# FertigLab/CoGAPS

Measured on AMD Instinct MI355X. Metric: Gibbs atom proposals/sec, 20000x2000 dense D, nPatterns=50, at 1/2/4/8 GPUs, higher is better.
Workload: dtype f32

## Files before the change

cogaps_amd/csrc/eval_kernel.h:

```cpp
#pragma once
#include "gaps_state.h"
#include "gen_kernel.h"

CG_DEVICE cg_f4 ld4(const float *base, uint32_t j) { return reinterpret_cast<const cg_f4 *>(base)[j]; }
CG_DEVICE cg_f4 ld4_stream(const float *base, uint32_t j) { return cg_ld4_stream(base, j); }
CG_DEVICE void st4(float *base, uint32_t j, cg_f4 v) { reinterpret_cast<cg_f4 *>(base)[j] = v; }
CG_DEVICE cg_f4 f4_zero() { cg_f4 z; z.x = 0.f; z.y = 0.f; z.z = 0.f; z.w = 0.f; return z; }
CG_DEVICE cg_f4 f4_one() { cg_f4 z; z.x = 1.f; z.y = 1.f; z.z = 1.f; z.w = 1.f; return z; }

struct EvalAcc { float s, m; };

#define EVAL_ELEM(V, DD, SS, AA) { float ratio = (V) / (SS); a.s = a.s + (V) * ratio; a.m = a.m + ratio * ((DD) - (AA)); }
#define EVAL_ELEM_CH(V, DD, SS, AA) { float ratio = (V) / (SS); a.s = a.s + (V) * ratio; a.m = a.m + ratio * ((DD) - ((AA) + ch * (V))); }

#define EVAL_MODE_ONE 0
#define EVAL_MODE_CH 1
#define EVAL_MODE_SAME 2

#if defined(GEN_TIMELINE)
extern __device__ unsigned long long g_chain_rt[256 * 4];
__device__ unsigned long long g_eval_timeline[2 * 16 * 2 * 12];
#define EVAL_TS(id) do { if ((t & 63u) == 0u && ets_n < 11u) { ets[ets_n++] = ((unsigned long long)cg_clock() << 8) | (unsigned long long)(id); } } while (0)
#define EVAL_TS_DUMP(ty) do { const uint32_t lastW_ = (cg_bdim() - 1u) >> 6; if (cg_bid() < 16u && (t & 63u) == 0u && ((t >> 6) == 0u || (t >> 6) == lastW_) && qlen >= 40u && (PHASE != EVAL_CHAIN || (qlen >= 140u && hot.gs->nSteps - hot.gs->nDone >= 512u))) { \
    unsigned long long *o_ = &g_eval_timeline[((PHASE != EVAL_FUSED && PHASE != EVAL_CHAIN ? 16u : 0u) * 2u + cg_bid() * 2u + ((t >> 6) ? 1u : 0u)) * 12u]; o_[0] = (unsigned long long)(ty); for (uint32_t i_ = 0; i_ < 11u; ++i_) o_[1 + i_] = i_ < ets_n ? ets[i_] : 0ull; } } while (0)
#define EVAL_PIN(x) asm volatile("" : "+v"(x) :: "memory")
#define EVAL_TS_PARAMS , unsigned long long (&ets)[11], uint32_t &ets_n
#define EVAL_TS_ARGS , ets, ets_n
#else
#define EVAL_TS(id) do { } while (0)
#define EVAL_TS_DUMP(ty) do { } while (0)
#define EVAL_PIN(x) do { } while (0)
#define EVAL_TS_PARAMS
#define EVAL_TS_ARGS
#endif

template <int NC, int V>
CG_DEVICE void eval_vfinish(const float *lds, float (&tot)[NC], const uint32_t nwaves = 0u, const uint32_t tid = 0xFFFFFFFFu)
{
    constexpr int NV = NC * V;
    const uint32_t t = tid == 0xFFFFFFFFu ? cg_tid() : tid, nw = cg_fresh_u32(nwaves ? nwaves : (cg_bdim() >> 6));
    if (t < 64u) {
        const uint32_t i = t < (uint32_t)NV ? t : 0u;
        float y[16];
#pragma unroll
        for (uint32_t w = 0; w < 16; ++w) y[w] = lds[w * NV + i];
#pragma unroll
        for (uint32_t w = 0; w < 16; ++w) y[w] = w < nw ? y[w] : 0.f;
#pragma unroll
        for (uint32_t stride = 1; stride < 16u; stride <<= 1) {
#pragma unroll
            for (uint32_t k = 0; k + stride < 16u; k += 2u * stride) y[k] = y[k] + y[k + stride];
        }
        float z = y[0];
        for (int off = 1; off < V; off <<= 1) z = z + cg_shfl_xor_f32(z, off);
#pragma unroll
        for (int c = 0; c < NC; ++c) tot[c] = cg_lane_read_f32(z, c * V);
    }
}

template <int V>
CG_DEVICE void eval_vpark(float x, int j, float *lds, float (&tot)[1])
{
    x = cg_wave_allsum_f32(x);
    const uint32_t t = cg_tid();
    if (cg_bdim() > 64u) { if ((t & 63u) == 0) lds[(t >> 6) * V + j] = x; }
    else tot[0] = x;
}

struct EvalSpec { uint64_t rng; uint32_t n, mm; float l1, l2; };
CG_DEVICE void eval_spec_run(EvalSpec &sp)
{
    uint64_t r = sp.rng;
    sp.l1 = gm_logf_m(pcg_uniform(r), sp.mm);
    if (sp.n > 1u) sp.l2 = gm_logf_m(pcg_uniform(r), sp.mm);
    sp.n = 0u;
}
template <int NR, int MODE>
CG_DEVICE void eval_alpha(const SamplerDev &S, const uint32_t (&row)[NR], const uint32_t (&col)[NR], uint32_t col2, float ch, uint32_t chunk0, uint32_t stride, float *lds, float (&tot)[2 * NR], EvalSpec &spec EVAL_TS_PARAMS)
{
    constexpr int NC = 2 * NR;
    const uint32_t nq = S.Npad >> 2, BS = cg_bdim(), t = cg_tid(), nw = BS >> 6;
    float ps[NR], pm[NR];
    for (int r = 0; r < NR; ++r) { ps[r] = 0.f; pm[r] = 0.f; }
#if defined(GEN_PROFILE)
    if (!(S.dbg & 4u))
#endif
    for (uint32_t j = chunk0 + t; j < nq; j += stride) {
        cg_f4 v[NR], w2, d[NR], s[NR], p[NR];
#pragma unroll
        for (int r = 0; r < NR; ++r) {
            const float *Dr = S.D + (size_t)row[r] * S.Npad, *Sr = S.S2 + (size_t)row[r] * S.Npad, *Ar = S.AP + (size_t)row[r] * S.Npad;
            const float *Vr = S.other + (size_t)col[r] * S.Npad, *V2 = S.other + (size_t)col2 * S.Npad;
            v[r] = ld4(Vr, j); d[r] = ld4_stream(Dr, j); if (!S.defaultS) s[r] = ld4_stream(Sr, j); p[r] = ld4(Ar, j); if (MODE == EVAL_MODE_SAME) w2 = ld4(V2, j);
        }
        if (spec.n) { cg_sched_fence(); eval_spec_run(spec); cg_sched_fence(); }
        if (S.defaultS) {
#pragma unroll
            for (int r = 0; r < NR; ++r) {
                const float sx = gm_max(d[r].x * 0.1f, 0.1f), sy = gm_max(d[r].y * 0.1f, 0.1f), sz = gm_max(d[r].z * 0.1f, 0.1f), sw = gm_max(d[r].w * 0.1f, 0.1f);
                s[r].x = sx * sx; s[r].y = sy * sy; s[r].z = sz * sz; s[r].w = sw * sw;
            }
        }
#pragma unroll
        for (int r = 0; r < NR; ++r) {
            EvalAcc a; a.s = ps[r]; a.m = pm[r];
            if (MODE == EVAL_MODE_CH) { EVAL_ELEM_CH(v[r].x, d[r].x, s[r].x, p[r].x) EVAL_ELEM_CH(v[r].y, d[r].y, s[r].y, p[r].y) EVAL_ELEM_CH(v[r].z, d[r].z, s[r].z, p[r].z) EVAL_ELEM_CH(v[r].w, d[r].w, s[r].w, p[r].w) }
            else if (MODE == EVAL_MODE_SAME) {
                { float x = v[r].x - w2.x; EVAL_ELEM(x, d[r].x, s[r].x, p[r].x) }
                { float x = v[r].y - w2.y; EVAL_ELEM(x, d[r].y, s[r].y, p[r].y) }
                { float x = v[r].z - w2.z; EVAL_ELEM(x, d[r].z, s[r].z, p[r].z) }
                { float x = v[r].w - w2.w; EVAL_ELEM(x, d[r].w, s[r].w, p[r].w) }
            } else { EVAL_ELEM(v[r].x, d[r].x, s[r].x, p[r].x) EVAL_ELEM(v[r].y, d[r].y, s[r].y, p[r].y) EVAL_ELEM(v[r].z, d[r].z, s[r].z, p[r].z) EVAL_ELEM(v[r].w, d[r].w, s[r].w, p[r].w) }
            ps[r] = a.s; pm[r] = a.m;
        }
    }
    { float z_ = ps[0]; EVAL_PIN(z_); ps[0] = z_; } EVAL_TS(10);
#pragma unroll
    for (int r = 0; r < NR; ++r) { ps[r] = cg_wave_allsum_f32(ps[r]); pm[r] = cg_wave_allsum_f32(pm[r]); }
    if (nw > 1) {
        if ((t & 63u) == 0) {
#pragma unroll
            for (int r = 0; r < NR; ++r) { lds[(t >> 6) * NC + 2 * r] = ps[r]; lds[(t >> 6) * NC + 2 * r + 1] = pm[r]; }
        }
        EVAL_TS(11);
        cg_sync();
        EVAL_TS(12);
        eval_vfinish<NC, 1>(lds, tot);
    } else {
#pragma unroll
        for (int r = 0; r < NR; ++r) { tot[2 * r] = ps[r]; tot[2 * r + 1] = pm[r]; }
    }
}

#define EVAL_SEQ_BS 256
CG_DEVICE float eval_seq_fold(float acc, const float *term, uint32_t n)
{
    for (uint32_t i = 0; i < n; ++i) acc = acc + term[i];
    return acc;
}
template <int NR, int MODE>
CG_DEVICE void eval_alpha_seq(const SamplerDev &S, const uint32_t (&row)[NR], const uint32_t (&col)[NR], uint32_t col2, float ch, float *term, float *lds, float (&tot)[2 * NR])
{
    constexpr int NC = 2 * NR;
    const uint32_t nq = S.Npad >> 2, BS = cg_bdim(), t = cg_tid();
    float acc = 0.f;
    for (uint32_t base = 0; base < nq; base += BS) {
        const uint32_t j = base + t;
        if (j < nq) {
#pragma unroll
            for (int r = 0; r < NR; ++r) {
                const float *Dr = S.D + (size_t)row[r] * S.Npad, *Ar = S.AP + (size_t)row[r] * S.Npad;
                const float *Vr = S.other + (size_t)col[r] * S.Npad, *V2 = S.other + (size_t)col2 * S.Npad;
                const cg_f4 v4 = ld4(Vr, j), d4 = ld4(Dr, j), p4 = ld4(Ar, j);
                cg_f4 s4, w4 = f4_zero();
                if (S.defaultS) {
                    const float sx = gm_max(d4.x * 0.1f, 0.1f), sy = gm_max(d4.y * 0.1f, 0.1f), sz = gm_max(d4.z * 0.1f, 0.1f), sw = gm_max(d4.w * 0.1f, 0.1f);
                    s4.x = sx * sx; s4.y = sy * sy; s4.z = sz * sz; s4.w = sw * sw;
                } else s4 = ld4(S.S2 + (size_t)row[r] * S.Npad, j);
                if (MODE == EVAL_MODE_SAME) w4 = ld4(V2, j);
                const float vv[4] = {v4.x, v4.y, v4.z, v4.w}, dd[4] = {d4.x, d4.y, d4.z, d4.w}, pp[4] = {p4.x, p4.y, p4.z, p4.w}, ss[4] = {s4.x, s4.y, s4.z, s4.w}, ww[4] = {w4.x, w4.y, w4.z, w4.w};
#pragma unroll
                for (int e = 0; e < 4; ++e) {
                    const float v = (MODE == EVAL_MODE_SAME) ? vv[e] - ww[e] : vv[e];
                    const float ratio = v / ss[e];
                    const float ap = (MODE == EVAL_MODE_CH) ? pp[e] + ch * vv[e] : pp[e];
                    term[(2 * r) * 4u * BS + 4u * t + (uint32_t)e] = v * ratio;
                    term[(2 * r + 1) * 4u * BS + 4u * t + (uint32_t)e] = ratio * (dd[e] - ap);
                }
            }
        }
        cg_sync();
        const uint32_t first = 4u * base, n = (S.N - first) < 4u * BS ? (S.N - first) : 4u * BS;
        if (t < (uint32_t)NC) acc = eval_seq_fold(acc, term + t * 4u * BS, n);
        cg_sync();
    }
    if (t < (uint32_t)NC) lds[t] = acc;
    cg_sync();
// ... 87 lines not shown
            st4(S.AP + (size_t)r1 * S.Npad, j, q);
        } else {
            st4(S.AP + (size_t)r1 * S.Npad, j, q);
            cg_f4 w = e.p2;
            w.x = w.x + d2 * e.v2.x; w.y = w.y + d2 * e.v2.y; w.z = w.z + d2 * e.v2.z; w.w = w.w + d2 * e.v2.w;
            st4(S.AP + (size_t)r2 * S.Npad, j, w);
        }
    }
    if (nq > stride) eval_update_ap2(S, r1, c1, d1, r2, c2, d2, chunk0 + stride, stride);
}

CG_DEVICE void eval_store_matrix(const SamplerDev &S, uint32_t row, uint32_t col, float oldv, float newv)
{
    S.mat[(size_t)col * S.Mpad + row] = newv;
    const bool was = oldv > 0.f, is = newv > 0.f;
    if (was != is) { if (is) cg_atomic_add_u32(&S.colPos[col], 1u); else cg_atomic_sub_u32(&S.colPos[col], 1u); }
}
CG_DEVICE void eval_cache_erase(const SamplerDev &S, uint32_t h, uint32_t row, uint32_t col)
{
    const uint32_t k = cg_atomic_add_u32(&S.gs->eraseCount, 1u);
    if (k < S.eraseCap) S.eraseList[k] = ((unsigned long long)(row * S.K + col) << 32) | (unsigned long long)h; else S.gs->error = GAPS_ERR_ERASE_CAP;
}
CG_DEVICE void eval_domain_move(const SamplerDev &S, const PropRec &p, const AtomRec &a)
{
    const uint32_t h = p.h1, l = a.left, r = a.right;
    const uint32_t b1 = gen_bin_of(S, p.curPos), b2 = gen_bin_of(S, p.pos);
    const uint32_t head1 = S.binHead[b1];
    atom_set_pos(S, h, l, r, p.pos);
    if (head1 == h) {
        if (r != CG_NONE && gen_bin_of(S, a.rpos) == b1) S.binHead[b1] = r;
        else { S.binHead[b1] = CG_NONE; bm_clear(S, b1); }
    }
    if (l == CG_NONE || gen_bin_of(S, a.lpos) != b2) S.binHead[b2] = h;
    bm_set(S, b2);
}
struct EvalAtoms { AtomRec a1; uint32_t left2; };
CG_DEVICE EvalAtoms eval_atoms_load(const SamplerDev &S, const PropRec &p, bool writer)
{
    EvalAtoms e; e.a1.pos = 0; e.a1.lpos = 0; e.a1.rpos = 0; e.a1.left = CG_NONE; e.a1.right = CG_NONE; e.a1.mass = 0.f; e.a1.rmass = 0.f; e.a1.idx = 0; e.a1.pad0 = 0; e.left2 = CG_NONE;
    if (writer) { e.a1 = S.atoms[p.h1]; if (p.type == 'E') e.left2 = S.atoms[p.h2].left; }
    return e;
}

template <int NC>
CG_DEVICE void eval_pair_fold(const float *lds, const uint32_t tv, const uint32_t nw, float (&tot)[NC])
{
    constexpr int NV = NC * 2;
    if (tv < 64u) {
        const uint32_t i = tv < (uint32_t)NV ? tv : 0u;
        float y[16];
#pragma unroll
        for (uint32_t w = 0; w < 16; ++w) y[w] = lds[w * NV + i];
#pragma unroll
        for (uint32_t w = 0; w < 16; ++w) y[w] = w < nw ? y[w] : 0.f;
#pragma unroll
        for (uint32_t stride = 1; stride < 16u; stride <<= 1) {
#pragma unroll
            for (uint32_t k = 0; k + stride < 16u; k += 2u * stride) y[k] = y[k] + y[k + stride];
        }
        float z = y[0];
        z = z + cg_shfl_xor_f32(z, 1);
#pragma unroll
        for (int c = 0; c < NC; ++c) tot[c] = cg_lane_read_f32(z, c * 2);
    }
}
template <int NR, int MODE>
CG_DEVICE void eval_pair_alpha(const SamplerDev &S, const uint32_t (&row)[NR], const uint32_t (&col)[NR], uint32_t col2, float ch, const uint32_t u, const uint32_t H, float *lds, EvalSpec &spec)
{
    constexpr int NC = 2 * NR;
    const uint32_t nq = S.Npad >> 2;
    float ps[NR][2], pm[NR][2];
    cg_f4 v[2][NR], w2[2], d[2][NR], sq[2][NR], pp[2][NR];
#pragma unroll
    for (int sl = 0; sl < 2; ++sl) {
        const uint32_t j = u + (uint32_t)sl * H, jj = j < nq ? j : nq - 1u;
#pragma unroll
        for (int r = 0; r < NR; ++r) {
            const float *Dr = S.D + (size_t)row[r] * S.Npad, *Ar = S.AP + (size_t)row[r] * S.Npad, *Vr = S.other + (size_t)col[r] * S.Npad;
            v[sl][r] = ld4(Vr, jj); d[sl][r] = ld4_stream(Dr, jj); pp[sl][r] = ld4(Ar, jj);
            if (!S.defaultS) sq[sl][r] = ld4_stream(S.S2 + (size_t)row[r] * S.Npad, jj);
        }
        w2[sl] = (MODE == EVAL_MODE_SAME) ? ld4(S.other + (size_t)col2 * S.Npad, jj) : f4_zero();
    }
    if (spec.n) { cg_sched_fence(); eval_spec_run(spec); cg_sched_fence(); }
#pragma unroll
    for (int sl = 0; sl < 2; ++sl) {
        const uint32_t j = u + (uint32_t)sl * H;
#pragma unroll
        for (int r = 0; r < NR; ++r) {
            if (S.defaultS) {
                const float sx = gm_max(d[sl][r].x * 0.1f, 0.1f), sy = gm_max(d[sl][r].y * 0.1f, 0.1f), sz = gm_max(d[sl][r].z * 0.1f, 0.1f), sw = gm_max(d[sl][r].w * 0.1f, 0.1f);
                sq[sl][r].x = sx * sx; sq[sl][r].y = sy * sy; sq[sl][r].z = sz * sz; sq[sl][r].w = sw * sw;
            }
            EvalAcc a; a.s = 0.f; a.m = 0.f;
            if (j < nq) {
                const cg_f4 vv = v[sl][r], dd = d[sl][r], ss = sq[sl][r], aa = pp[sl][r], ww = w2[sl];
                if (MODE == EVAL_MODE_CH) { EVAL_ELEM_CH(vv.x, dd.x, ss.x, aa.x) EVAL_ELEM_CH(vv.y, dd.y, ss.y, aa.y) EVAL_ELEM_CH(vv.z, dd.z, ss.z, aa.z) EVAL_ELEM_CH(vv.w, dd.w, ss.w, aa.w) }
                else if (MODE == EVAL_MODE_SAME) {
                    { float x = vv.x - ww.x; EVAL_ELEM(x, dd.x, ss.x, aa.x) }
                    { float x = vv.y - ww.y; EVAL_ELEM(x, dd.y, ss.y, aa.y) }
                    { float x = vv.z - ww.z; EVAL_ELEM(x, dd.z, ss.z, aa.z) }
                    { float x = vv.w - ww.w; EVAL_ELEM(x, dd.w, ss.w, aa.w) }
                } else { EVAL_ELEM(vv.x, dd.x, ss.x, aa.x) EVAL_ELEM(vv.y, dd.y, ss.y, aa.y) EVAL_ELEM(vv.z, dd.z, ss.z, aa.z) EVAL_ELEM(vv.w, dd.w, ss.w, aa.w) }
            }
            ps[r][sl] = a.s; pm[r][sl] = a.m;
        }
    }
#pragma unroll
    for (int r = 0; r < NR; ++r) {
#pragma unroll
        for (int sl = 0; sl < 2; ++sl) { ps[r][sl] = cg_wave_allsum_f32(ps[r][sl]); pm[r][sl] = cg_wave_allsum_f32(pm[r][sl]); }
    }
    if ((u & 63u) == 0u) {
        float *o = lds + (u >> 6) * (NC * 2);
#pragma unroll
        for (int r = 0; r < NR; ++r) { o[(2 * r) * 2 + 0] = ps[r][0]; o[(2 * r) * 2 + 1] = ps[r][1]; o[(2 * r + 1) * 2 + 0] = pm[r][0]; o[(2 * r + 1) * 2 + 1] = pm[r][1]; }
    }
}
CG_DEVICE void eval_pair_update(const SamplerDev &S, const DecRec &d, const uint32_t u, const uint32_t H)
{
    const uint32_t nq = S.Npad >> 2;
    if (d.n == 0u) return;
    float *AP1 = S.AP + (size_t)d.r1 * S.Npad; const float *V1 = S.other + (size_t)d.c1 * S.Npad;
    const bool second = d.n == 2u, same = second && d.r1 == d.r2;
    float *AP2 = S.AP + (size_t)(second ? d.r2 : d.r1) * S.Npad; const float *V2 = S.other + (size_t)(second ? d.c2 : d.c1) * S.Npad;
    cg_f4 v1[2], p1[2], v2[2], p2[2];
#pragma unroll
    for (int sl = 0; sl < 2; ++sl) {
        const uint32_t j = u + (uint32_t)sl * H, jj = j < nq ? j : nq - 1u;
        v1[sl] = ld4(V1, jj); p1[sl] = ld4(AP1, jj); v2[sl] = ld4(V2, jj); p2[sl] = ld4(AP2, jj);
    }
#pragma unroll
    for (int sl = 0; sl < 2; ++sl) {
        const uint32_t j = u + (uint32_t)sl * H;
        if (j < nq) {
            cg_f4 q = p1[sl];
            q.x = q.x + d.d1 * v1[sl].x; q.y = q.y + d.d1 * v1[sl].y; q.z = q.z + d.d1 * v1[sl].z; q.w = q.w + d.d1 * v1[sl].w;
            if (same) { q.x = q.x + d.d2 * v2[sl].x; q.y = q.y + d.d2 * v2[sl].y; q.z = q.z + d.d2 * v2[sl].z; q.w = q.w + d.d2 * v2[sl].w; }
            st4(AP1, j, q);
            if (second && !same) {
                cg_f4 w = p2[sl];
                w.x = w.x + d.d2 * v2[sl].x; w.y = w.y + d.d2 * v2[sl].y; w.z = w.z + d.d2 * v2[sl].z; w.w = w.w + d.d2 * v2[sl].w;
                st4(AP2, j, w);
            }
        }
    }
}
CG_DEVICE void eval_chain_pair(const SamplerDev &S, unsigned long long *grans, const uint32_t tag, const float T, const PropRec &pA, const PropRec &pB, const uint32_t qA, const uint32_t qB)
{
    CG_SHARED float ldsP[2][16 * 8];
    CG_SHARED DecRec decP[2];
    const uint32_t t = cg_tid(), H = cg_bdim() >> 1, h = t >= H ? 1u : 0u, u = t - h * H, nwH = H >> 6;
    const PropRec p = h ? pB : pA;
    const uint32_t q = h ? qB : qA;
    const uint32_t mm = GM_MATH_PORTABLE;
    const float lambda = S.lambda;
    const bool scalarLane = u < 64u;
    uint64_t rng = p.rng;
    const bool two = (p.type == 'M' || p.type == 'E');
    const float m1 = p.m1, m2 = p.m2, old1 = p.old1, old2 = p.old2;
    const bool gibbs1 = (p.gibbs & 1u) != 0u, gibbs2 = (p.gibbs & 2u) != 0u;
    const bool need = (p.type == 'B') ? gibbs1 : ((p.type == 'D' || p.type == 'M') ? true : (gibbs1 || gibbs2));
    const bool diff = two && p.r1 != p.r2;
    const uint32_t alphaUnits = need ? (!two ? 4u : (diff ? 8u : 5u)) : 0u;
    EvalSpec spec; spec.rng = rng; spec.mm = mm; spec.l1 = 0.f; spec.l2 = 0.f;
    spec.n = (scalarLane && need && (p.type == 'D' || p.type == 'M')) ? ((p.type == 'D' && gibbs1) ? 2u : 1u) : 0u;
    float *lds = &ldsP[h][0];
    if (need) {
        const uint32_t rowA[1] = {p.r1}, colA[1] = {p.c1};
        if (diff) { const uint32_t rowAB[2] = {p.r1, p.r2}, colAB[2] = {p.c1, p.c2}; eval_pair_alpha<2, EVAL_MODE_ONE>(S, rowAB, colAB, 0u, 0.f, u, H, lds, spec); }
        else if (p.type == 'D') eval_pair_alpha<1, EVAL_MODE_CH>(S, rowA, colA, 0u, -1.f * m1, u, H, lds, spec);
        else if (two) eval_pair_alpha<1, EVAL_MODE_SAME>(S, rowA, colA, p.c2, 0.f, u, H, lds, spec);
        else eval_pair_alpha<1, EVAL_MODE_ONE>(S, rowA, colA, 0u, 0.f, u, H, lds, spec);
    }
    cg_sync();
    float s = 0.f, smu = 0.f;
    if (need) {
        if (diff) { float tot[4] = {0.f, 0.f, 0.f, 0.f}; eval_pair_fold<4>(lds, u, nwH, tot); s = tot[0] + tot[2]; smu = tot[1] - tot[3]; }
        else { float t2[2] = {0.f, 0.f}; eval_pair_fold<2>(lds, u, nwH, t2); s = t2[0]; smu = t2[1]; }
        if (spec.n) eval_spec_run(spec);
    }
    s = s * T; smu = smu * T;
    DecRec owe; owe.n = 0; owe.r1 = 0; owe.c1 = 0; owe.d1 = 0.f; owe.r2 = 0; owe.c2 = 0; owe.d2 = 0.f; owe.pad = 0;
    if (scalarLane) {
        uint32_t code = CHAIN_NONE, nUpd = 0; float val = 0.f;
        if (p.type == 'B') {
            float bv = 0.f; uint32_t bhas = 0;
            if (gibbs1) { OptF g = gm_gibbs_mass(s, smu, 0.f, S.maxGibbsMass, rng, S.luts, true, lambda); bv = g.v; bhas = g.has ? 1u : 0u; }
            else { bv = pcg_exponential(rng, lambda, mm); bhas = 1u; }
            if (bhas != 0u && bv >= GAPS_EPSILON) { code = CHAIN_APPLY; val = bv; nUpd = 1u; owe.n = 1u; owe.r1 = p.r1; owe.c1 = p.c1; owe.d1 = bv; }
            else code = CHAIN_ERASE;
        } else if (p.type == 'D') {
            float rebirth = m1; bool drew = false;
            if (gibbs1) { OptF g = gm_gibbs_mass(s, smu, 0.f, S.maxGibbsMass, rng, S.luts, true, lambda); if (g.has) { rebirth = g.v; drew = true; } }
            const float deltaLL = rebirth * (smu - s * rebirth / 2.f);
            const float logU = drew ? spec.l2 : spec.l1;
            if (logU < deltaLL) {
                if (rebirth != m1) { const float nv = gm_max(old1 + (rebirth - m1), 0.f); code = CHAIN_APPLY; val = rebirth; nUpd = 1u; owe.n = 1u; owe.r1 = p.r1; owe.c1 = p.c1; owe.d1 = nv - old1; }
            } else { const float nv = gm_max(old1 + (-1.f * m1), 0.f); code = CHAIN_ERASE; nUpd = 1u; owe.n = 1u; owe.r1 = p.r1; owe.c1 = p.c1; owe.d1 = nv - old1; }
        } else if (p.type == 'M') {
            const float deltaLL = -1.f * m1 * (smu + s * m1 / 2.f);
            if (spec.l1 < deltaLL) { const float nv1 = gm_max(old1 + (-m1), 0.f); code = CHAIN_APPLY; nUpd = 2u; owe.n = 2u; owe.r1 = p.r1; owe.c1 = p.c1; owe.d1 = nv1 - old1; owe.r2 = p.r2; owe.c2 = p.c2; owe.d2 = m1; }
        } else if (need) {
            OptF g0 = gm_gibbs_mass(s, smu, -m1, m2, rng, S.luts, false, 0.f);
            const float gv = g0.v, n1 = m1 + gv, n2 = m2 - gv;
            if (g0.has && n1 > GAPS_EPSILON && n2 > GAPS_EPSILON) {
                const float nv1 = gm_max(old1 + (n1 - m1), 0.f), nv2 = gm_max(old2 + (n2 - m2), 0.f);
                code = CHAIN_APPLY; val = gv; nUpd = 2u; owe.n = 2u; owe.r1 = p.r1; owe.c1 = p.c1; owe.d1 = nv1 - old1; owe.r2 = p.r2; owe.c2 = p.c2; owe.d2 = nv2 - old2;
            }
        }
        if (u == 0u) {
            unsigned long long *gr = grans + (size_t)q * CHAIN_GRAN_STRIDE; const uint32_t units = nUpd * 3u + alphaUnits;
            cg_store_agent_u64(&gr[0], ((unsigned long long)tag << 32) | (unsigned long long)(code | (units << 8)));
            cg_store_agent_u64(&gr[1], ((unsigned long long)tag << 32) | (unsigned long long)gm_f2u(val));
            decP[h] = owe;
        }
    }
    cg_sync();
    const DecRec d = decP[h];
    eval_pair_update(S, d, u, H);
    cg_sync();
}

#if defined(GEN_PROFILE) && !defined(GEN_SUBMARKS) && !defined(GEN_ROUNDMARKS)
#define EVAL_PROF(i) do { if (t == 0 && cg_bid() == 0) { unsigned long long now_ = cg_clock(); cg_atomic_add_u64(&S.gs->prof[8 + (i)], now_ - eprof_last); eprof_last = now_; } } while (0)
#else
#define EVAL_PROF(i) do { } while (0)
#endif

#define EVAL_FUSED 0
#define EVAL_ALPHA 1
#define EVAL_APPLY 2
#define EVAL_SEQ 3
#define EVAL_CHAIN 5
#define EVAL_CHAIN_SPLIT 6
#define EVAL_DECIDE 4

struct EvalHot { const PropRec *queue; const GenScalars *gs; uint32_t queueCap; const ChainSlot *slot; unsigned long long *grans; };
struct EvalFirst { PropRec p; uint32_t qlen; float T; uint32_t tag; };
template <int PHASE>
CG_DEVICE EvalFirst eval_first(const EvalHot hot, uint32_t slices, uint32_t vbid)
{
    const uint32_t qFirst = (PHASE == EVAL_FUSED || PHASE == EVAL_SEQ || PHASE == EVAL_CHAIN) ? vbid : vbid / slices;
    EvalFirst f; f.p = hot.queue[qFirst < hot.queueCap ? qFirst : 0u]; f.T = hot.gs->annealTemp;
    if (PHASE == EVAL_CHAIN || PHASE == EVAL_CHAIN_SPLIT) { const ChainSlot cs = *hot.slot; f.qlen = cs.qlen; f.tag = cs.tag; }
    else { f.qlen = hot.gs->qlen; f.tag = (PHASE == EVAL_DECIDE) ? (uint32_t)hot.gs->batchEpoch : 0u; }
    return f;
}
template <int PHASE>
CG_DEVICE const SamplerDev &eval_record(const SamplerDev CG_CONSTANT *sp)
{
    cg_sched_fence();
    cg_const_lines lines;
    cg_const_warm_begin<sizeof(SamplerDev)>(sp, lines);
    sp = cg_const_warm_end(sp, lines);
    return *(const SamplerDev *)sp;
}
CG_DEVICE void eval_chain_updates(const SamplerDev &S, const EvalHot hot, const uint32_t tag, const uint32_t qlen, const uint32_t wg, const uint32_t nwg)
{
    const uint32_t TPB = cg_bdim(), nq = S.Npad >> 2;
    uint32_t parts = (nq + 4u * TPB - 1u) / (4u * TPB);
    parts = parts < 1u ? 1u : (parts > 64u ? 64u : parts);
    for (uint32_t item = wg; item < qlen * parts; item += nwg) {
        const uint32_t q = item / parts, part = item - q * parts;
        const PropRec p = hot.queue[q < hot.queueCap ? q : 0u];
        const unsigned long long *gr = hot.grans + (size_t)q * CHAIN_GRAN_STRIDE;
        unsigned long long g0 = 0ull, g1 = 0ull; uint32_t spins = 0; bool have = true;
        for (;;) {
            g0 = cg_load_l2_u64(&gr[0]); g1 = cg_load_l2_u64(&gr[1]);
            const bool ok = (uint32_t)(g0 >> 32) == tag && (uint32_t)(g1 >> 32) == tag;
            if (cg_ballot(!ok) == 0ull) break;
            if (cg_poll_expired(++spins)) { if (cg_tid() == 0u) S.gs->error = GAPS_ERR_SPIN; have = false; break; }
            cg_poll_pause();
        }
        if (!have) return;
        const uint32_t code = (uint32_t)g0 & 0xFFu; const float val = gm_u2f((uint32_t)g1);
        const float m1 = p.m1, m2 = p.m2, old1 = p.old1, old2 = p.old2;
        if (code == CHAIN_APPLY) {
            if (p.type == 'B') eval_update_ap(S, p.r1, p.c1, val, part * TPB, TPB * parts);
            else if (p.type == 'D') { const float nv = gm_max(old1 + (val - m1), 0.f); eval_update_ap(S, p.r1, p.c1, nv - old1, part * TPB, TPB * parts); }
            else if (p.type == 'M') { const float nv1 = gm_max(old1 + (-m1), 0.f); eval_update_ap2(S, p.r1, p.c1, nv1 - old1, p.r2, p.c2, m1, part * TPB, TPB * parts); }
            else if (p.type == 'E') {
                const float n1 = m1 + val, n2 = m2 - val;
                const float nv1 = gm_max(old1 + (n1 - m1), 0.f), nv2 = gm_max(old2 + (n2 - m2), 0.f);
                eval_update_ap2(S, p.r1, p.c1, nv1 - old1, p.r2, p.c2, nv2 - old2, part * TPB, TPB * parts);
            }
        } else if (code == CHAIN_ERASE && p.type == 'D') { const float nv = gm_max(old1 + (-1.f * m1), 0.f); eval_update_ap(S, p.r1, p.c1, nv - old1, part * TPB, TPB * parts); }
    }
}

template <int PHASE, bool SINGLE>
CG_DEVICE void eval_body(const SamplerDev &S, uint32_t slices, const uint32_t vbid, const uint32_t vgdim, const EvalHot hot, const EvalFirst &first)
{
#if defined(GEN_TIMELINE)
    unsigned long long ets[11]; uint32_t ets_n = 0;
#endif
    constexpr bool CHAINP = PHASE == EVAL_CHAIN_SPLIT;
    constexpr bool CHAIN = PHASE == EVAL_CHAIN || CHAINP;
    constexpr bool FUSEDF = PHASE == EVAL_FUSED || PHASE == EVAL_CHAIN;
    const uint32_t qFirst = (FUSEDF || PHASE == EVAL_SEQ) ? vbid : vbid / slices;
    PropRec pNext = first.p;
    const uint32_t qlen = first.qlen;
    const float T = first.T;
    CG_SHARED float lds[16 * 4];
    CG_SHARED float decf; CG_SHARED uint32_t deci;

    CG_SHARED float seqTerm[PHASE == EVAL_SEQ ? 4 * 4 * EVAL_SEQ_BS : 1];
    constexpr bool WHOLE = FUSEDF || PHASE == EVAL_SEQ;
    const uint32_t mm = (PHASE == EVAL_SEQ) ? S.mathMode : GM_MATH_PORTABLE;
    const uint32_t t = cg_tid(), BS = cg_bdim();
#if defined(GEN_PROFILE) && !defined(GEN_SUBMARKS) && !defined(GEN_ROUNDMARKS)
    unsigned long long eprof_last = cg_clock();
#endif
    const float lambda = S.lambda;
    EVAL_TS(0);
    const bool multiWave = BS > 64u;
    const bool scalarLane = !multiWave || t < 64u;
    const uint32_t slice = WHOLE ? 0u : vbid % slices;
    const uint32_t qStep = WHOLE ? vgdim : vgdim / slices;
    const uint32_t chunk0 = slice * BS, stride = WHOLE ? BS : S.redW;
    constexpr bool DECIDE = PHASE == EVAL_DECIDE || CHAINP;
    const bool decider = DECIDE && slice + 1u == slices;
    const bool writer = !CHAIN && (DECIDE ? decider : slice == 0u) && t == 0u;
#if defined(GEN_TIMELINE)
#define EVAL_PUBLISH_RT() do { if (CHAIN && t == 0u && q < 255u && qlen >= 140u && hot.gs->nSteps - hot.gs->nDone >= 512u) g_chain_rt[q * 4u + 1u] = __builtin_amdgcn_s_memrealtime(); } while (0)
#else
#define EVAL_PUBLISH_RT() do { } while (0)
#endif
#define EVAL_PUBLISH(CODE, VAL, NUPD) do { EVAL_TS(7); EVAL_PUBLISH_RT(); if (CHAIN && t == 0u) { unsigned long long *gr_ = hot.grans + (size_t)q * CHAIN_GRAN_STRIDE; const uint32_t units_ = (NUPD) * 3u + alphaUnits; \
        cg_store_agent_u64(&gr_[0], ((unsigned long long)first.tag << 32) | (unsigned long long)((CODE) | (units_ << 8))); \
        cg_store_agent_u64(&gr_[1], ((unsigned long long)first.tag << 32) | (unsigned long long)gm_f2u(VAL)); } } while (0)
#define EVAL_BCAST(F0, I0) do { if (multiWave && !DECIDE) { if (t == 0) { decf = (F0); deci = (I0); } cg_sync(); (F0) = decf; (I0) = deci; } } while (0)
    if (PHASE == EVAL_DECIDE && vbid == 0u && t == 0u) S.gs->applyCount = qlen;
    for (uint32_t q = qFirst; ; q += qStep) {
        const PropRec p = pNext;
        if (q >= qlen) break;
        if (PHASE == EVAL_CHAIN && q + qStep < qlen && (S.Npad >> 2) <= BS && BS >= 128u) {
            const uint32_t qB = q + qStep;
            const PropRec pB = hot.queue[qB < hot.queueCap ? qB : 0u];
            const uint32_t qN = qB + qStep;
            if (qN < qlen) pNext = hot.queue[qN < hot.queueCap ? qN : 0u];
#if defined(COGAPS_EMUL)
            if (t == 0u) cg_atomic_add_u64(&S.gs->prof[7], 1ull);
#endif
            eval_chain_pair(S, hot.grans, first.tag, T, p, pB, q, qB);
            if (qN >= qlen) break;
            q = qB;
            continue;
        }
        { uint32_t ty_ = p.type; EVAL_PIN(ty_); }
        EVAL_TS(1);
        uint64_t rng = p.rng; uint32_t nUpd = 0;
#if defined(EVAL_ATOMS_LATE)
        EvalAtoms ea = eval_atoms_load(S, p, writer && PHASE == EVAL_SEQ);
#else
        EvalAtoms ea = eval_atoms_load(S, p, writer && (PHASE == EVAL_FUSED || PHASE == EVAL_SEQ));
#endif
        bool eaLoaded = false;
        const bool two = (p.type == 'M' || p.type == 'E');
        const float m1 = p.m1, m2 = p.m2, old1 = p.old1, old2 = p.old2;
        const bool gibbs1 = (p.gibbs & 1u) != 0u, gibbs2 = (p.gibbs & 2u) != 0u;
        EVAL_PROF(0);
        EVAL_TS(2);
#if defined(GEN_PROFILE)
        if (S.dbg & 1u) { if (p.type == 0xFFu || m1 == -1.f) S.queueUnits[q] = (uint32_t)old1; break; }
#endif
        bool need = (p.type == 'B') ? gibbs1 : ((p.type == 'D' || p.type == 'M') ? true : (gibbs1 || gibbs2));
#if defined(GEN_PROFILE)
        if (S.dbg & 16u) need = false;
#endif
        const bool diff = two && p.r1 != p.r2;
        const uint32_t alphaUnits = need ? (!two ? 4u : (diff ? 8u : 5u)) : 0u;
        float s = 0.f, smu = 0.f;
        uint32_t typeX = p.type;
        constexpr bool PRE = FUSEDF && SINGLE;
        EvalPre pre; pre.v1 = f4_zero(); pre.p1 = f4_zero(); pre.v2 = f4_zero(); pre.p2 = f4_zero();
        const uint32_t jPre = chunk0 + t;
#define EVAL_PREFETCH() do { if (PRE && jPre < (S.Npad >> 2)) { \
            pre.v1 = ld4(S.other + (size_t)p.c1 * S.Npad, jPre); pre.p1 = ld4(S.AP + (size_t)p.r1 * S.Npad, jPre); \
            if (two) { pre.v2 = ld4(S.other + (size_t)p.c2 * S.Npad, jPre); if (p.r1 != p.r2) pre.p2 = ld4(S.AP + (size_t)p.r2 * S.Npad, jPre); } } } while (0)
        DecRec owe; owe.n = 0; owe.r1 = 0; owe.c1 = 0; owe.d1 = 0.f; owe.r2 = 0; owe.c2 = 0; owe.d2 = 0.f; owe.pad = 0;
#define EVAL_UPD1(ROW, COL, DELTA) do { if (DECIDE) { owe.n = 1u; owe.r1 = (ROW); owe.c1 = (COL); owe.d1 = (DELTA); } \
            else if (PRE) eval_update_pre1(S, (ROW), (COL), (DELTA), chunk0, stride, pre.v1, pre.p1); else eval_update_ap(S, (ROW), (COL), (DELTA), chunk0, stride); } while (0)
#define EVAL_UPD2(R1, C1, D1, R2, C2, D2) do { if (DECIDE) { owe.n = 2u; owe.r1 = (R1); owe.c1 = (C1); owe.d1 = (D1); owe.r2 = (R2); owe.c2 = (C2); owe.d2 = (D2); } \
            else if (PRE) eval_update_pre2(S, (R1), (C1), (D1), (R2), (C2), (D2), chunk0, stride, pre); else eval_update_ap2(S, (R1), (C1), (D1), (R2), (C2), (D2), chunk0, stride); } while (0)
        constexpr bool AHEAD = (FUSEDF && SINGLE) || DECIDE;
        EvalSpec spec; spec.rng = rng; spec.mm = mm; spec.l1 = 0.f; spec.l2 = 0.f;
        spec.n = (AHEAD && scalarLane && need && (p.type == 'D' || p.type == 'M')) ? ((p.type == 'D' && gibbs1) ? 2u : 1u) : 0u;
        if (need) {
            float tot[4] = {0.f, 0.f, 0.f, 0.f};
            if (PHASE == EVAL_SEQ) {
                const uint32_t rowA[1] = {p.r1}, colA[1] = {p.c1};
                if (diff) {
                    const uint32_t rowAB[2] = {p.r1, p.r2}, colAB[2] = {p.c1, p.c2};
                    eval_alpha_seq<2, EVAL_MODE_ONE>(S, rowAB, colAB, 0u, 0.f, seqTerm, lds, tot);
                } else {
                    float t2[2] = {0.f, 0.f};
                    if (p.type == 'D') eval_alpha_seq<1, EVAL_MODE_CH>(S, rowA, colA, 0u, -1.f * m1, seqTerm, lds, t2);
                    else if (two) eval_alpha_seq<1, EVAL_MODE_SAME>(S, rowA, colA, p.c2, 0.f, seqTerm, lds, t2);
                    else eval_alpha_seq<1, EVAL_MODE_ONE>(S, rowA, colA, 0u, 0.f, seqTerm, lds, t2);
                    tot[0] = t2[0]; tot[1] = t2[1];
                }
            } else if (PHASE != EVAL_APPLY) {
                const uint32_t rowA[1] = {p.r1}, colA[1] = {p.c1};
                if (diff) {
                    const uint32_t rowAB[2] = {p.r1, p.r2}, colAB[2] = {p.c1, p.c2};
                    eval_alpha<2, EVAL_MODE_ONE>(S, rowAB, colAB, 0u, 0.f, chunk0, stride, lds, tot, spec EVAL_TS_ARGS);
                } else {
                    float t2[2] = {0.f, 0.f};
                    if (p.type == 'D') eval_alpha<1, EVAL_MODE_CH>(S, rowA, colA, 0u, -1.f * m1, chunk0, stride, lds, t2, spec EVAL_TS_ARGS);
                    else if (two) eval_alpha<1, EVAL_MODE_SAME>(S, rowA, colA, p.c2, 0.f, chunk0, stride, lds, t2, spec EVAL_TS_ARGS);
                    else eval_alpha<1, EVAL_MODE_ONE>(S, rowA, colA, 0u, 0.f, chunk0, stride, lds, t2, spec EVAL_TS_ARGS);
                    tot[0] = t2[0]; tot[1] = t2[1];
                }
                if (PHASE == EVAL_ALPHA) { if (t == 0) { float *o = S.partials + (size_t)q * 64u + slice; o[0] = tot[0]; o[16] = tot[1]; o[32] = tot[2]; o[48] = tot[3]; } }
                if (DECIDE && t < 64u) {
                    unsigned long long *gr = S.grans + (size_t)q * 64u;
                    if (!decider) {
                        if (t < 4u) { const float v = t == 0u ? tot[0] : (t == 1u ? tot[1] : (t == 2u ? tot[2] : tot[3])); cg_store_agent_u64(&gr[slice * 4u + t], ((unsigned long long)first.tag << 32) | (unsigned long long)gm_f2u(v)); }
                    } else {
                        ea = eval_atoms_load(S, p, writer); eaLoaded = true;
                        const uint32_t comp = t >> 4, sl = t & 15u;
                        const bool want = sl + 1u < slices;
                        unsigned long long g = 0ull; uint32_t spins = 0;
                        for (;;) {
                            if (want) g = cg_load_l2_u64(&gr[sl * 4u + comp]);
                            const bool ok = !want || (uint32_t)(g >> 32) == first.tag;
                            if (cg_ballot(!ok) == 0ull) break;
                            if (cg_poll_expired(++spins)) { if (t == 0u) S.gs->error = GAPS_ERR_SPIN; typeX = 0u; break; }
                            cg_poll_pause();
                        }
                        const float own = comp == 0u ? tot[0] : (comp == 1u ? tot[1] : (comp == 2u ? tot[2] : tot[3]));
                        float z = want ? gm_u2f((uint32_t)g) : (sl + 1u == slices ? own : 0.f);
                        const uint32_t slots = S.redW / BS;
                        for (uint32_t st = 1; st < slots; st <<= 1) z = z + cg_shfl_xor_f32(z, (int)st);
                        tot[0] = cg_lane_read_f32(z, 0); tot[1] = cg_lane_read_f32(z, 16); tot[2] = cg_lane_read_f32(z, 32); tot[3] = cg_lane_read_f32(z, 48);
                    }
                }
            } else {
                if (t < 64u) {
                    const uint32_t slots = S.redW / BS;
                    float z = ((t & 15u) < slices) ? S.partials[(size_t)q * 64u + t] : 0.f;
                    for (uint32_t st = 1; st < slots; st <<= 1) z = z + cg_shfl_xor_f32(z, (int)st);
                    tot[0] = cg_lane_read_f32(z, 0); tot[1] = cg_lane_read_f32(z, 16); tot[2] = cg_lane_read_f32(z, 32); tot[3] = cg_lane_read_f32(z, 48);
                }
            }
            s = diff ? tot[0] + tot[2] : tot[0]; smu = diff ? tot[1] - tot[3] : tot[1];
            if (AHEAD && spec.n) eval_spec_run(spec);
        }
        EVAL_PIN(s); EVAL_TS(3);
        if (FUSEDF) EVAL_PREFETCH();
#if defined(EVAL_ATOMS_LATE)
        if (PHASE == EVAL_FUSED) ea = eval_atoms_load(S, p, writer);
#endif
        if (PHASE == EVAL_APPLY || (DECIDE && !eaLoaded)) ea = eval_atoms_load(S, p, writer);
        if (PHASE == EVAL_ALPHA || (DECIDE && !decider)) { if (q + qStep >= qlen) break; { const uint32_t qn_ = q + qStep; pNext = hot.queue[qn_ < hot.queueCap ? qn_ : 0u]; } cg_sync(); continue; }
        s = s * T; smu = smu * T;
#if defined(GEN_PROFILE)
        if (S.dbg & 8u) { if (q + qStep >= qlen) break; { const uint32_t qn_ = q + qStep; pNext = hot.queue[qn_ < hot.queueCap ? qn_ : 0u]; } cg_sync(); continue; }
#endif
        if (typeX == 'B') {
            float bv = 0.f; uint32_t bhas = 0;
            if (scalarLane) {
                if (gibbs1) { OptF g = gm_gibbs_mass(s, smu, 0.f, S.maxGibbsMass, rng, S.luts, true, lambda); bv = g.v; bhas = g.has ? 1u : 0u; }
                else { bv = pcg_exponential(rng, lambda, mm); bhas = 1u; }
                if (bhas != 0u && bv >= GAPS_EPSILON) EVAL_PUBLISH(CHAIN_APPLY, bv, 1u); else EVAL_PUBLISH(CHAIN_ERASE, 0.f, 0u);
            }
            EVAL_PIN(bv); EVAL_TS(4);
            EVAL_BCAST(bv, bhas);
            EVAL_TS(5);
            if (bhas != 0u && bv >= GAPS_EPSILON) {
                EVAL_UPD1(p.r1, p.c1, bv);
                ++nUpd;
                if (writer) { atom_set_mass(S, p.h1, ea.a1.left, bv); eval_store_matrix(S, p.r1, p.c1, old1, old1 + bv); }
            } else if (writer) eval_cache_erase(S, p.h1, p.r1, p.c1);
        } else if (typeX == 'D') {
            float rebirth = m1;
            EVAL_PROF(1);
            uint32_t acc = 0;
            if (scalarLane) {
                bool drew = false;
                if (gibbs1) {
                    OptF g = gm_gibbs_mass(s, smu, 0.f, S.maxGibbsMass, rng, S.luts, true, lambda);
                    if (g.has) { rebirth = g.v; drew = true; }
                }
                const float deltaLL = rebirth * (smu - s * rebirth / 2.f);
                const float logU = (AHEAD && need) ? (drew ? spec.l2 : spec.l1) : gm_logf_m(pcg_uniform(rng), mm);
                acc = (logU < deltaLL) ? 1u : 0u;
                if (acc != 0u) { if (rebirth != m1) EVAL_PUBLISH(CHAIN_APPLY, rebirth, 1u); else EVAL_PUBLISH(CHAIN_NONE, 0.f, 0u); } else EVAL_PUBLISH(CHAIN_ERASE, 0.f, 1u);
            }
            EVAL_PIN(acc); EVAL_TS(4);
            EVAL_BCAST(rebirth, acc);
            EVAL_TS(5);
            EVAL_PROF(2);
            if (acc != 0u) {
                if (rebirth != m1) {
                    const float nv = gm_max(old1 + (rebirth - m1), 0.f);
                    EVAL_UPD1(p.r1, p.c1, nv - old1);
                    ++nUpd;
                    if (writer) { eval_store_matrix(S, p.r1, p.c1, old1, nv); atom_set_mass(S, p.h1, ea.a1.left, rebirth); }
                }
            } else {
                const float nv = gm_max(old1 + (-1.f * m1), 0.f);
                EVAL_UPD1(p.r1, p.c1, nv - old1);
                ++nUpd;
                if (writer) { eval_store_matrix(S, p.r1, p.c1, old1, nv); eval_cache_erase(S, p.h1, p.r1, p.c1); }
            }
            EVAL_PROF(3);
        } else if (typeX == 'M') {
            uint32_t acc = 0; float unused = 0.f;
            if (scalarLane) { const float deltaLL = -1.f * m1 * (smu + s * m1 / 2.f); const float logU = (AHEAD && need) ? spec.l1 : gm_logf_m(pcg_uniform(rng), mm); acc = (logU < deltaLL) ? 1u : 0u;
                              if (acc) EVAL_PUBLISH(CHAIN_APPLY, 0.f, 2u); else EVAL_PUBLISH(CHAIN_NONE, 0.f, 0u); }
            EVAL_PIN(acc); EVAL_TS(4);
            EVAL_BCAST(unused, acc);
            EVAL_TS(5);
            if (acc) {
                const float nv1 = gm_max(old1 + (-m1), 0.f);
                EVAL_UPD2(p.r1, p.c1, nv1 - old1, p.r2, p.c2, m1);
                nUpd += 2;
                if (writer) {
                    eval_domain_move(S, p, ea.a1);
                    eval_store_matrix(S, p.r1, p.c1, old1, nv1);
                    eval_store_matrix(S, p.r2, p.c2, old2, old2 + m1);
                }
            }
        } else if (need && typeX == 'E') {
            float gv = 0.f; uint32_t gh = 0;
            if (scalarLane) { OptF g0 = gm_gibbs_mass(s, smu, -m1, m2, rng, S.luts, false, 0.f); gv = g0.v; gh = g0.has ? 1u : 0u;
                              if (gh != 0u && m1 + gv > GAPS_EPSILON && m2 - gv > GAPS_EPSILON) EVAL_PUBLISH(CHAIN_APPLY, gv, 2u); else EVAL_PUBLISH(CHAIN_NONE, 0.f, 0u); }
            EVAL_PIN(gv); EVAL_TS(4);
            EVAL_BCAST(gv, gh);
            EVAL_TS(5);
            const float n1 = m1 + gv, n2 = m2 - gv;
            if (gh != 0u && n1 > GAPS_EPSILON && n2 > GAPS_EPSILON) {
                const float nv1 = gm_max(old1 + (n1 - m1), 0.f);
                const float nv2 = gm_max(old2 + (n2 - m2), 0.f);
                EVAL_UPD2(p.r1, p.c1, nv1 - old1, p.r2, p.c2, nv2 - old2);
                nUpd += 2;
                if (writer) {
                    eval_store_matrix(S, p.r1, p.c1, old1, nv1);
                    eval_store_matrix(S, p.r2, p.c2, old2, nv2);
                    atom_set_mass(S, p.h1, ea.a1.left, n1); atom_set_mass(S, p.h2, ea.left2, n2);
                }
            }
        }
        else EVAL_PUBLISH(CHAIN_NONE, 0.f, 0u);
        EVAL_TS(6);
        EVAL_TS_DUMP(p.type | (nUpd << 8) | ((p.r1 == p.r2 ? 1u : 0u) << 16));
        if (DECIDE && writer) S.dec[q] = owe;
        if (writer) {
            uint32_t units = nUpd * 3u;
            if (need) units += !two ? 4u : (diff ? 8u : 5u);
            S.queueUnits[q] = units;
        }
        if (q + qStep >= qlen) break;
        { const uint32_t qn_ = q + qStep; pNext = hot.queue[qn_ < hot.queueCap ? qn_ : 0u]; }
        cg_sync();
    }
#if !defined(COGAPS_EMUL)
    if (CHAINP) eval_chain_updates(S, hot, first.tag, qlen, vbid, vgdim);
#endif
}

template <int PHASE>
#ifndef EVAL_APPLY_WAVES
#define EVAL_APPLY_WAVES 6
#endif
CG_KERNEL void CG_LAUNCH_BOUNDS2((PHASE == EVAL_SEQ ? EVAL_SEQ_BS : 1024), (PHASE == EVAL_FUSED || PHASE == EVAL_SEQ ? 4 : (PHASE == EVAL_APPLY || PHASE == EVAL_DECIDE ? EVAL_APPLY_WAVES : 8))) eval_kernel(const PropRec *hotQueue, const GenScalars *hotGs, uint32_t hotCap, uint32_t slices, const SamplerDev CG_CONSTANT *sp)
{
    EvalHot hot; hot.queue = hotQueue; hot.gs = hotGs; hot.queueCap = hotCap; hot.slot = nullptr; hot.grans = nullptr;
    const EvalFirst first = eval_first<PHASE>(hot, slices, cg_bid());
    const SamplerDev &S = eval_record<PHASE>(sp);
    eval_body<PHASE, true>(S, slices, cg_bid(), cg_gdim(), hot, first);
}

template <int PHASE>
#ifndef EVAL_MULTI_FUSED_WAVES
#define EVAL_MULTI_FUSED_WAVES 6
#endif
CG_KERNEL void CG_LAUNCH_BOUNDS2(1024, (PHASE == EVAL_FUSED ? EVAL_MULTI_FUSED_WAVES : (PHASE == EVAL_APPLY ? EVAL_APPLY_WAVES : 8))) eval_kernel_multi(const SamplerDev CG_CONSTANT *arr, uint32_t slices, uint32_t wgPerChain)
{
    const uint32_t chain = cg_bid() / wgPerChain;
    const SamplerDev CG_CONSTANT *sp = arr + chain;
    cg_const_warm<sizeof(SamplerDev)>(sp);
    const SamplerDev &S = *(const SamplerDev *)sp;
    EvalHot hot; hot.queue = S.queue; hot.gs = S.gs; hot.queueCap = S.queueCap; hot.slot = nullptr; hot.grans = nullptr;
    const uint32_t vbid = cg_bid() - chain * wgPerChain;
    eval_body<PHASE, false>(S, slices, vbid, wgPerChain, hot, eval_first<PHASE>(hot, slices, vbid));
}

CG_DEVICE void eval_apply_items(const SamplerDev &S, const uint32_t wg, const uint32_t nwg)
{
    const uint32_t count = S.gs->applyCount;
    const uint32_t TPB = cg_bdim(), nq = S.Npad >> 2;
    uint32_t parts = (nq + 4u * TPB - 1u) / (4u * TPB);
    parts = parts < 1u ? 1u : (parts > 64u ? 64u : parts);
    for (uint32_t item = wg; item < count * parts; item += nwg) {
        const uint32_t q = item / parts, part = item - q * parts;
        const DecRec d = S.dec[q];
        if (d.n == 1u) eval_update_ap(S, d.r1, d.c1, d.d1, part * TPB, TPB * parts);
        else if (d.n == 2u) eval_update_ap2(S, d.r1, d.c1, d.d1, d.r2, d.c2, d.d2, part * TPB, TPB * parts);
    }
}
template <int WIN>
CG_KERNEL void CG_LAUNCH_BOUNDS(WIN + 64) gen_apply_kernel(const uint64_t *lcgMul, const uint64_t *lcgInc, GenScalars *gs, const unsigned long long *eraseList, const uint32_t *queueUnits,
                                                          uint32_t eraseCap, uint32_t queueCap, const SamplerDev CG_CONSTANT *sp)
{
    if (cg_bid() != 0u) {
        cg_const_warm<sizeof(SamplerDev)>(sp);
        eval_apply_items(*(const SamplerDev *)sp, cg_bid() - 1u, cg_gdim() - 1u);
        return;
    }
    GenHot hot; hot.lcgMul = lcgMul; hot.lcgInc = lcgInc; hot.gs = gs; hot.eraseList = eraseList; hot.queueUnits = queueUnits; hot.eraseCap = eraseCap; hot.queueCap = queueCap;
    gen_body<WIN, true, false, 0>(sp, hot);
}
```

cogaps_amd/csrc/gen_chain_apply.h:

```cpp
#pragma once
struct ChainItem {
    uint32_t type; float m1, m2, old1, old2; uint64_t pos; unsigned long long eraseEntry;
    float *mass1, *rm1, *mass2, *rm2;
    float *mat1, *mat2; uint32_t *col1, *col2;
    uint64_t *pos1, *rposL, *lposR;
    uint32_t mb1, mb2;
    uint32_t *head1, *head2; uint32_t head1Val, h1;
    unsigned long long *b0clr, *b0set, *b1set, *b2set; uint32_t bit1, bit2, bit1w, bit2w;
    uint32_t hL, hR, h2, l2, cell1, cell2, idx;
    uint32_t sparse; float *rows1, *rows2; unsigned long long *fl1, *fl2; unsigned long long fbit1, fbit2; float colv1, colv2; uint32_t flg1, flg2;
};
CG_DEVICE void chain_item_clear(ChainItem &it)
{
    it.type = 0; it.m1 = 0.f; it.m2 = 0.f; it.old1 = 0.f; it.old2 = 0.f; it.pos = 0; it.eraseEntry = 0ull;
    it.mass1 = nullptr; it.rm1 = nullptr; it.mass2 = nullptr; it.rm2 = nullptr; it.mat1 = nullptr; it.mat2 = nullptr; it.col1 = nullptr; it.col2 = nullptr;
    it.mb1 = 0; it.mb2 = 0;
    it.pos1 = nullptr; it.rposL = nullptr; it.lposR = nullptr; it.head1 = nullptr; it.head2 = nullptr; it.head1Val = CG_NONE; it.h1 = 0;
    it.b0clr = nullptr; it.b0set = nullptr; it.b1set = nullptr; it.b2set = nullptr; it.bit1 = 0; it.bit2 = 0; it.bit1w = 0; it.bit2w = 0;
    it.hL = CG_NONE; it.hR = CG_NONE; it.h2 = CG_NONE; it.l2 = CG_NONE; it.cell1 = 0; it.cell2 = 0; it.idx = 0;
    it.sparse = 0; it.rows1 = nullptr; it.rows2 = nullptr; it.fl1 = nullptr; it.fl2 = nullptr; it.fbit1 = 0ull; it.fbit2 = 0ull; it.colv1 = 0.f; it.colv2 = 0.f; it.flg1 = 0; it.flg2 = 0;
}
struct ChainMid { AtomRec a; uint32_t l2, head1, b1, b2; unsigned long long x1, x2;
                  float colv1, colv2; unsigned long long fw1, fw2; };
CG_DEVICE ChainMid chain_fetch_mid(const SamplerDev &S, const PropRec &p, const bool sparse)
{
    ChainMid m;
    const uint32_t hE = p.type == 'E' ? p.h2 : p.h1;
    m.b1 = gen_bin_of(S, p.curPos); m.b2 = gen_bin_of(S, p.pos);
    const uint32_t w0 = m.b2 >> 6, w1 = w0 >> 6, w2 = w1 >> 6;
    m.a = S.atoms[p.h1];
    m.l2 = S.atoms[hE].left;
    m.head1 = S.binHead[m.b1];
    m.x1 = S.bits1[w1]; m.x2 = S.bits2[w2];
    m.colv1 = 0.f; m.colv2 = 0.f; m.fw1 = 0ull; m.fw2 = 0ull;
    if (sparse) {
        m.colv1 = S.mat[(size_t)p.c1 * S.Mpad + p.r1]; m.fw1 = S.mflags[(size_t)p.c1 * S.Mw + (p.r1 >> 6)];
        m.colv2 = S.mat[(size_t)p.c2 * S.Mpad + p.r2]; m.fw2 = S.mflags[(size_t)p.c2 * S.Mw + (p.r2 >> 6)];
    }
    return m;
}
CG_DEVICE void chain_fetch_build(const SamplerDev &S, const PropRec &p, const ChainMid &m, ChainItem &it, const bool sparse);
CG_DEVICE void chain_fetch(const SamplerDev &S, const PropRec *queueRd, uint32_t q, ChainItem &it, const bool sparse)
{
    const PropRec p = queueRd[q];
    const ChainMid m = chain_fetch_mid(S, p, sparse);
    chain_fetch_build(S, p, m, it, sparse);
}
CG_DEVICE void chain_fetch_build(const SamplerDev &S, const PropRec &p, const ChainMid &m, ChainItem &it, const bool sparse)
{
    chain_item_clear(it);
    it.type = p.type; it.m1 = p.m1; it.m2 = p.m2; it.old1 = p.old1; it.old2 = p.old2; it.pos = p.pos; it.h1 = p.h1;
    it.eraseEntry = ((unsigned long long)(p.r1 * S.K + p.c1) << 32) | (unsigned long long)p.h1;
    const AtomRec a = m.a;
    it.hL = a.left; it.hR = a.right; it.idx = a.idx; it.cell1 = p.r1 * S.K + p.c1; it.cell2 = p.r2 * S.K + p.c2; it.h2 = p.h2; it.l2 = m.l2;
    it.mass1 = &S.atoms[p.h1].mass; it.rm1 = a.left != CG_NONE ? &S.atoms[a.left].rmass : nullptr;
    it.mat1 = &S.mat[(size_t)p.c1 * S.Mpad + p.r1]; it.col1 = &S.colPos[p.c1];
    const bool two = p.type == 'M' || p.type == 'E';
    if (two) { it.mat2 = &S.mat[(size_t)p.c2 * S.Mpad + p.r2]; it.col2 = &S.colPos[p.c2]; }
    if (sparse) {
        it.sparse = 1u;
        it.rows1 = &S.rows[(size_t)p.r1 * S.Kpad + p.c1]; it.fl1 = &S.mflags[(size_t)p.c1 * S.Mw + (p.r1 >> 6)]; it.fbit1 = 1ull << (p.r1 & 63u);
        it.colv1 = m.colv1; it.flg1 = (uint32_t)((m.fw1 >> (p.r1 & 63u)) & 1ull);
        if (two) {
            it.rows2 = &S.rows[(size_t)p.r2 * S.Kpad + p.c2]; it.fl2 = &S.mflags[(size_t)p.c2 * S.Mw + (p.r2 >> 6)]; it.fbit2 = 1ull << (p.r2 & 63u);
            it.colv2 = m.colv2; it.flg2 = (uint32_t)((m.fw2 >> (p.r2 & 63u)) & 1ull);
        }
    }
    if (p.type == 'E') { const uint32_t l2 = m.l2; it.mass2 = &S.atoms[p.h2].mass; it.rm2 = l2 != CG_NONE ? &S.atoms[l2].rmass : nullptr; }
    if (p.type == 'M') {
        const uint32_t b1 = m.b1, b2 = m.b2;
        it.mb1 = b1; it.mb2 = b2;
        const uint32_t head1 = m.head1;
        const uint32_t w0 = b2 >> 6, w1 = w0 >> 6, w2 = w1 >> 6;
        const unsigned long long x1 = m.x1, x2 = m.x2;
        it.pos1 = &S.atoms[p.h1].pos; it.rposL = a.left != CG_NONE ? &S.atoms[a.left].rpos : nullptr; it.lposR = a.right != CG_NONE ? &S.atoms[a.right].lpos : nullptr;
        if (head1 == p.h1) {
            it.head1 = &S.binHead[b1];
            if (a.right != CG_NONE && gen_bin_of(S, a.rpos) == b1) it.head1Val = a.right; else { it.head1Val = CG_NONE; it.b0clr = &S.bits0[b1 >> 6]; it.bit1 = b1 & 63u; }
        }
        if (a.left == CG_NONE || gen_bin_of(S, a.lpos) != b2) it.head2 = &S.binHead[b2];
        it.b0set = &S.bits0[w0]; it.bit2 = b2 & 63u;
        if (!((x1 >> (w0 & 63u)) & 1ull)) { it.b1set = &S.bits1[w1]; it.bit1w = w0 & 63u; }
        if (!((x2 >> (w1 & 63u)) & 1ull)) { it.b2set = &S.bits2[w2]; it.bit2w = w1 & 63u; }
    }
}
CG_DEVICE void chain_store_matrix(float *cell, uint32_t *col, float oldv, float newv)
{
    *cell = newv;
    const bool was = oldv > 0.f, is = newv > 0.f;
    if (was != is) { if (is) cg_atomic_add_u32(col, 1u); else cg_atomic_sub_u32(col, 1u); }
}
CG_DEVICE void chain_store_hybrid(float *rowCell, float *colCell, unsigned long long *flagWord, unsigned long long bit, uint32_t *colCount, float rowNew, float colNew, bool wasFlagged)
{
    *rowCell = rowNew;
    const bool zero = colNew < GAPS_EPSILON;
    if (zero) {
        if (wasFlagged) { (void)cg_atomic_and_u64(flagWord, ~bit); (void)cg_atomic_sub_u32(colCount, 1u); }
        *colCell = 0.f;
    } else {
        if (!wasFlagged) { (void)cg_atomic_or_u64(flagWord, bit); (void)cg_atomic_add_u32(colCount, 1u); }
        *colCell = colNew;
    }
}
CG_DEVICE bool chain_apply(const ChainItem &it, uint32_t code, float val)
{
    const uint32_t tB = it.type == 'B', tD = it.type == 'D', tM = it.type == 'M', tE = it.type == 'E';
    const bool app = code == CHAIN_APPLY, era = code == CHAIN_ERASE;
    const float n1 = tE ? it.m1 + val : val, n2 = it.m2 - val;
    float d1 = tB ? val : (tD ? (val - it.m1) : (tM ? -it.m1 : (n1 - it.m1)));
    d1 = (era && tD) ? -1.f * it.m1 : d1;
    const float s1 = it.old1 + d1;
    const float nv1 = tB ? s1 : gm_max(s1, 0.f);
    const float s2 = it.old2 + (tM ? it.m1 : (n2 - it.m2));
    const float nv2 = tM ? s2 : gm_max(s2, 0.f);
    const bool doMat1 = app || (era && tD != 0u), doMat2 = app && (tM | tE) != 0u;
    const bool doMass1 = app && tM == 0u, doMass2 = app && tE != 0u;
    if (doMass1) { *it.mass1 = n1; if (it.rm1) *it.rm1 = n1; }
    if (doMass2) { *it.mass2 = n2; if (it.rm2) *it.rm2 = n2; }
    if (it.sparse) {
        if (doMat1) { const float colNew = tB ? it.colv1 + d1 : nv1; chain_store_hybrid(it.rows1, it.mat1, it.fl1, it.fbit1, it.col1, nv1, colNew, it.flg1 != 0u); }
        if (doMat2) { const float colNew = tM ? it.colv2 + it.m1 : nv2; chain_store_hybrid(it.rows2, it.mat2, it.fl2, it.fbit2, it.col2, nv2, colNew, it.flg2 != 0u); }
    } else {
        if (doMat1) chain_store_matrix(it.mat1, it.col1, it.old1, nv1);
        if (doMat2) chain_store_matrix(it.mat2, it.col2, it.old2, nv2);
    }
    if (app && tM != 0u) {
        *it.pos1 = it.pos; if (it.rposL) *it.rposL = it.pos; if (it.lposR) *it.lposR = it.pos;
        if (it.head1) *it.head1 = it.head1Val;
        if (it.b0clr) cg_atomic_and_u64(it.b0clr, ~(1ull << it.bit1));
        if (it.head2) *it.head2 = it.h1;
        cg_atomic_or_u64(it.b0set, 1ull << it.bit2);
        if (it.b1set) cg_atomic_or_u64(it.b1set, 1ull << it.bit1w);
        if (it.b2set) cg_atomic_or_u64(it.b2set, 1ull << it.bit2w);
    }
    return era;
}
```

cogaps_amd/csrc/gen_draw.h:

```cpp
#pragma once
struct GenRoundCtx {
    unsigned t; uint64_t jm0, ji0, jm1, ji1, seed1, batchEpoch, g_qrng; uint32_t n0, updBase, remaining, K, g_skip, e_prevQ; float dp0, g_u1, g_u2; GenScalars *gs;
    float tabHi, tabLo;
    PropRec *queueOut;
    uint32_t dpBase;
    uint32_t sparse;
};
struct GenSpec {
    uint32_t bBefore, dBefore, guess, active; float u1, u2;
    uint32_t go, ct, info; uint64_t rng, pos; uint32_t bin, r1, c1;
};
template <int WIN>
CG_DEVICE void gen_spec_a1(const SamplerDev &S, GenShared<WIN> &sh, const GenRoundCtx &c, const uint32_t nLo, const uint32_t nHi, const float dpAtLo, const float dpAtHi, GenSpec &sp)
{
    const unsigned t = c.t;
    const uint32_t winN = c.remaining < (uint32_t)WIN ? c.remaining : (uint32_t)WIN;
    const uint32_t active = t < winN;
    uint64_t s = (c.g_skip ? c.jm1 : c.jm0) * c.g_qrng + (c.g_skip ? c.ji1 : c.ji0);
    float u1 = pcg_uniform(s), u2 = pcg_uniform(s);
    const uint32_t cached = (c.g_skip != 0u) & (uint32_t)(t == 0u);
    u1 = cached ? c.g_u1 : u1; u2 = cached ? c.g_u2 : u2;
    const uint32_t gLo = gen_decide(u1, u2, nLo, nLo, dpAtLo, dpAtLo), gHi = gen_decide(u1, u2, nHi, nHi, dpAtHi, dpAtHi);
    if (cg_ballot(active && gLo != gHi) != 0ull && (t & 63u) == 0u) sh.specBad = 1u;
#if defined(GEN_SPEC_BAD_EVERY)
    if (t == 0u && (sh.g.batchEpoch % (uint64_t)GEN_SPEC_BAD_EVERY) == 0ull) sh.specBad = 1u;
#endif
    const uint32_t guess = active ? gHi : (uint32_t)GEN_T_NONE;
    sh.u1[t] = u1; sh.u2[t] = u2;
    uint32_t eX[4], tX[4];
    gen_count4<WIN>(sh.wtot4, t, guess == 'B', guess == 'D', guess == 'M', guess == 'E', eX, tX);
    sp.bBefore = eX[0]; sp.dBefore = eX[1]; sp.u1 = u1; sp.u2 = u2; sp.guess = guess; sp.active = active;
    const uint32_t goA = (uint32_t)(guess != GEN_T_NONE);
    const uint32_t k0 = (uint32_t)(guess == 'B') | (uint32_t)(guess == 'D'), k1 = (uint32_t)(guess == 'M');
    const uint32_t T0 = tX[0] + tX[1], T1 = tX[2], T2 = tX[3];
    if (goA) {
        uint32_t slot = T0 + T1 + eX[3];
        slot = k1 ? T0 + eX[2] : slot;
        slot = k0 ? eX[0] + eX[1] : slot;
        sh.perm[slot] = (uint16_t)t;
        sh.info[t] = guess | (eX[0] << 8);
    }
    if (t == 0) { sh.nWork = T0 + T1 + T2; sh.nBD = T0; }
}
template <int WIN>
CG_DEVICE void gen_spec_slot(const SamplerDev &S, GenShared<WIN> &sh, const GenRoundCtx &c, GenSpec &sp)
{
    const unsigned t = c.t;
    const bool go = t < sh.nWork;
    sp.go = go ? 1u : 0u;
    sp.ct = go ? (uint32_t)sh.perm[t] : 0u;
    sp.info = go ? sh.info[sp.ct] : 0u;
    sp.rng = go ? pcg_from_seed(sh.seed[sp.ct]) : 0ull;
    sp.pos = 0; sp.bin = 0; sp.r1 = 0; sp.c1 = 0;
    if (go && (sp.info & 0xFFu) == 'B') {
        uint64_t x = pcg_u64(sp.rng);
        while (x >= S.limitL) x = pcg_u64(sp.rng);
        sp.pos = (S.iPartL == 1ull ? x : gm_udiv64(x, S.iPartL)) + 1ull;
        sp.bin = gen_bin_of(S, sp.pos); sp.r1 = gen_div_k(S, sp.bin); sp.c1 = sp.bin - sp.r1 * c.K;
    }
}

CG_DEVICE void gen_mark_dirty(uint32_t *dirty, uint32_t bin)
{
    const uint32_t w = (bin >> 6) & 16383u;
    cg_atomic_or_u32(&dirty[w >> 5], 1u << (w & 31u));
}

struct GenNotePos { uint32_t a, b; };
template <int WORDS>
CG_DEVICE GenNotePos gen_note_pos(uint32_t key)
{
    constexpr uint32_t LOG2 = WORDS == 4096 ? 17u : (WORDS == 2048 ? 16u : 13u);
    static_assert(WORDS == 4096 || WORDS == 2048 || WORDS == 256, "bit numbers are 17 / 16 / 13 bits of the hash");
    const uint32_t h = key * 2654435761u;
    GenNotePos p; p.a = h >> (32u - LOG2); p.b = (h ^ (h >> 11)) & ((1u << LOG2) - 1u);
    return p;
}
CG_DEVICE void gen_note_set(uint32_t *bits, const GenNotePos p)
{
    cg_atomic_or_u32(&bits[p.a >> 5], 1u << (p.a & 31u));
    cg_atomic_or_u32(&bits[p.b >> 5], 1u << (p.b & 31u));
}
CG_DEVICE uint32_t gen_note_get(const uint32_t *bits, const GenNotePos p)
{
    return (bits[p.a >> 5] >> (p.a & 31u)) & (bits[p.b >> 5] >> (p.b & 31u)) & 1u;
}

struct GenDraw {
    uint32_t go, flags; bool isB, pick;
    uint64_t rng, rngPick, pos, cpos;
    uint32_t h1, h2, i1, hl, hr, r1, c1, r2, c2, bin;
    float nm1, nm2, amass, m2x, old1, old2; uint32_t gib1, gib2;
    uint64_t lposB, rposB; float rmassB;
    uint32_t headBin, v2, v3, xPick; bool redo;
};
CG_DEVICE void gen_draw_clear(GenDraw &d)
{
    d.go = 0; d.flags = 0; d.isB = false; d.pick = false; d.rng = 0; d.rngPick = 0; d.pos = 0; d.cpos = 0;
    d.h1 = CG_NONE; d.h2 = CG_NONE; d.i1 = CG_NONE; d.hl = CG_NONE; d.hr = CG_NONE; d.r1 = 0; d.c1 = 0; d.r2 = 0; d.c2 = 0; d.bin = 0;
    d.nm1 = 0.f; d.nm2 = 0.f; d.amass = 0.f; d.m2x = 0.f; d.old1 = 0.f; d.old2 = 0.f; d.gib1 = 0; d.gib2 = 0; d.lposB = 0; d.rposB = 0; d.rmassB = 0.f;
    d.headBin = 0; d.v2 = CG_NONE; d.v3 = CG_NONE; d.xPick = 0; d.redo = false;
}
template <int WIN, bool SPEC, bool AHEAD = false>
CG_DEVICE void gen_draw_a(const SamplerDev &S, const GenRoundCtx &c, const GenSpec *spec, const bool go, const uint32_t type, const uint32_t bBefore, const uint64_t rng0, const uint32_t nR, GenDraw &d)
{
    gen_draw_clear(d);
    d.go = go ? 1u : 0u;
    d.isB = go && type == 'B';
    d.pick = go && type != 'B';
    d.rng = rng0;
    const uint32_t nT = nR + bBefore;
    if (d.isB) {
        if (SPEC) { d.pos = spec->pos; d.bin = spec->bin; d.r1 = spec->r1; d.c1 = spec->c1; }
        else {
            uint64_t x = pcg_u64(d.rng);
            while (x >= S.limitL) x = pcg_u64(d.rng);
            d.pos = (S.iPartL == 1ull ? x : gm_udiv64(x, S.iPartL)) + 1ull;
            d.bin = gen_bin_of(S, d.pos); d.r1 = gen_div_k(S, d.bin); d.c1 = d.bin - d.r1 * c.K;
        }
        d.i1 = nT;
    } else if (d.pick) {
        if (AHEAD) {
            uint64_t r2 = d.rng; d.xPick = pcg_u32(r2);
            if (d.xPick >= nT * (0xFFFFFFFFu / nT)) d.redo = true;
        }
        d.i1 = pcg_uniform32(d.rng, 0u, nT - 1u);
        if (d.i1 >= nR) { d.flags |= GEN_F_FAIL; d.pick = false; }
    }
    d.rngPick = d.rng;
}
template <int WIN, bool AHEAD, class F>
CG_DEVICE void gen_draw_b(const SamplerDev &S, GenShared<WIN> &sh, const GenRoundCtx &c, const uint32_t type, GenDraw &d, F underTrip, const uint32_t keepH1 = CG_NONE, const bool soft = false)
{
    const uint32_t K = c.K;
    const bool isB = d.isB, pick = d.pick;
    uint32_t flags = d.flags;
    uint64_t rng = d.rng, pos = d.pos, cpos = 0, lbpos = 0, rbpos = 0;
    uint32_t h1 = CG_NONE, h2 = CG_NONE, hl = CG_NONE, hr = CG_NONE;
    uint32_t r1 = d.r1, c1 = d.c1, r2 = 0, c2 = 0; float nm1 = 0.f, nm2 = 0.f;
    uint32_t bin = d.bin, headBin = 0; unsigned long long w0 = 0;
    const uint32_t i1 = d.i1;
    uint32_t v1 = CG_NONE;
    unsigned long long w0n = 0ull;
    uint32_t v2 = CG_NONE;
    AtomRec b3; b3.pos = 0; b3.lpos = 0; b3.rpos = 0; b3.left = CG_NONE; b3.right = CG_NONE; b3.mass = 0.f; b3.rmass = 0.f; b3.idx = 0;
    if (isB) { w0 = S.bits0[bin >> 6]; w0n = ((bin >> 6) + 1u < S.nWords0) ? S.bits0[(bin >> 6) + 1u] : 0ull; }
    if (pick) v1 = keepH1 != CG_NONE ? keepH1 : S.vec[i1];
    underTrip();
    bool slowB = false;
    if (isB) {
        const uint32_t bit = bin & 63u;
        if ((w0 >> bit) & 1ull) headBin = bin;
        else {
            flags |= GEN_F_BINEMPTY; if (w0 == 0ull) flags |= GEN_F_WORDZERO;
            const unsigned long long m = (bit == 63u) ? 0ull : (w0 & ~((2ull << bit) - 1ull));
            if (m) headBin = (bin & ~63u) + (uint32_t)cg_ctz64(m); else if (w0n) headBin = (bin & ~63u) + 64u + (uint32_t)cg_ctz64(w0n);
            else slowB = true;
        }
    }
    AtomRec a; a.pos = 0; a.lpos = 0; a.rpos = 0; a.left = CG_NONE; a.right = CG_NONE; a.mass = 0.f; a.rmass = 0.f; a.idx = 0;
    if (isB && !slowB) v2 = S.binHead[headBin];
    if (pick) { h1 = v1; a = S.atoms[h1]; }
    uint64_t lp = 0, rp = 0;
    float m2x = 0.f;
    bool frontE = false;
    if (pick) {
        cpos = a.pos;
        const uint32_t b1 = gen_bin_of(S, cpos);
        r1 = gen_div_k(S, b1); c1 = b1 - r1 * K;
        hl = a.left;
        if (type == 'M') { hr = a.right; lp = a.lpos; rp = a.rpos; }
        else if (type == 'E') {
            hr = a.right;
            if (hr != CG_NONE) { h2 = hr; rbpos = a.rpos; m2x = a.rmass; }
            else { h2 = sh.g.front; frontE = true; }
        }
    }
    if ((AHEAD || soft) && frontE) { d.redo = true; frontE = false; h2 = h1; }
    float old1 = 0.f, old2 = 0.f; uint32_t gib1 = 0, gib2 = 0;
    uint64_t lposB = 0, rposB = 0; float rmassB = 0.f;
    if (AHEAD && isB && !slowB && v2 == CG_NONE) { d.redo = true; slowB = true; }
    if (isB && !slowB) b3 = S.atoms[v2];
    if (frontE) b3 = S.atoms[h2];
    if (isB || pick) { old1 = c.sparse ? S.rows[(size_t)r1 * S.Kpad + c1] : S.mat[(size_t)c1 * S.Mpad + r1]; gib1 = S.otherColPos[c1]; }
    if (pick && type == 'M') {
        if (hl != CG_NONE) { flags |= GEN_F_HASLEFT; lbpos = lp; } else lbpos = 0;
        if (hr != CG_NONE) { flags |= GEN_F_HASRIGHT; rbpos = rp; } else rbpos = S.rboundNone;
        pos = pcg_uniform64(rng, lbpos + 1ull, rbpos - 1ull);
        const uint32_t bin2 = gen_bin_of(S, pos);
        r2 = gen_div_k(S, bin2); c2 = bin2 - r2 * K;
        if (r1 == r2 && c1 == c2) flags |= GEN_F_INLINE;
    }
    if (pick && type == 'E' && !frontE) {
        flags |= GEN_F_HASRIGHT;
        const uint32_t bin2 = gen_bin_of(S, rbpos);
        r2 = gen_div_k(S, bin2); c2 = bin2 - r2 * K;
    }
    if (pick && (type == 'M' || (type == 'E' && !frontE))) { old2 = c.sparse ? S.rows[(size_t)r2 * S.Kpad + c2] : S.mat[(size_t)c2 * S.Mpad + r2]; gib2 = S.otherColPos[c2]; }
    if (isB) {
        if (!slowB) {
            if ((flags & GEN_F_BINEMPTY) || b3.pos > pos) { hr = v2; hl = b3.left; lposB = b3.lpos; rposB = b3.pos; rmassB = b3.mass; flags |= GEN_F_NEWHEAD; }
            else if (b3.pos == pos) slowB = true;
            else {
                uint32_t cur = v2, nxt = b3.right; uint64_t curPos = b3.pos, nxtPos = b3.rpos; float nxtMass = b3.rmass;
                for (;;) {
                    if (nxt == CG_NONE) break;
                    if (nxtPos == pos) { slowB = true; break; }
                    if (nxtPos > pos) break;
                    if (AHEAD) { if (d.v3 != CG_NONE) { d.redo = true; break; } d.v3 = nxt; }
                    const AtomRec w = S.atoms[nxt];
                    cur = nxt; curPos = nxtPos; nxt = w.right; nxtPos = w.rpos; nxtMass = w.rmass;
                }
                hl = cur; hr = nxt; lposB = curPos; rposB = nxtPos; rmassB = nxtMass;
            }
        }
        if (AHEAD && slowB) { d.redo = true; slowB = false; }
#if defined(EXP_NO_SLOW)
        slowB = false;
#endif
        if (slowB) {
            bool occ, nh;
            gen_find_gap(S, pos, bin, &hl, &hr, &occ, &nh);
            while (occ) {
                pos = pcg_uniform64(rng, 1ull, S.domainLenU);
                bin = gen_bin_of(S, pos); r1 = gen_div_k(S, bin); c1 = bin - r1 * K;
                gen_find_gap(S, pos, bin, &hl, &hr, &occ, &nh);
            }
            flags &= ~(GEN_F_BINEMPTY | GEN_F_WORDZERO | GEN_F_NEWHEAD);
            if (nh) flags |= GEN_F_NEWHEAD;
            if (S.binHead[bin] == CG_NONE) { flags |= GEN_F_BINEMPTY; if (S.bits0[bin >> 6] == 0ull) flags |= GEN_F_WORDZERO; }
            old1 = c.sparse ? S.rows[(size_t)r1 * S.Kpad + c1] : S.mat[(size_t)c1 * S.Mpad + r1]; gib1 = S.otherColPos[c1];
            lposB = (hl != CG_NONE) ? S.atoms[hl].pos : 0ull;
            if (hr != CG_NONE) { rposB = S.atoms[hr].pos; rmassB = S.atoms[hr].mass; } else { rposB = 0ull; rmassB = 0.f; }
        }
    } else if (pick && type == 'E') {
        if (frontE) {
            rbpos = b3.pos; m2x = b3.mass;
            const uint32_t bin2 = gen_bin_of(S, rbpos);
            r2 = gen_div_k(S, bin2); c2 = bin2 - r2 * K;
            old2 = c.sparse ? S.rows[(size_t)r2 * S.Kpad + c2] : S.mat[(size_t)c2 * S.Mpad + r2]; gib2 = S.otherColPos[c2];
        }
        if (r1 == r2 && c1 == c2 && !((AHEAD || soft) && d.redo)) {
            flags |= GEN_F_INLINE;
            const float m1 = a.mass, m2 = m2x;
#if defined(EXP_NO_GAMMA)
            const float newMass = m1;
#else
            const float newMass = pcg_trunc_gamma_upper(rng, S.luts, m1 + m2, 1.f / S.lambda, S.mathMode);
#endif
            const float delta = (m1 > m2) ? newMass - m1 : m2 - newMass;
            if (m1 + delta > GAPS_EPSILON && m2 - delta > GAPS_EPSILON) { flags |= GEN_F_APPLY; nm1 = m1 + delta; nm2 = m2 - delta; }
        }
    }
    d.flags = flags; d.rng = rng; d.pos = pos; d.cpos = cpos; d.h1 = h1; d.h2 = h2; d.hl = hl; d.hr = hr; d.r1 = r1; d.c1 = c1; d.r2 = r2; d.c2 = c2; d.bin = bin;
    d.nm1 = nm1; d.nm2 = nm2; d.amass = a.mass; d.m2x = m2x; d.old1 = old1; d.old2 = old2; d.gib1 = gib1; d.gib2 = gib2; d.lposB = lposB; d.rposB = rposB; d.rmassB = rmassB;
    d.headBin = headBin; d.v2 = v2;
}

struct GenCheck { GenNotePos atomA, atomB, slot, cellA, cellB, eraseA; uint32_t iPartS; };
CG_DEVICE GenCheck gen_draw_check(const GenSpec &sp, const GenDraw &d, const uint32_t nRs, const uint32_t K)
{
    const bool isB = (sp.info & 0xFFu) == 'B';
    GenCheck c;
    c.cellA = gen_note_pos<GEN_DIRTY_CELLS>(isB ? d.bin : d.r1 * K + d.c1); c.cellB = gen_note_pos<GEN_DIRTY_CELLS>(d.r2 * K + d.c2);
    c.atomA = gen_note_pos<GEN_DIRTY_ATOMS>(isB ? d.v2 : d.h1); c.atomB = gen_note_pos<GEN_DIRTY_ATOMS>(d.v3); c.slot = gen_note_pos<GEN_DIRTY_ATOMS>(~d.i1);
    c.eraseA = gen_note_pos<GEN_DIRTY_ERASE>(d.h1);
    c.iPartS = 0xFFFFFFFFu / (nRs + (sp.info >> 8));
    return c;
}
#ifndef GEN_MOVED_PICK_ATOMS_PER_ERASED
#define GEN_MOVED_PICK_ATOMS_PER_ERASED 10240u
#endif
template <int WIN>
CG_DEVICE uint32_t gen_draw_valid(const SamplerDev &S, GenShared<WIN> &sh, const GenSpec &sp, const GenDraw &d, const GenCheck &ck, const uint32_t nR, const uint32_t m, uint32_t &moved)
{
    moved = 0u;
    const uint32_t type = sp.info & 0xFFu, bBefore = sp.info >> 8;
    uint32_t bad = d.redo ? 1u : 0u, light = 0u;
#if defined(GEN_AHEAD_BAD_EVERY)
    if (((sp.ct + (uint32_t)sh.g.batchEpoch) % (uint32_t)GEN_AHEAD_BAD_EVERY) == 0u) { if (sp.ct & 1u) bad = 1u; else light = 1u; }
#endif
    const bool isB = type == 'B';
    const bool reads = isB || d.pick;
    const uint32_t nA = gen_note_get(sh.dAtom, ck.atomA), nB = gen_note_get(sh.dAtom, ck.atomB), nS = gen_note_get(sh.dAtom, ck.slot);
    const uint32_t cA = gen_note_get(sh.dCell, ck.cellA), cB = gen_note_get(sh.dCell, ck.cellB);
    if (isB) { if (reads) bad |= nA | cA; if (d.v3 != CG_NONE) bad |= nB; }
    else if (d.pick) {
        const uint32_t nE = gen_note_get(sh.dErase, ck.eraseA);
        light |= nA | cA | ((type == 'M' || type == 'E') ? cB : 0u);
        bad |= nA & nE;
    }
#if defined(GEN_TIMELINE)
    uint32_t tlSame = 1u, tlQ = 0u, tlRem = 0u, tlDirty = 0u;
#endif
    if (isB) {
        const uint32_t wFirst = d.bin >> 6;
        uint32_t wLast = d.headBin >> 6; wLast = wLast > wFirst + 1u ? wLast : wFirst + 1u;
        uint32_t dd = (wLast - wFirst >= 16384u) ? 1u : 0u;
        for (uint32_t w = wFirst; !dd && w <= wLast; ) {
            const uint32_t wm = w & 16383u, n = 32u - (wm & 31u), left = wLast - w + 1u, take = n < left ? n : left;
            const uint32_t bits = sh.dirty[wm >> 5] >> (wm & 31u);
            dd = bits & (take >= 32u ? 0xFFFFFFFFu : ((1u << take) - 1u));
            w += take;
        }
        bad |= dd ? 1u : 0u;
#if defined(GEN_TIMELINE)
        tlDirty = dd;
#endif
    } else if (m != 0u && type != 0u) {
        const uint32_t nT = nR + bBefore;
        uint32_t q = ck.iPartS, rem = 0xFFFFFFFFu - q * nT;
        const uint32_t up = (uint32_t)(rem >= nT);
        q += up; rem -= up ? nT : 0u;
        const uint32_t lo = d.i1 * q;
        const uint32_t same = (uint32_t)(rem < nT) & (uint32_t)(d.xPick < 0xFFFFFFFFu - rem) & (uint32_t)(d.xPick >= lo) & (uint32_t)(d.xPick - lo < q) & (uint32_t)(!(d.pick && d.i1 >= nR));
        const uint32_t nSp = d.pick ? nS : 0u;
        moved = (uint32_t)((uint64_t)nR >= (uint64_t)(GEN_MOVED_PICK_ATOMS_PER_ERASED) * (uint64_t)m) & (same ^ 1u) & (uint32_t)(bad == 0u) & (nSp ^ 1u);
        bad |= ((same ^ 1u) & (moved ^ 1u)) | nSp;
        light |= moved;
#if defined(GEN_TIMELINE)
        tlSame = same; tlQ = q; tlRem = rem;
#endif
    }
    const bool ok = !(d.go != 0u && (bad | light) != 0u);
    const uint32_t level = d.go == 0u ? 0u : (bad ? 2u : (light && (d.pick || moved) ? 1u : (light ? 2u : 0u)));
#if defined(GEN_TIMELINE)
    if (d.go) {
        const uint32_t movedL = (!isB && m != 0u && type != 0u) ? (uint32_t)(((bad & 1u) != 0u) && !(d.redo) && !((reads ? (nA | cA) : 0u) & 1u)) : 0u;
        cg_atomic_add_u64(&g_ahead_why[0], 1ull);
        if (!ok) cg_atomic_add_u64(&g_ahead_why[1], 1ull);
        if (movedL | moved) cg_atomic_add_u64(&g_ahead_why[2], 1ull);
        if (d.pick && m != 0u && nS) cg_atomic_add_u64(&g_ahead_why[3], 1ull);
        if (reads && (nA | ((isB && d.v3 != CG_NONE) ? nB : 0u))) cg_atomic_add_u64(&g_ahead_why[4], 1ull);
        if (reads && (cA | ((d.pick && (type == 'M' || type == 'E')) ? cB : 0u))) cg_atomic_add_u64(&g_ahead_why[5], 1ull);
        if (isB && !ok && !d.redo && !(nA | cA)) cg_atomic_add_u64(&g_ahead_why[6], 1ull);
        if (d.redo) cg_atomic_add_u64(&g_ahead_why[7], 1ull);
    }
    if (level == 2u) {
        uint32_t cause = d.redo ? 64u : 0u;
        if (isB) {
            const uint32_t hasB = (uint32_t)(d.v3 != CG_NONE);
            const uint32_t ers = (nA & gen_note_get(sh.dErase, gen_note_pos<GEN_DIRTY_ERASE>(d.v2))) | (hasB & nB & gen_note_get(sh.dErase, gen_note_pos<GEN_DIRTY_ERASE>(d.v3)));
            if (tlDirty) cause |= 4u;
            if (ers) cause |= 2u; else if (nA | cA | (hasB & nB)) cause |= 1u;
        } else {
            if (d.pick && (nA & gen_note_get(sh.dErase, ck.eraseA))) cause |= 32u;
            if (tlSame == 0u) {
                uint32_t clear = 0u;
                if (!d.redo && tlQ != 0u && tlRem < nR + bBefore && d.xPick < 0xFFFFFFFFu - tlRem) {
                    const uint32_t iNew = d.xPick / tlQ;
                    clear = (uint32_t)(iNew < nR) & (gen_note_get(sh.dAtom, gen_note_pos<GEN_DIRTY_ATOMS>(~iNew)) ^ 1u);
                }
                cause |= clear ? 8u : 16u;
            } else if (d.pick && m != 0u && nS) cause |= 128u;
        }
        if (cause) cg_atomic_or_u32(&sh.rtCause, cause);
    }
    if (moved) cg_atomic_or_u32(&sh.rtCause, 256u);
#endif
#if defined(COGAPS_EMUL)
    if (d.go) cg_atomic_add_u64(&S.gs->prof[level == 0u ? 8 : (level == 1u ? 10 : 9)], 1ull);
#endif
    (void)ok;
    return level;
}
```

cogaps_amd/csrc/gen_handover_pass.h:

```cpp
            uint32_t unitAcc = 0;
            for (uint32_t base = 0; base < e_prevQ; base += HP_STRIDE) {
                const uint32_t q = base + (HP_LANE);
                bool have = (HP_MINE) && q < e_prevQ;
                if (HP_FETCH(base)) { chain_item_clear(it); if (have) chain_fetch(S, hot.queueRd, q, it, isSparse); }
                const GenNotePos nH1 = gen_note_pos<GEN_DIRTY_ATOMS>(it.h1), nHL = gen_note_pos<GEN_DIRTY_ATOMS>(it.hL), nHR = gen_note_pos<GEN_DIRTY_ATOMS>(it.hR),
                                 nH2 = gen_note_pos<GEN_DIRTY_ATOMS>(it.h2), nL2 = gen_note_pos<GEN_DIRTY_ATOMS>(it.l2), nIdx = gen_note_pos<GEN_DIRTY_ATOMS>(~it.idx),
                                 nC1 = gen_note_pos<GEN_DIRTY_CELLS>(it.cell1), nC2 = gen_note_pos<GEN_DIRTY_CELLS>(it.cell2);
                const unsigned long long *gr = hot.grans + (size_t)q * CHAIN_GRAN_STRIDE;
                unsigned long long g0 = 0ull, g1 = 0ull; uint32_t spins = 0;
                for (;;) {
                    if (have) { g0 = cg_load_l2_u64(&gr[0]); g1 = cg_load_l2_u64(&gr[1]); }
                    const bool ok = !have || ((uint32_t)(g0 >> 32) == tag && (uint32_t)(g1 >> 32) == tag);
                    if (cg_ballot(!ok) == 0ull) break;
                    if (cg_poll_expired(++spins)) { if (!ok) { have = false; S.queueUnits[q] = CHAIN_DROPPED_MARK(tag); } if ((t & 63u) == 0u) { gs->error = GAPS_ERR_SPIN; sh.spinFail = 1u; } break; }
                    cg_poll_pause();
                }
#if defined(GEN_TEST_SPIN_FAIL_EPOCH)
                if (cg_ballot(have && tag == (uint32_t)GEN_TEST_SPIN_FAIL_EPOCH && (q % 3u) == 1u) != 0ull) {
                    if (have && (q % 3u) == 1u) { have = false; S.queueUnits[q] = CHAIN_DROPPED_MARK(tag); }
                    if ((t & 63u) == 0u) { gs->error = GAPS_ERR_SPIN; sh.spinFail = 1u; }
                }
#endif
                GEN_TS(33);
                if (base == 0u) GEN_RT_AT(3, WIN);
                const uint32_t code = have ? ((uint32_t)g0 & 0xFFu) : CHAIN_NONE;
                if (have) unitAcc += ((uint32_t)g0 >> 8) << (it.sparse ? 5u : 0u);
                const bool er = have && code == CHAIN_ERASE, ap = have && code == CHAIN_APPLY;
                if (er) gen_mark_dirty(sh.dirty, it.cell1);
                if (ap && it.type == 'M') { gen_mark_dirty(sh.dirty, it.mb1); gen_mark_dirty(sh.dirty, it.mb2); }
                if (er || ap) {
                    gen_note_set(sh.dAtom, nH1);
                    if (it.hL != CG_NONE) gen_note_set(sh.dAtom, nHL);
                    if ((er || it.type == 'M') && it.hR != CG_NONE) gen_note_set(sh.dAtom, nHR);
                    if (ap && it.type == 'E') { gen_note_set(sh.dAtom, nH2); if (it.l2 != CG_NONE) gen_note_set(sh.dAtom, nL2); }
                    if (er) {
                        gen_note_set(sh.dAtom, nIdx);
                        gen_note_set(sh.dErase, gen_note_pos<GEN_DIRTY_ERASE>(it.h1));
                        if (it.hL != CG_NONE) gen_note_set(sh.dErase, gen_note_pos<GEN_DIRTY_ERASE>(it.hL));
                        if (it.hR != CG_NONE) gen_note_set(sh.dErase, gen_note_pos<GEN_DIRTY_ERASE>(it.hR));
                    }
                    if (ap || it.type == 'D') gen_note_set(sh.dCell, nC1);
                    if (ap && (it.type == 'M' || it.type == 'E')) gen_note_set(sh.dCell, nC2);
                }
                const unsigned long long em = cg_ballot(er);
                if (em) {
                    const uint32_t cntE = (uint32_t)cg_popc64(em);
                    uint32_t b0 = 0;
                    if ((t & 63u) == 0u) b0 = cg_atomic_add_u32(&sh.eraseN, cntE);
                    b0 = cg_wave_bcast_u32(b0, 0);
                    if (er) {
                        const uint32_t k = b0 + (uint32_t)cg_popc64(em & ((1ull << (t & 63u)) - 1ull));
                        const unsigned long long e = it.eraseEntry;
                        if (k < (uint32_t)FLUSH_MAX) sh.eraseTmp[k] = e;
                        if (k < eraseCap) eraseList[k] = e; else gs->error = GAPS_ERR_ERASE_CAP;
                    }
                }
                if (have) chain_apply(it, code, gm_u2f((uint32_t)g1));
#if defined(COGAPS_EMUL)
                if (have && base) cg_atomic_add_u64(&gs->prof[6], 1ull);
                if (have && HP_FETCH(0u)) cg_atomic_add_u64(&gs->prof[2], 1ull);
#endif
            }
            const uint32_t waveUnits = cg_wave_sum_u32(unitAcc);
            if ((t & 63u) == 0u && waveUnits) cg_atomic_add_u32(&sh.unitSum, waveUnits);
```

cogaps_amd/csrc/gen_kernel.h:

```cpp
#pragma once
#include "gaps_state.h"

#if defined(GEN_TIMELINE)
__device__ unsigned long long g_timeline[8 * 64];
#define GEN_TS(id) do { if ((t & 63u) == 0u && ts_n < 64u) { sh.ts[(t & ~63u) + ts_n] = ((unsigned long long)cg_clock() << 8) | (unsigned long long)(id); ++ts_n; } } while (0)
#define GEN_TS_DUMP_WAVE() do { if ((t & 63u) == 0u && ts_ok && (t >> 6) < 8u) { for (uint32_t i_ = 0; i_ < 64u; ++i_) g_timeline[(t & ~63u) + i_] = i_ < ts_n ? sh.ts[(t & ~63u) + i_] : 0ull; } } while (0)
#define GEN_TS_INIT() uint32_t ts_n = 0
#define GEN_TS_RESUME(k) ts_n = (k)
#define GEN_TS_ZERO(a, b) do { if ((t & 63u) == 0u) for (uint32_t i_ = (a); i_ < (b); ++i_) sh.ts[(t & ~63u) + i_] = 0ull; } while (0)
#define GEN_PIN(x) asm volatile("" : "+v"(x) :: "memory")
__device__ unsigned long long g_ahead_why[8];
__device__ unsigned long long g_chain_gen[8];
#define GEN_RT(i) do { if (t == 0u) sh.rt[(i)] = __builtin_amdgcn_s_memrealtime(); } while (0)
#define GEN_RT_AT(i, lane) do { if (t == (unsigned)(lane)) sh.rt[(i)] = __builtin_amdgcn_s_memrealtime(); } while (0)
#define GEN_LOG_N 65536
__device__ unsigned long long g_chain_log[GEN_LOG_N * 8]; __device__ unsigned int g_chain_log_n;
#define GEN_RT_DUMP() do { if (t == 0u && sh.rtOn) { for (int i_ = 0; i_ < 8; ++i_) g_chain_gen[i_] = sh.rt[i_]; } \
    if (t == 0u && sh.rtLog) { const unsigned int k_ = atomicAdd(&g_chain_log_n, 1u) % GEN_LOG_N; for (int i_ = 0; i_ < 6; ++i_) g_chain_log[k_ * 8 + i_] = sh.rt[i_]; \
        g_chain_log[k_ * 8 + 6] = sh.rtInfo; g_chain_log[k_ * 8 + 7] = (unsigned long long)roundNo | ((unsigned long long)sh.rtCause << 32); } } while (0)
#else
#define GEN_TS(id) do { } while (0)
#define GEN_TS_INIT() do { } while (0)
#define GEN_TS_RESUME(k) do { } while (0)
#define GEN_TS_ZERO(a, b) do { } while (0)
#define GEN_PIN(x) do { } while (0)
#define GEN_RT(i) do { } while (0)
#define GEN_RT_AT(i, lane) do { } while (0)
#define GEN_RT_DUMP() do { } while (0)
#define GEN_TS_DUMP_WAVE() do { } while (0)
#endif

#if defined(GEN_TIMELINE_ROUND2)
#define GEN_TS_ROUND_OK(r) ((r) == 2u)
#else
#define GEN_TS_ROUND_OK(r) true
#endif
#define GEN_T_NONE 0
#define GEN_F_INLINE 1u
#define GEN_F_FAIL 2u
#define GEN_F_HAZARD 4u
#define GEN_F_HASRIGHT 8u
#define GEN_F_APPLY 16u
#define GEN_F_HASLEFT 32u
#define GEN_F_NEWHEAD 64u
#define GEN_F_BINEMPTY 128u
#define GEN_F_WORDZERO 256u

#define GEN_STAMP_COMMITTED 0xFFFFFFull
#define GEN_TAB_BBITS (WIN <= 128 ? 9 : 10)
#define GEN_TAB_NB (1 << GEN_TAB_BBITS)
#ifndef GEN_LDS_ROUNDS_MAX
#define GEN_LDS_ROUNDS_MAX 3
#endif
#define GEN_LDS_ROUNDS_FIT (((4 * GEN_TAB_NB) * 7 * 10) / (31 * WIN * 10))
#define GEN_LDS_ROUNDS (GEN_LDS_ROUNDS_FIT >= GEN_LDS_ROUNDS_MAX ? GEN_LDS_ROUNDS_MAX : (GEN_LDS_ROUNDS_FIT < 1 ? 1 : GEN_LDS_ROUNDS_FIT))
#define GEN_K_ROW 0u
#define GEN_K_ATOM 1u
#define GEN_K_GAP 2u
#define GEN_K_INL 3u
#define GEN_GS_WORDS ((uint32_t)(offsetof(GenScalars, evalProps) / 4u + 2u))
#define GEN_GS_ERROR_WORD ((uint32_t)(offsetof(GenScalars, error) / 4u))
#ifndef FLUSH_MAX
#define FLUSH_MAX 64
#endif
#define CG_KEEP 0xFFFFFFFEu
#define GEN_CHAIN_THREADS 512

#define GEN_DIRTY_ATOMS 4096
#define GEN_DIRTY_CELLS 2048
#define GEN_DIRTY_ERASE 256
struct GenTabVal { uint32_t used, gap, inl, pad; };
struct GenTabKeys { uint32_t k[4]; };

template <int WIN>
struct GenShared {
    uint64_t cpos[WIN], pos[WIN];
    float u1[WIN], u2[WIN];
    uint8_t type[WIN];
    uint64_t seed[WIN];
    uint32_t info[WIN];
    uint16_t perm[WIN];
    unsigned long long mq[WIN / 64], mb[WIN / 64], md[WIN / 64];
    uint32_t wtotA[3][WIN / 64], wtotB[3][WIN / 64], wtot4[4][WIN / 64];
    uint64_t fpos[FLUSH_MAX], flpos[FLUSH_MAX], frpos[FLUSH_MAX]; float frmass[FLUSH_MAX]; uint32_t fh[FLUSH_MAX], fl[FLUSH_MAX], fr[FLUSH_MAX], fidx[FLUSH_MAX], fbin[FLUSH_MAX], fhead[FLUSH_MAX], vt[FLUSH_MAX], lowSlot[FLUSH_MAX], lowH[FLUSH_MAX];
    uint32_t nLow, newFront, flushM, flushBase, unitSum, frontPending;
    uint32_t freeTop[16];
#if defined(GEN_TIMELINE)
    unsigned long long ts[8 * 64];
    unsigned long long rt[8]; uint32_t rtOn, rtLog; unsigned long long rtInfo; uint32_t rtCause;
#endif
    alignas(16) uint32_t bkey[4 * GEN_TAB_NB];
    alignas(16) GenTabVal bval[4 * GEN_TAB_NB];
    float dpLo[WIN], dpHi[WIN];
    uint64_t jmul[WIN + 1], jinc[WIN + 1];
    GenScalars g;
    uint64_t qrngRound, batchEpoch;
    uint32_t roundNo, stopKey;
    uint32_t nR, minAtoms, processed, qlen, skip, remaining;
    uint32_t nWork, nBD, updBase; float u1c, u2c;
    unsigned long long eraseTmp[FLUSH_MAX]; uint32_t eraseN, specBad, spinFail;
    float dpWin[4 * WIN];
    uint32_t dirty[512];
    alignas(16) uint32_t dAtom[GEN_DIRTY_ATOMS]; uint32_t dCell[GEN_DIRTY_CELLS]; uint32_t dErase[GEN_DIRTY_ERASE]; uint32_t anyRedo;
};

CG_DEVICE uint32_t gen_bin_of(const SamplerDev &S, uint64_t pos)
{
    double e = (double)pos * S.invBinLen;
    uint32_t q = (e >= S.numBins) ? (uint32_t)S.numBins : (uint32_t)e;
    const uint64_t prod = (uint64_t)q * S.binLength;
    if (prod > pos) --q;
    else if (pos - prod >= S.binLength) ++q;
    return q;
}

CG_DEVICE uint32_t gen_div_k(const SamplerDev &S, uint32_t bin)
{
    uint32_t q = (uint32_t)((double)bin * S.invK);
    q += (uint32_t)(bin - q * S.K >= S.K);
    return q;
}

CG_DEVICE void bm_set(const SamplerDev &S, uint32_t bin)
{
    uint32_t w0 = bin >> 6, w1 = w0 >> 6, w2 = w1 >> 6;
    cg_atomic_or_u64(&S.bits0[w0], 1ull << (bin & 63));
    if (!((S.bits1[w1] >> (w0 & 63)) & 1ull)) cg_atomic_or_u64(&S.bits1[w1], 1ull << (w0 & 63));
    if (!((S.bits2[w2] >> (w1 & 63)) & 1ull)) cg_atomic_or_u64(&S.bits2[w2], 1ull << (w1 & 63));
}
CG_DEVICE void bm_clear(const SamplerDev &S, uint32_t bin)
{
    cg_atomic_and_u64(&S.bits0[bin >> 6], ~(1ull << (bin & 63)));
}
CG_DEVICE uint32_t bm_prev_flat(const unsigned long long *w, uint32_t i)
{
    uint32_t wi = i >> 6, bit = i & 63;
    unsigned long long m = bit ? (w[wi] & ((1ull << bit) - 1ull)) : 0ull;
    for (;;) {
        if (m) return (wi << 6) + 63u - (uint32_t)cg_clz64(m);
        if (wi == 0) return CG_NONE;
        --wi; m = w[wi];
    }
}
CG_DEVICE uint32_t bm_next_flat(const unsigned long long *w, uint32_t nw, uint32_t i)
{
    uint32_t wi = i >> 6, bit = i & 63;
    unsigned long long m = (bit == 63) ? 0ull : (w[wi] & ~((2ull << bit) - 1ull));
    for (;;) {
        if (m) return (wi << 6) + (uint32_t)cg_ctz64(m);
        ++wi; if (wi >= nw) return CG_NONE;
        m = w[wi];
    }
}
CG_DEVICE uint32_t bm_prev_l1(const SamplerDev &S, uint32_t i)
{
    uint32_t wi = i >> 6, bit = i & 63;
    unsigned long long m = bit ? (S.bits1[wi] & ((1ull << bit) - 1ull)) : 0ull;
    if (m) return (wi << 6) + 63u - (uint32_t)cg_clz64(m);
    uint32_t cur = wi;
    for (;;) {
        uint32_t p = bm_prev_flat(S.bits2, cur);
        if (p == CG_NONE) return CG_NONE;
        unsigned long long x = S.bits1[p];
        if (x) return (p << 6) + 63u - (uint32_t)cg_clz64(x);
        cur = p;
    }
}
CG_DEVICE uint32_t bm_next_l1(const SamplerDev &S, uint32_t i)
{
    uint32_t wi = i >> 6, bit = i & 63;
    unsigned long long m = (bit == 63) ? 0ull : (S.bits1[wi] & ~((2ull << bit) - 1ull));
    if (m) return (wi << 6) + (uint32_t)cg_ctz64(m);
    uint32_t cur = wi;
    for (;;) {
        uint32_t p = bm_next_flat(S.bits2, S.nWords2, cur);
        if (p == CG_NONE) return CG_NONE;
        unsigned long long x = S.bits1[p];
        if (x) return (p << 6) + (uint32_t)cg_ctz64(x);
        cur = p;
    }
}
CG_DEVICE uint32_t bm_prev_bin(const SamplerDev &S, uint32_t bin)
{
    uint32_t wi = bin >> 6, bit = bin & 63;
    unsigned long long m = bit ? (S.bits0[wi] & ((1ull << bit) - 1ull)) : 0ull;
    if (m) return (wi << 6) + 63u - (uint32_t)cg_clz64(m);
// ... 185 lines not shown
```

cogaps_amd/csrc/gen_populate.h:

```cpp
#pragma once

#include "gen_flush.h"
#include "gen_draw.h"
#include "gen_round.h"
#include "gen_chain_apply.h"

struct GenClockEnd {
    unsigned long long *slot; unsigned t;
    CG_DEVICE GenClockEnd(unsigned t_) : slot(nullptr), t(t_) {}
    CG_DEVICE ~GenClockEnd() { if (slot && (t & 63u) == 0u) cg_atomic_max_u64(slot, cg_realtime()); }
};
template <int WIN, bool ASYNC, bool CHAIN = false, int SP = -1>
CG_DEVICE void gen_body_sh(const SamplerDev CG_CONSTANT *sp, const GenHot hot, GenShared<WIN> &sh)
{
    GenClockEnd clockEnd(cg_tid());
    constexpr unsigned TPB = (unsigned)WIN + 64u;
    const unsigned t = cg_tid();
    const bool attempt = t < (unsigned)WIN, helper = t >= (unsigned)WIN && t < TPB, spare = t >= TPB, applier = CHAIN && !attempt;
    const unsigned ht = t - (unsigned)WIN, ta = attempt ? t : 0u;
    GenScalars *gs = hot.gs;

    GEN_TS_INIT(); GEN_TS(0); GEN_TS(0);
    GEN_RT(0);
    const uint64_t jm0 = hot.lcgMul[2u * ta], ji0 = hot.lcgInc[2u * ta];
    const uint64_t jm1 = hot.lcgMul[ta ? 2u * (ta - 1u) : 0u], ji1 = hot.lcgInc[ta ? 2u * (ta - 1u) : 0u];
    unsigned long long specE = (!CHAIN && helper && ht < (unsigned)FLUSH_MAX && ht < hot.eraseCap) ? hot.eraseList[ht] : 0ull;
    PropRec p0; p0.type = 0; p0.h1 = 0; p0.h2 = 0; p0.pos = 0; p0.curPos = 0; p0.r1 = 0; p0.c1 = 0; p0.r2 = 0; p0.c2 = 0; p0.m1 = 0.f; p0.m2 = 0.f; p0.old1 = 0.f; p0.old2 = 0.f;
    if (applier && ht < hot.queueCap) p0 = hot.queueRd[ht];

    uint32_t units = (!CHAIN && attempt && t < hot.queueCap) ? hot.queueUnits[t] : 0u;
    const uint64_t jmW = hot.lcgMul[2 * WIN], jiW = hot.lcgInc[2 * WIN];
    constexpr uint32_t GSW = (uint32_t)(sizeof(GenScalars) / 4u);
    static_assert(GSW <= 2u * TPB, "at most two words of GenScalars per lane");
    const uint32_t gword = (t < GSW) ? reinterpret_cast<const uint32_t *>(gs)[t] : 0u;
    const uint32_t gword2 = (t + TPB < GSW) ? reinterpret_cast<const uint32_t *>(gs)[t + TPB] : 0u;
    cg_sched_fence();
    GEN_TS(26);
    cg_const_lines lines;
    if (ASYNC) cg_const_warm_begin<sizeof(SamplerDev)>(sp, lines);
    {
        GenTabKeys none; none.k[0] = none.k[1] = none.k[2] = none.k[3] = GEN_TAB_EMPTY;
        static_assert(offsetof(GenShared<WIN>, bval) == offsetof(GenShared<WIN>, bkey) + 16u * (size_t)GEN_TAB_NB, "keys and value words are contiguous");
        constexpr uint32_t UNITS = 5u * (uint32_t)GEN_TAB_NB, ROUNDS = (UNITS + TPB - 1u) / TPB;
        GenTabKeys *tab = reinterpret_cast<GenTabKeys *>(&sh.bkey[0]) + t;
#pragma unroll
        for (uint32_t k = 0; k < ROUNDS; ++k) { if (!CHAIN && !spare && ((k + 1u) * TPB <= UNITS || t + k * TPB < UNITS)) tab[k * TPB] = none; }
        if (CHAIN) {
            static_assert(offsetof(GenShared<WIN>, dCell) == offsetof(GenShared<WIN>, dAtom) + 4u * (size_t)GEN_DIRTY_ATOMS
                          && offsetof(GenShared<WIN>, dErase) == offsetof(GenShared<WIN>, dCell) + 4u * (size_t)GEN_DIRTY_CELLS, "the note tables are contiguous");
            GenTabKeys *dt = reinterpret_cast<GenTabKeys *>(&sh.dAtom[0]);
            GenTabKeys zero; zero.k[0] = zero.k[1] = zero.k[2] = zero.k[3] = 0u;
            for (uint32_t i = t; i < (uint32_t)(GEN_DIRTY_ATOMS + GEN_DIRTY_CELLS + GEN_DIRTY_ERASE) / 4u; i += cg_bdim()) dt[i] = zero;
        }
    }
    GEN_TS(27);
    if (ASYNC) sp = cg_const_warm_end(sp, lines);
    const SamplerDev &S = *(const SamplerDev *)sp;
    const bool isSparse = SP < 0 ? S.sparse != 0u : SP != 0;
    GEN_TS(28);
    if (t < GSW) reinterpret_cast<uint32_t *>(&sh.g)[t] = gword;
    if (t + TPB < GSW) reinterpret_cast<uint32_t *>(&sh.g)[t + TPB] = gword2;
    if (t == 0) { sh.newFront = CG_KEEP; sh.unitSum = 0; sh.jmul[WIN] = jmW; sh.jinc[WIN] = jiW; if (CHAIN) { sh.eraseN = 0; sh.specBad = 0; sh.spinFail = 0; sh.anyRedo = 0; } }
    if (attempt) { sh.jmul[t] = jm0; sh.jinc[t] = ji0; }
    GEN_TS(29);
    cg_sync_lds();
    uint32_t e_m = CHAIN ? 0u : cg_uniform_u32(sh.g.eraseCount);
    const uint32_t e_n = cg_uniform_u32(sh.g.nAtoms), e_fc = cg_uniform_u32(sh.g.freeCount), e_prevQ = cg_uniform_u32(sh.g.qlen),
                   e_nDone = cg_uniform_u32(sh.g.nDone), e_nSteps = cg_uniform_u32(sh.g.nSteps);
    GEN_TS(1);
    const bool updateDone = e_nDone >= e_nSteps;
    uint64_t seedC = 0ull; bool dpStaged = false, trySpec = false, specDone = false; uint32_t dpBase = 0;
    GenSpec specKeep; specKeep.bBefore = 0; specKeep.dBefore = 0; specKeep.guess = 0; specKeep.active = 0; specKeep.u1 = 0.f; specKeep.u2 = 0.f; specKeep.go = 0; specKeep.ct = 0; specKeep.info = 0;
    specKeep.rng = 0; specKeep.pos = 0; specKeep.bin = 0; specKeep.r1 = 0; specKeep.c1 = 0;
    uint64_t epoch0 = 0;
    GenDraw drawKeep; gen_draw_clear(drawKeep);
    GenCheck checkKeep; checkKeep.atomA.a = checkKeep.atomA.b = checkKeep.atomB.a = checkKeep.atomB.b = checkKeep.slot.a = checkKeep.slot.b = 0u;
    checkKeep.cellA.a = checkKeep.cellA.b = checkKeep.cellB.a = checkKeep.cellB.b = checkKeep.eraseA.a = checkKeep.eraseA.b = 0u; checkKeep.iPartS = 1u;
    if (!CHAIN) {
        GEN_TS_ZERO(7u, 13u);
#if defined(GEN_TIMELINE)
        if (t == 0u) { sh.rtOn = 0u; sh.rtLog = 0u; sh.rtCause = 0u; }
#endif
        if (attempt) {
            if (t >= e_prevQ) units = 0;
            for (uint32_t q = t + WIN; q < e_prevQ; q += WIN) units += S.queueUnits[q];
            const uint32_t waveUnits = cg_wave_sum_u32(units);
            if ((t & 63u) == 0u && waveUnits) cg_atomic_add_u32(&sh.unitSum, waveUnits);
        }
    } else {
        unsigned long long *const eraseList = S.eraseList; const uint32_t eraseCap = S.eraseCap;
        GEN_TS(30);
        GEN_RT(1);
#if defined(GEN_TIMELINE)
        if (t == 0u) { sh.rtOn = (e_prevQ >= 140u && e_nSteps - e_nDone >= 512u) ? 1u : 0u; sh.rt[6] = 0ull; sh.rt[7] = 0ull; sh.rtCause = 0u; sh.rtLog = (WIN == 256 && e_prevQ >= 100u && e_nSteps - e_nDone >= 512u) ? 1u : 0u; }
#endif
#if defined(GEN_TEST_APPLIER_LANES)
        const uint32_t NA = (uint32_t)GEN_TEST_APPLIER_LANES, al = t - (uint32_t)WIN;
        const bool applying = applier && al < NA;
#else
        const uint32_t NA = cg_bdim() - (uint32_t)WIN, al = t - (uint32_t)WIN;
        const bool applying = applier;
#endif
        const bool have0 = applying && al < e_prevQ;
#if defined(GEN_TEST_APPLIER_LANES)
        constexpr bool ATTEMPTS_APPLY = SP == 1;
#else
        constexpr bool ATTEMPTS_APPLY = SP == 1 && 2 * WIN >= GEN_CHAIN_THREADS;
#endif
        const uint32_t passLanes = ATTEMPTS_APPLY ? NA + (uint32_t)WIN : NA;
        ChainMid mid0; mid0.l2 = CG_NONE; mid0.head1 = CG_NONE; mid0.b1 = 0; mid0.b2 = 0; mid0.x1 = 0ull; mid0.x2 = 0ull;
        mid0.a.pos = 0; mid0.a.lpos = 0; mid0.a.rpos = 0; mid0.a.left = CG_NONE; mid0.a.right = CG_NONE; mid0.a.mass = 0.f; mid0.a.rmass = 0.f; mid0.a.idx = 0; mid0.a.pad0 = 0;
        const uint32_t freeTopAhead = (helper && ht < 16u && ht < e_fc) ? S.freeHandles[e_fc - 1u - ht] : CG_NONE;
        if (applier) mid0 = chain_fetch_mid(S, p0, isSparse);
        if (!updateDone && attempt) seedC = S.seeds[e_nDone + t < e_nSteps ? e_nDone + t : e_nSteps - 1u];
        const uint32_t span = e_prevQ + (uint32_t)(WIN - 1);
        dpBase = e_n > span ? e_n - span : 0u;
        const uint32_t dpCnt = e_n + (uint32_t)WIN - dpBase;
        dpStaged = !updateDone && dpCnt <= 4u * (uint32_t)WIN;
        const uint32_t nLo = e_n > e_prevQ ? e_n - e_prevQ : 0u, nHi = e_n;
        trySpec = dpStaged && nLo >= 2u;
        float dpw[4] = {0.f, 0.f, 0.f, 0.f};
        if (dpStaged && !spare) {
#pragma unroll
            for (uint32_t k = 0; k < 4u; ++k) { const uint32_t i = t + k * TPB; dpw[k] = S.deathProb[dpBase + (i < dpCnt ? i : dpCnt - 1u)]; }
        }
        cg_sched_fence();
        GEN_TS(31);
        GenRoundCtx rcS; GenSpec spS;
        rcS.t = t; rcS.jm0 = jm0; rcS.ji0 = ji0; rcS.jm1 = jm1; rcS.ji1 = ji1; rcS.seed1 = 0ull; rcS.g_qrng = sh.g.qrng; rcS.g_skip = sh.g.useCached ? 1u : 0u;
        rcS.g_u1 = sh.g.u1; rcS.g_u2 = sh.g.u2; rcS.remaining = e_nSteps - e_nDone; rcS.K = S.K; rcS.sparse = isSparse ? 1u : 0u;
        spS.bBefore = 0; spS.dBefore = 0; spS.guess = 0; spS.active = 0; spS.u1 = 0.f; spS.u2 = 0.f; spS.go = 0; spS.ct = 0; spS.info = 0; spS.rng = 0; spS.pos = 0; spS.bin = 0; spS.r1 = 0; spS.c1 = 0;
        if (trySpec && attempt) {
            const float dpAtLo = gm_death_prob((double)(uint64_t)nLo, S.domainLenD, S.alphaD, S.numBins), dpAtHi = gm_death_prob((double)(uint64_t)nHi, S.domainLenD, S.alphaD, S.numBins);
            gen_spec_a1<WIN>(S, sh, rcS, nLo, nHi, dpAtLo, dpAtHi, spS);
        } else if (trySpec) cg_sync_lds();
        if (trySpec) { for (uint32_t i = t; i < 512u; i += cg_bdim()) sh.dirty[i] = 0u; }
        if (dpStaged && !spare) {
#pragma unroll
            for (uint32_t k = 0; k < 4u; ++k) { const uint32_t i = t + k * TPB; if (i < dpCnt) sh.dpWin[i] = dpw[k]; }
        }
        ChainItem it; chain_item_clear(it);
        if (trySpec) {
            if (attempt && spS.guess != (uint32_t)GEN_T_NONE) sh.seed[t] = seedC;
            cg_sync_lds();
            if (attempt) gen_spec_slot<WIN>(S, sh, rcS, spS);
        }
        const bool drawAhead = trySpec && cg_uniform_u32(sh.specBad) == 0u;
        if (have0) chain_fetch_build(S, p0, mid0, it, isSparse);
        if (helper && ht < 16u) sh.freeTop[ht] = freeTopAhead;
        GEN_TS(32);
        epoch0 = sh.g.batchEpoch;
        const uint32_t tag = (uint32_t)epoch0;
        if (S.launchClock) clockEnd.slot = S.launchClock + 2u * (tag % GAPS_CLOCK_RING) + 1u;
#if defined(COGAPS_EMUL)
        if (t == 0 && e_prevQ) cg_atomic_add_u64(&gs->prof[13], 1ull);
#endif
        if (attempt) {
#if !defined(EXP_NO_AHEAD)
            if (drawAhead) {
                const uint32_t typeS = spS.info & 0xFFu;
                gen_draw_a<WIN, true, true>(S, rcS, &spS, spS.go != 0u, typeS, spS.info >> 8, spS.rng, e_n, drawKeep);
                gen_draw_b<WIN, true>(S, sh, rcS, typeS, drawKeep, [&]() {});
            }
#endif
            if (drawAhead) checkKeep = gen_draw_check(spS, drawKeep, e_n, rcS.K);
            GEN_PIN(drawKeep.flags); GEN_PIN(drawKeep.old1); GEN_PIN(drawKeep.old2);
            GEN_TS(36);
            GEN_RT(2);
            if constexpr (ATTEMPTS_APPLY) {
#define HP_STRIDE passLanes
#define HP_LANE (NA + t)
#define HP_MINE true
#define HP_FETCH(b) true
#include "gen_handover_pass.h"
#undef HP_STRIDE
#undef HP_LANE
#undef HP_MINE
#undef HP_FETCH
            }
        } else {
            {
                GenTabKeys none; none.k[0] = none.k[1] = none.k[2] = none.k[3] = GEN_TAB_EMPTY;
                constexpr uint32_t UNITS = 5u * (uint32_t)GEN_TAB_NB;
                GenTabKeys *tab = reinterpret_cast<GenTabKeys *>(&sh.bkey[0]);
                const uint32_t nAll = cg_bdim() - (uint32_t)WIN;
#pragma unroll 4
                for (uint32_t i = t - (uint32_t)WIN; i < UNITS; i += nAll) tab[i] = none;
            }
#define HP_STRIDE passLanes
#define HP_LANE al
#define HP_MINE applying
#define HP_FETCH(b) (b)
#include "gen_handover_pass.h"
#undef HP_STRIDE
#undef HP_LANE
#undef HP_MINE
#undef HP_FETCH
        }
        GEN_TS(34);
        if (drawAhead) cg_sync_lds(); else cg_sync();
        GEN_TS(35);
        GEN_RT(4);
        const uint32_t sfRaw = sh.spinFail, emRaw = sh.eraseN;
        if (cg_uniform_u32(sfRaw) != 0u) {
            if (t == 0u) { gs->applyCount = e_prevQ; gs->savedErase = emRaw; gs->qlen = 0u; gs->nSteps = e_nDone; ChainSlot cs; cs.qlen = 0u; cs.tag = tag + 1u; *hot.slotWr = cs; }
            return;
        }
        if (spare) {
            if (drawAhead && !updateDone) { cg_sync_lds(); cg_sync(); }
            { const bool ts_ok = e_prevQ >= 140u && e_nSteps - e_nDone >= 512u; (void)ts_ok; GEN_TS_DUMP_WAVE(); }
            return;
        }
        e_m = cg_uniform_u32(emRaw);
        if (e_m > eraseCap) e_m = eraseCap;
        if (helper) specE = (ht < (unsigned)FLUSH_MAX && ht < e_m) ? sh.eraseTmp[ht] : 0ull;
        specDone = drawAhead;
#if defined(GEN_TIMELINE)
        if (t == 0u) sh.rtInfo = (unsigned long long)e_prevQ | ((unsigned long long)e_m << 16) | ((unsigned long long)(specDone ? 1u : 0u) << 32);
#endif
#if defined(COGAPS_EMUL)
        if (t == 0 && !updateDone) cg_atomic_add_u64(&gs->prof[specDone ? 12 : 11], 1ull);
#endif
        if (specDone) specKeep = spS;
    }
    if (updateDone) {
        if (!CHAIN) cg_sync_lds();
        if (!helper) return;
        GenFlushRegs fr;
        gen_flush_fetch<WIN>(S, fr, ht, e_m, e_n, specE, e_fc);
        if (ht == 0) { sh.flushM = 0; sh.flushBase = e_fc; sh.nLow = 0; }
        cg_wave_sync();
        for (int part = 0; part < 4; ++part) { gen_flush_part<WIN>(S, sh, fr, ht, e_m, e_n, e_fc, part); cg_wave_sync(); }
        if (ht == 0) { gs->nAtoms = sh.g.nAtoms; gs->front = sh.g.front; gs->freeCount = sh.g.freeCount; gs->eraseCount = 0; gs->qlen = 0; gs->batchNproc = 0; gs->updateFlushed = 1;
                       gs->evalBytes = sh.g.evalBytes + (unsigned long long)sh.unitSum * S.unitBytes; gs->evalProps = sh.g.evalProps + e_prevQ;
                       if (CHAIN) { ChainSlot cs; cs.qlen = 0; cs.tag = (uint32_t)sh.g.batchEpoch; *hot.slotWr = cs; } }
        return;
    }
    if (helper) { gen_helper<WIN>(S, sh, gs, ht, specE, e_m, e_n, e_fc, e_prevQ, e_nDone, e_nSteps, CHAIN ? hot.slotWr : nullptr, CHAIN && specDone); return; }

    const uint64_t seed1 = CHAIN ? seedC : ((e_nDone + t < e_nSteps) ? S.seeds[e_nDone + t] : 0ull);
    const uint32_t n0 = e_n - e_m;
    const bool fromWin = CHAIN && dpStaged;
    float tabHi = 0.f, tabLo = 0.f, dp0 = 0.f;
    if (!(CHAIN && specDone)) {
        tabHi = fromWin ? sh.dpWin[n0 + t - dpBase] : S.deathProb[n0 + t]; tabLo = (n0 >= t) ? (fromWin ? sh.dpWin[n0 - t - dpBase] : S.deathProb[n0 - t]) : 0.f;
        dp0 = fromWin ? sh.dpWin[n0 - dpBase] : gm_death_prob((double)(uint64_t)n0, S.domainLenD, S.alphaD, S.numBins);
    }
    const uint64_t batchEpoch = (CHAIN ? epoch0 : sh.g.batchEpoch) + 1;
    const uint32_t updBase = e_nDone;
// ... 68 lines not shown
```

cogaps_amd/csrc/gen_round.h:

```cpp
#pragma once
template <int WIN, bool FIRST, bool SPEC = false, bool AHEAD = false>
CG_DEVICE bool gen_round(const SamplerDev &S, GenShared<WIN> &sh, const GenRoundCtx &c, const uint32_t roundNo, const GenSpec *spec = nullptr, const GenDraw *ahead = nullptr, const bool aheadValid = true, const bool keepPick = false, const bool movedPick = false)
{
    static_assert(FIRST || !SPEC, "only a batch's first window is classified ahead of the decisions");
    static_assert(SPEC || !AHEAD, "only a window classified ahead is drawn ahead");
    const unsigned t = c.t;
    const uint64_t jm0 = c.jm0, ji0 = c.ji0, jm1 = c.jm1, ji1 = c.ji1, seed1 = c.seed1, batchEpoch = c.batchEpoch;
    const uint32_t updBase = c.updBase, remaining = c.remaining, K = c.K;
    GenScalars *gs = c.gs;
    constexpr bool first = FIRST;
    GEN_TS_INIT(); GEN_TS_RESUME(FIRST ? (AHEAD ? 16u : 13u) : 40u);
    GEN_TS(4);
    const uint32_t nR = first ? c.n0 : sh.nR, minR = first ? c.n0 : sh.minAtoms, skip = first ? c.g_skip : sh.skip, processed = first ? 0u : sh.processed;
    const uint64_t qrngRound = first ? c.g_qrng : sh.qrngRound;
    const float u1c = first ? c.g_u1 : sh.u1c, u2c = first ? c.g_u2 : sh.u2c;
    const float dpLo0 = first ? c.dp0 : sh.dpLo[0], dpHi0 = first ? c.dp0 : sh.dpHi[0];
    const uint32_t left_ = remaining - processed;
    const uint32_t winN = left_ < (uint32_t)WIN ? left_ : (uint32_t)WIN;

    uint32_t bBeforeA1 = 0, dBeforeA1 = 0, guessA1 = 0, activeA1 = 0; float u1A1 = 0.f, u2A1 = 0.f;
    if (SPEC) { bBeforeA1 = spec->bBefore; dBeforeA1 = spec->dBefore; guessA1 = spec->guess; activeA1 = spec->active; u1A1 = spec->u1; u2A1 = spec->u2; }
    else {
        const uint32_t active = t < winN;
        const uint32_t tt = active ? t : 0u;
// ... 3 lines not shown
        const uint32_t cached = (skip != 0u) & (uint32_t)(t == 0u);
        u1 = cached ? u1c : u1; u2 = cached ? u2c : u2;
        uint32_t guess = gen_decide(u1, u2, minR, nR, dpLo0, dpHi0);
        guess = active ? guess : (uint32_t)GEN_T_NONE;
        GEN_PIN(guess); GEN_PIN(u1); GEN_PIN(u2);
        GEN_TS(5);
        sh.u1[t] = u1; sh.u2[t] = u2;
        if (first) { sh.dpHi[t] = c.tabHi; sh.dpLo[t] = c.tabLo; }
        uint32_t eX[4], tX[4];
        gen_count4<WIN>(sh.wtot4, t, guess == 'B', guess == 'D', guess == 'M', guess == 'E', eX, tX);
        GEN_TS(6);
        bBeforeA1 = eX[0]; dBeforeA1 = eX[1]; u1A1 = u1; u2A1 = u2; guessA1 = guess; activeA1 = active;
        const uint32_t go = (uint32_t)(guess != GEN_T_NONE);
        const uint32_t k0 = (uint32_t)(guess == 'B') | (uint32_t)(guess == 'D'), k1 = (uint32_t)(guess == 'M');
        const uint32_t T0 = tX[0] + tX[1], T1 = tX[2], T2 = tX[3];
        if (go) {
            uint32_t slot = T0 + T1 + eX[3];
            slot = k1 ? T0 + eX[2] : slot;
            slot = k0 ? eX[0] + eX[1] : slot;
            sh.perm[slot] = (uint16_t)t;
            sh.info[t] = guess | (eX[0] << 8);
            sh.seed[t] = mySeed;
        }
        GEN_TS(8);
        if (t == 0) sh.nWork = T0 + T1 + T2;
    }
    if (!SPEC) cg_sync_lds();
    GEN_TS(9);

    const bool go = SPEC ? spec->go != 0u : t < sh.nWork;
    const uint32_t ct = SPEC ? spec->ct : (go ? (uint32_t)sh.perm[t] : 0u);
    const uint32_t info = SPEC ? spec->info : (go ? sh.info[ct] : 0u);
    const uint32_t type = info & 0xFFu, bBefore = info >> 8;
    auto exactDecide = [&]() {
        const float dpLoX = SPEC ? (nR >= dBeforeA1 ? sh.dpWin[nR - dBeforeA1 - c.dpBase] : 0.f) : sh.dpLo[dBeforeA1];
        const float dpHiX = SPEC ? sh.dpWin[nR + bBeforeA1 - c.dpBase] : sh.dpHi[bBeforeA1];
        const uint32_t exact = gen_decide(u1A1, u2A1, (uint64_t)minR - dBeforeA1, (uint64_t)nR + bBeforeA1, dpLoX, dpHiX);
        const uint32_t hazA = activeA1 & (uint32_t)(exact != guessA1);
        const uint32_t failA = activeA1 & (hazA ^ 1u) & (uint32_t)(guessA1 == GEN_T_NONE);
        if (hazA | failA) cg_atomic_min_u32(&sh.stopKey, 2u * t + (hazA ^ 1u));
        GEN_TS(7);
    };
    GenDraw d;
    if (AHEAD) {
        d = *ahead;
        if (d.isB) d.i1 = nR + bBefore;
#if !defined(EXP_NO_REDO)
        const bool again = go && !aheadValid;
        if (cg_ballot(again) != 0ull) {
            const bool soft = again && keepPick && movedPick;
            GenDraw r; gen_draw_a<WIN, SPEC>(S, c, spec, again, type, bBefore, SPEC ? spec->rng : 0ull, nR, r);
            gen_draw_b<WIN, false>(S, sh, c, type, r, [&]() {}, (keepPick && !movedPick) ? ahead->h1 : CG_NONE, soft);
            if (cg_ballot(soft) != 0ull) {
                uint32_t cut = (soft && r.redo) ? 1u : 0u;
                if (soft && r.pick) cut |= gen_note_get(sh.dAtom, gen_note_pos<GEN_DIRTY_ATOMS>(~r.i1)) | gen_note_get(sh.dErase, gen_note_pos<GEN_DIRTY_ERASE>(r.h1));
#if defined(GEN_TEST_MOVED_PICK_FLAG_EVERY)
                if (soft && ((ct + (uint32_t)batchEpoch) % (uint32_t)GEN_TEST_MOVED_PICK_FLAG_EVERY) == 0u) cut = 1u;
#endif
                if (cut) r.flags |= GEN_F_HAZARD;
#if defined(GEN_TIMELINE)
                if (cut) cg_atomic_or_u32(&sh.rtCause, 512u);
#endif
#if defined(COGAPS_EMUL)
                if (soft) cg_atomic_add_u64(&gs->prof[cut ? 3 : 1], 1ull);
#endif
            }
            if (again) d = r;
        }
#endif
        exactDecide();
    } else {
        gen_draw_a<WIN, SPEC>(S, c, spec, go, type, bBefore, SPEC ? spec->rng : (go ? pcg_from_seed(sh.seed[ct]) : 0ull), nR, d);
        GEN_PIN(d.i1); GEN_PIN(d.bin); GEN_PIN(d.pos);
        GEN_TS(10);
        if (FIRST) cg_sync();
        GEN_TS(25);
        gen_draw_b<WIN, false>(S, sh, c, type, d, exactDecide);
    }
    uint32_t flags = d.flags;
    const bool isB = d.isB, pick = d.pick;
    const uint64_t rng = d.rng, pos = d.pos, cpos = d.cpos;
    uint32_t h1 = d.h1, h2 = d.h2, i1 = d.i1, i2 = CG_NONE; const uint32_t hl = d.hl, hr = d.hr;
    const uint32_t r1 = d.r1, c1 = d.c1, r2 = d.r2, c2 = d.c2, bin = d.bin; const float nm1 = d.nm1, nm2 = d.nm2;
    const float old1 = d.old1, old2 = d.old2, m2x = d.m2x; const uint32_t gib1 = d.gib1, gib2 = d.gib2;
    const uint64_t lposB = d.lposB, rposB = d.rposB; const float rmassB = d.rmassB;
    struct { float mass; } a; a.mass = d.amass;
    (void)isB; (void)pick;
    GEN_TS(14);

    const bool live = go && !(flags & GEN_F_FAIL);
    const bool queuedM = live && type == 'M' && !(flags & GEN_F_INLINE);
    const bool ldsRound = FIRST || roundNo <= (uint32_t)GEN_LDS_ROUNDS;
#if defined(COGAPS_EMUL)
    if (!FIRST && t == 0) cg_atomic_add_u64(&gs->prof[ldsRound ? 14 : 15], 1ull);
#endif
    const uint32_t gord = processed + ct;
    uint32_t rs0 = 0, rs1 = 0, rs2 = 0, rf0 = 0, rf1 = 0, rf2 = 0;
    uint64_t d9 = 0, d10 = 0;
    if (!FIRST && ldsRound && live && type == 'B') { d9 = (hl != CG_NONE) ? S.atomDest[hl] : 0ull; d10 = (hr != CG_NONE) ? S.atomDest[hr] : 0ull; }
    if (go) { sh.cpos[ct] = cpos; sh.pos[ct] = pos; sh.type[ct] = queuedM ? (uint8_t)'M' : (uint8_t)0; }
    if (live && ldsRound) {
        const uint32_t inl = flags & GEN_F_INLINE, tB = type == 'B', tD = type == 'D', tM = type == 'M';
        const uint32_t k0 = inl ? h1 : (GEN_TAB_ROW | r1), f0 = inl << 1;
        const uint32_t use1 = 1u ^ (inl & tM), use2 = tM & (inl ^ 1u);
        const uint32_t hlKey = (hl == CG_NONE) ? GEN_TAB_FRONT : hl;
        uint32_t k1 = GEN_TAB_ROW | r2;
        k1 = tD ? h1 : k1;
        k1 = tB ? hlKey : k1;
        k1 = inl ? h2 : k1;
        k1 = use1 ? k1 : k0;
        uint32_t f1 = inl ? 2u : tB; f1 = use1 ? f1 : f0;
        const uint32_t k2 = use2 ? h1 : k0, f2 = use2 ? 0u : f0;
        const uint32_t hh0 = gen_tab_hash(k0), hh1 = gen_tab_hash(k1), hh2 = gen_tab_hash(k2);
        uint32_t b0 = gen_tab_bucket<WIN>(hh0), b1_ = gen_tab_bucket<WIN>(hh1), b2_ = gen_tab_bucket<WIN>(hh2);
        const uint32_t j0 = gen_tab_start<WIN>(hh0), j1 = gen_tab_start<WIN>(hh1), j2 = gen_tab_start<WIN>(hh2);
        uint32_t s0 = 0, s1 = 0, s2 = 0, d0 = 0, d1 = 0, d2 = 0;
        for (uint32_t i = 0; ; ++i) {
            const uint32_t p0 = d0 ? s0 : 4u * b0 + ((j0 + i) & 3u), p1 = d1 ? s1 : 4u * b1_ + ((j1 + i) & 3u), p2 = d2 ? s2 : 4u * b2_ + ((j2 + i) & 3u);
            const uint32_t o0 = cg_atomic_cas_u32(&sh.bkey[p0], GEN_TAB_EMPTY, k0);
            const uint32_t o1 = cg_atomic_cas_u32(&sh.bkey[p1], GEN_TAB_EMPTY, k1);
            const uint32_t o2 = cg_atomic_cas_u32(&sh.bkey[p2], GEN_TAB_EMPTY, k2);
            s0 = p0; s1 = p1; s2 = p2;
            d0 |= (uint32_t)(o0 == GEN_TAB_EMPTY) | (uint32_t)(o0 == k0);
            d1 |= (uint32_t)(o1 == GEN_TAB_EMPTY) | (uint32_t)(o1 == k1);
            d2 |= (uint32_t)(o2 == GEN_TAB_EMPTY) | (uint32_t)(o2 == k2);
            if (d0 & d1 & d2) break;
            const uint32_t wrap = (i & 3u) == 3u;
            b0 = (b0 + wrap) & (uint32_t)(GEN_TAB_NB - 1); b1_ = (b1_ + wrap) & (uint32_t)(GEN_TAB_NB - 1); b2_ = (b2_ + wrap) & (uint32_t)(GEN_TAB_NB - 1);
        }
        uint32_t *words = &sh.bval[0].used;
        cg_atomic_min_u32(&words[4u * s0 + f0], gord);
        cg_atomic_min_u32(&words[4u * s1 + f1], gord);
        cg_atomic_min_u32(&words[4u * s2 + f2], gord);
        rs0 = s0; rs1 = s1; rs2 = s2; rf0 = f0; rf1 = f1; rf2 = f2;
    } else if (live) {
        uint32_t rk[3], rid[3]; int nk = 0;
        const bool inl = (flags & GEN_F_INLINE) != 0;
        if (type == 'B') { rk[0] = GEN_K_ROW; rid[0] = r1; rk[1] = GEN_K_GAP; rid[1] = (hl == CG_NONE) ? 0u : hl + 1u; nk = 2; }
        else if (type == 'D') { rk[0] = GEN_K_ROW; rid[0] = r1; rk[1] = GEN_K_ATOM; rid[1] = h1; nk = 2; }
        else if (type == 'M') {
            if (inl) { rk[0] = GEN_K_INL; rid[0] = h1; nk = 1; }
            else { rk[0] = GEN_K_ROW; rid[0] = r1; rk[1] = GEN_K_ROW; rid[1] = r2; rk[2] = GEN_K_ATOM; rid[2] = h1; nk = 3; }
        } else {
            if (inl) { rk[0] = GEN_K_INL; rid[0] = h1; rk[1] = GEN_K_INL; rid[1] = h2; nk = 2; }
            else { rk[0] = GEN_K_ROW; rid[0] = r1; rk[1] = GEN_K_ROW; rid[1] = r2; nk = 2; }
        }
        const unsigned long long st = gen_stamp(batchEpoch, roundNo, ct);
        for (int k = 0; k < nk; ++k) cg_atomic_max_u64(gen_stamp_ptr(S, rk[k], rid[k]), st);
    }
    GEN_TS(15);
    if (ldsRound) cg_sync_lds(); else cg_sync();
    GEN_TS(16);

    if (live && ldsRound) {
        const uint32_t tB = type == 'B', tM = type == 'M', tE = type == 'E', inl = flags & GEN_F_INLINE;
        const uint32_t hasL = hl != CG_NONE, hasR = hr != CG_NONE, noRight = (flags & GEN_F_HASRIGHT) == 0u;
        uint32_t key[6], use[6];
        key[0] = GEN_TAB_ROW | r1; use[0] = 1u;
        key[1] = GEN_TAB_ROW | r2; use[1] = tM | tE;
        key[2] = ((tM | tB) & hasL) ? hl : GEN_TAB_FRONT; use[2] = tM | tB | (tE & noRight);
        const uint32_t eInl = tE & (uint32_t)(inl != 0u);
        key[3] = eInl ? (hasL ? hl : GEN_TAB_FRONT) : hr; use[3] = ((tM | tB) & hasR) | eInl;
        const uint32_t tD = type == 'D';
        key[4] = h1; use[4] = tM | tE | tD;
        key[5] = h2; use[5] = tE;
        uint32_t bk[6]; GenTabKeys kq[6];
        for (int k = 0; k < 6; ++k) { bk[k] = gen_tab_bucket<WIN>(gen_tab_hash(key[k])); kq[k] = *(const GenTabKeys *)&sh.bkey[4u * bk[k]]; }
// ... 95 lines not shown
                else if (u == 2 && sh.type[ix] == 'M') { ma = sh.cpos[ix]; mb = sh.pos[ix]; mv = true; }
                if (mv) { const uint64_t lo = ma < mb ? ma : mb, hi = ma < mb ? mb : ma; if (lo < pos && pos < hi) fail = true; }
                if (res[6 + k] == 2) haz = true;
            }
        } else if (tM) {
            if (res[2] != 0 || res[3] != 0) fail = true;
            if (res[4] == 2 || res[5] == 2) fail = true;
            if (res[6] == 2 || res[7] == 2 || res[8] == 2) haz = true;
        } else if (tE) {
            if (res[4] == 2 || res[5] == 2) fail = true;
            if (res[6] == 2 || res[7] == 2) haz = true;
            if (res[9] == 2) haz = true;
        } else if (tD) {
            if (res[6] == 2) haz = true;
        }
        if (haz) flags |= GEN_F_HAZARD; else if (fail) flags |= GEN_F_FAIL;
    }
    GEN_TS(18);
    if (go && (flags & (GEN_F_HAZARD | GEN_F_FAIL))) cg_atomic_min_u32(&sh.stopKey, 2u * ct + ((flags & GEN_F_HAZARD) ? 0u : 1u));
    if (ldsRound) cg_sync_lds(); else cg_sync();
    GEN_TS(19);

    const uint32_t stopKey = sh.stopKey;
    const uint32_t stopT = (stopKey == 0xFFFFFFFFu) ? winN : (stopKey >> 1);
    const bool stopFail = (stopKey != 0xFFFFFFFFu) && (stopKey & 1u);
    const bool commit = go && ct < stopT;
    const bool queued = commit && (type == 'B' || type == 'D' || !(flags & GEN_F_INLINE));
    const uint32_t c_fc = sh.g.freeCount, c_handleHi = sh.g.handleHi, c_flushBase = sh.flushBase, c_flushM = sh.flushM, c_qlen = sh.qlen;
    const uint32_t c_traceOn = sh.g.traceOn, c_traceCount = sh.g.traceCount, c_traceCap = sh.g.traceCap, c_nBatches = sh.g.nBatches;
    const bool endB = stopFail || (processed + stopT >= remaining);
    if (commit) {
        const unsigned long long bit = 1ull << (ct & 63u);
        if (queued) cg_atomic_or_u64(&sh.mq[ct >> 6], bit);
        if (type == 'B') { cg_atomic_or_u64(&sh.mb[ct >> 6], bit); if (hl == CG_NONE) sh.frontPending = 1u; }
        if (type == 'D') cg_atomic_or_u64(&sh.md[ct >> 6], bit);
    }
    cg_sync_lds();
    GEN_TS(20);
    if (commit) {
        uint32_t qBefore = 0, bRank = 0;
        {
            const uint32_t wq = ct >> 6; const unsigned long long lt = (1ull << (ct & 63u)) - 1ull;
            for (uint32_t w = 0; w < wq; ++w) { qBefore += (uint32_t)cg_popc64(sh.mq[w]); bRank += (uint32_t)cg_popc64(sh.mb[w]); }
            qBefore += (uint32_t)cg_popc64(sh.mq[wq] & lt); bRank += (uint32_t)cg_popc64(sh.mb[wq] & lt);
        }
        const unsigned long long done = (batchEpoch << 24) | GEN_STAMP_COMMITTED;
        const bool more = !endB;
        if (type == 'B') {
            const uint32_t fc = c_fc;
            uint32_t hb;
            if (bRank < fc) { const uint32_t fi = fc - 1u - bRank; hb = (fi >= c_flushBase && fi - c_flushBase < c_flushM) ? sh.fh[fi - c_flushBase] : ((fi < c_flushBase && c_flushBase - 1u - fi < 16u) ? sh.freeTop[c_flushBase - 1u - fi] : S.freeHandles[fi]); }
            else hb = c_handleHi + (bRank - fc);
            const uint32_t idx = nR + bRank;
            if (hb >= S.atomCap || idx >= S.atomCap) { gs->error = GAPS_ERR_ATOM_CAP; hb = 0; }
            S.vec[idx] = hb;
            AtomRec n; n.pos = pos; n.lpos = lposB; n.rpos = rposB; n.left = hl; n.right = hr; n.mass = 0.f; n.rmass = rmassB; n.idx = idx; n.pad0 = 0;
            S.atoms[hb] = n;
            h1 = hb;
            if (hl != CG_NONE) { S.atoms[hl].right = hb; S.atoms[hl].rpos = pos; S.atoms[hl].rmass = 0.f; } else { sh.g.front = hb; if (endB) gs->front = hb; }
            if (hr != CG_NONE) { S.atoms[hr].left = hb; S.atoms[hr].lpos = pos; }
            if (flags & GEN_F_NEWHEAD) S.binHead[bin] = hb;
            if (flags & GEN_F_BINEMPTY) {
                cg_atomic_or_u64(&S.bits0[bin >> 6], 1ull << (bin & 63u));
                if (flags & GEN_F_WORDZERO) { const uint32_t wa = bin >> 6, wb = wa >> 6, wc = wb >> 6; cg_atomic_or_u64(&S.bits1[wb], 1ull << (wa & 63u)); cg_atomic_or_u64(&S.bits2[wc], 1ull << (wb & 63u)); }
            }
            if (more) { S.rowStamp[r1] = done; S.atomStamp[hb] = done; S.atomDest[hb] = 0ull; }
        } else if (type == 'D') {
            if (more) { S.rowStamp[r1] = done; S.atomStamp[h1] = done; S.atomDest[h1] = 0ull; }
        } else if (type == 'M') {
            if (flags & GEN_F_INLINE) atom_set_pos(S, h1, hl, hr, pos);
            else if (more) { S.rowStamp[r1] = done; S.rowStamp[r2] = done; S.atomStamp[h1] = done; S.atomDest[h1] = pos; }
        } else {
            if (flags & GEN_F_INLINE) { if (flags & GEN_F_APPLY) { atom_set_mass(S, h1, hl, nm1); atom_set_mass(S, h2, (hr != CG_NONE) ? h1 : CG_NONE, nm2); } }
            else if (more) { S.rowStamp[r1] = done; S.rowStamp[r2] = done; }
        }
        if (queued) {
            const uint32_t slot = c_qlen + qBefore;
            if (slot >= S.queueCap) gs->error = GAPS_ERR_QUEUE_CAP;
            else {
                if (c_traceOn && type == 'E') i2 = S.atoms[h2].idx;
                PropRec p; p.pos = (type == 'M') ? pos : 0ull; p.rng = rng; p.h1 = h1; p.h2 = h2; p.i1 = i1; p.i2 = i2;
                p.r1 = r1; p.c1 = c1; p.r2 = r2; p.c2 = c2; p.type = type; p.batch = 0; p.pad[0] = p.pad[1] = p.pad[2] = 0;
                const bool two = type == 'M' || type == 'E';
                p.gibbs = (gib1 > 0u ? 1u : 0u) | ((two && gib2 > 0u) ? 2u : 0u);
                p.m1 = (type == 'B') ? 0.f : a.mass; p.m2 = (type == 'E') ? m2x : 0.f;
                p.old1 = old1; p.old2 = two ? old2 : 0.f; p.curPos = (type == 'M') ? cpos : 0ull;
                c.queueOut[slot] = p;
                if (c_traceOn) { const uint32_t ti = c_traceCount + slot; if (ti < c_traceCap) { p.batch = c_nBatches; S.trace[ti] = p; } }
            }
        }
    }
    if (!endB && ldsRound) {
        if (live) {
            uint32_t *words = &sh.bval[0].used;
            const bool behind = !(ct < stopT);
            if (rf0 != 0u || behind) cg_atomic_cas_u32(&words[4u * rs0 + rf0], gord, GEN_TAB_EMPTY);
            if (rf1 != 0u || behind) cg_atomic_cas_u32(&words[4u * rs1 + rf1], gord, GEN_TAB_EMPTY);
            if (rf2 != 0u || behind) cg_atomic_cas_u32(&words[4u * rs2 + rf2], gord, GEN_TAB_EMPTY);
        }
        if (commit && type == 'B' && roundNo + 1u <= (uint32_t)GEN_LDS_ROUNDS) {
            const uint32_t sb = gen_tab_claim<WIN>(sh, h1);
            cg_atomic_min_u32(&sh.bval[sb].used, gord);
        }
    }
    GEN_TS(21);
    if (endB) { GEN_TS(22); GEN_RT(5); GEN_RT_DUMP(); { const bool ts_ok = c.e_prevQ >= 140u && c.remaining >= 512u && GEN_TS_ROUND_OK(roundNo); (void)ts_ok; GEN_TS_DUMP_WAVE(); } }
    return endB;
}
```

cogaps_amd/csrc/sparse_kernels.h:

```cpp
#pragma once
#include "eval_kernel.h"
#include "aux_kernels.h"

#define SP_KMAX 512
#define SP_GROUP_THREADS 256u
#define SP_CHAIN_GROUPS(WIDE) ((WIDE) ? 1u : 2u)
CG_DEVICE uint32_t sp_tid() { return cg_tid() & (SP_GROUP_THREADS - 1u); }
CG_DEVICE uint32_t sp_grp() { return cg_tid() / SP_GROUP_THREADS; }

CG_DEVICE float sp_dot(const float *a, const float *b, uint32_t n)
{
    float d = 0.f;
    if (n <= 25u) { for (uint32_t i = n; i-- > 0u;) d = d + a[i] * b[i]; }
    else { for (uint32_t i = 0; i < n; ++i) d = d + a[i] * b[i]; }
    return d;
}

struct SpRow { cg_f4 r[16]; };
CG_DEVICE void sp_row_load(SpRow &R, const float *row, uint32_t n)
{
    const uint32_t nq = cg_fresh_u32((n + 3u) >> 2);
#pragma unroll
    for (uint32_t c = 0; c < 16u; ++c) R.r[c] = c < nq ? ld4(row, c) : f4_zero();
}
// ... 457 lines not shown
        float s = s0, m = m0;
        for (uint32_t i = 0; i < total; ++i) { s = s + sc[i]; m = m + sc[S.Npad + i]; if (MODE == SP_MODE_CH) m = m + sc[2u * S.Npad + i]; }
        bc[0] = s; bc[1] = m;
        visited += total;
    }
    cg_sync();
    sOut = bc[0]; mOut = bc[1];
    cg_sync();
}

struct SpCell { float colv; bool flagged; };
CG_DEVICE SpCell sp_cell_load(const SamplerDev &S, uint32_t row, uint32_t col)
{
    SpCell c;
    c.colv = S.mat[(size_t)col * S.Mpad + row];
    c.flagged = ((S.mflags[(size_t)col * S.Mw + (row >> 6)] >> (row & 63u)) & 1ull) != 0ull;
    return c;
}
CG_DEVICE void sp_store_col(const SamplerDev &S, uint32_t row, uint32_t col, float newCol, bool zero, bool wasFlagged)
{
    unsigned long long *f = S.mflags + (size_t)col * S.Mw + (row >> 6);
    const unsigned long long bit = 1ull << (row & 63u);
    if (zero) {
        if (wasFlagged) { (void)cg_atomic_and_u64(f, ~bit); (void)cg_atomic_sub_u32(&S.colPos[col], 1u); }
        S.mat[(size_t)col * S.Mpad + row] = 0.f;
    } else {
        if (!wasFlagged) { (void)cg_atomic_or_u64(f, bit); (void)cg_atomic_add_u32(&S.colPos[col], 1u); }
        S.mat[(size_t)col * S.Mpad + row] = newCol;
    }
}
CG_DEVICE void sp_change_matrix(const SamplerDev &S, uint32_t row, uint32_t col, float oldRow, float delta, const SpCell &cell)
{
    S.rows[(size_t)row * S.Kpad + col] = oldRow + delta;
    const bool zero = cell.colv + delta < GAPS_EPSILON;
    sp_store_col(S, row, col, cell.colv + delta, zero, cell.flagged);
}
CG_DEVICE void sp_safely_change_matrix(const SamplerDev &S, uint32_t row, uint32_t col, float oldRow, float delta, const SpCell &cell)
{
    const float newVal = gm_max(oldRow + delta, 0.f);
    S.rows[(size_t)row * S.Kpad + col] = newVal;
    sp_store_col(S, row, col, newVal, newVal < GAPS_EPSILON, cell.flagged);
}

template <bool SEQ, bool WIDE>
struct SpShared {
    float lds[16 * 4];
    float arowA[SP_KMAX], arowB[SP_KMAX];
    float z2A[SP_KMAX], z2B[SP_KMAX];
    float decf; uint32_t deci;
    uint32_t nzShared;
    uint32_t seqCnt[SEQ ? SP_SEQ_WORDS + 1 : 1]; float seqBc[2];
    SpBal<(WIDE ? SP_BAL_CAP_WIDE : SP_BAL_CAP)> bal;
};
template <bool SEQ, bool WIDE, bool CHAIN>
CG_DEVICE void eval_sparse_body_sh(const SamplerDev &S, const uint32_t vbid, const uint32_t vgdim, const EvalHot hot, const EvalFirst &first, SpShared<SEQ, WIDE> &sm)
{
    PropRec pNext = first.p;
    const uint32_t qlen = first.qlen;
    const float T = first.T;
    float (&lds)[16 * 4] = sm.lds;
    float (&arowA)[SP_KMAX] = sm.arowA; float (&arowB)[SP_KMAX] = sm.arowB; float (&z2A)[SP_KMAX] = sm.z2A; float (&z2B)[SP_KMAX] = sm.z2B;
    float &decf = sm.decf; uint32_t &deci = sm.deci; uint32_t &nzShared = sm.nzShared;
    uint32_t (&seqCnt)[SEQ ? SP_SEQ_WORDS + 1 : 1] = sm.seqCnt; float (&seqBc)[2] = sm.seqBc;
    SpBal<(WIDE ? SP_BAL_CAP_WIDE : SP_BAL_CAP)> &bal = sm.bal;
    const uint32_t mm = SEQ ? S.mathMode : GM_MATH_PORTABLE;
    const uint32_t t = sp_tid(), BS = S.spW, K = S.K;
    const float lambda = S.lambda, beta = S.beta;
    const bool multiWave = BS > 64u;
    const bool scalarLane = !multiWave || t < 64u;
#if defined(GEN_TIMELINE)
    unsigned long long ets[11]; uint32_t ets_n = 0;
#endif
    EVAL_TS(0);
    for (uint32_t q = vbid; ; q += vgdim) {
        const PropRec p = pNext;
        if (q >= qlen) break;
        EVAL_TS(1);
#if defined(COGAPS_EMUL)
        if (CHAIN && t == 0u && sp_grp() != 0u) cg_atomic_add_u64(&S.gs->prof[4], 1ull);
#endif
        uint64_t rng = p.rng;
        const EvalAtoms ea = eval_atoms_load(S, p, !CHAIN && t == 0u);
        const bool two = (p.type == 'M' || p.type == 'E');
        const float m1 = p.m1, m2 = p.m2, old1 = p.old1, old2 = p.old2;
        const bool gibbs1 = (p.gibbs & 1u) != 0u, gibbs2 = (p.gibbs & 2u) != 0u;
        const bool need = (p.type == 'B') ? gibbs1 : ((p.type == 'D' || p.type == 'M') ? true : (gibbs1 || gibbs2));
        const bool diff = two && p.r1 != p.r2;
        float s = 0.f, smu = 0.f;
        uint32_t nz = 0;
        if (t == 0) nzShared = 0u;
        SpCell cell1, cell2; cell1.colv = 0.f; cell1.flagged = false; cell2 = cell1;
        if (!CHAIN && t == 0u) { cell1 = sp_cell_load(S, p.r1, p.c1); if (two) cell2 = sp_cell_load(S, p.r2, p.c2); }
        const float z1a = need ? S.Z1[p.c1] : 0.f, z1b = (need && two) ? S.Z1[p.c2] : 0.f;
        SpPre preA, preB; preA.dfl = preA.fv = 0ull; preA.dbase = 0u; preB = preA;
        if (!SEQ && need) { preA = sp_preload(S, p.r1, p.c1, p.c2, two && !diff); if (diff) preB = sp_preload(S, p.r2, p.c2, 0u, false); }
        if (need) {
            for (uint32_t k = t; k < S.Kpad; k += BS) {
                arowA[k] = S.rows[(size_t)p.r1 * S.Kpad + k];
                if (diff) arowB[k] = S.rows[(size_t)p.r2 * S.Kpad + k];
                if (k < K) { z2A[k] = S.Z2[(size_t)p.c1 * K + k]; if (two) z2B[k] = S.Z2[(size_t)p.c2 * K + k]; }
            }
            cg_sync();
            EVAL_TS(2);
            if (SEQ) {
                uint32_t vis = 0;
                if (diff) {
                    float sa, ma, sb, mb;
                    sp_alpha_seq<SP_MODE_ONE>(S, p.r1, p.c1, 0u, 0.f, arowA, z1a, -1.f * sp_dot(arowA, z2A, K), seqCnt, seqBc, sa, ma, vis);
                    sp_alpha_seq<SP_MODE_ONE>(S, p.r2, p.c2, 0u, 0.f, arowB, z1b, -1.f * sp_dot(arowB, z2B, K), seqCnt, seqBc, sb, mb, vis);
                    sa = sa * beta; ma = ma * beta; sb = sb * beta; mb = mb * beta;
                    s = sa + sb; smu = ma - mb;
                } else if (two) {
                    const float s0 = z1a - 2.f * z2B[p.c1] + z1b;
                    float d0 = 0.f;
                    for (uint32_t k = 0; k < K; ++k) d0 += arowA[k] * (z2A[k] - z2B[k]);
                    sp_alpha_seq<SP_MODE_SAME>(S, p.r1, p.c1, p.c2, 0.f, arowA, s0, -1.f * d0, seqCnt, seqBc, s, smu, vis);
                    s = s * beta; smu = smu * beta;
                } else if (p.type == 'D') {
                    const float ch = -1.f * m1;
                    float m0 = -1.f * sp_dot(arowA, z2A, K);
                    m0 -= ch * z2A[p.c1];
                    sp_alpha_seq<SP_MODE_CH>(S, p.r1, p.c1, 0u, ch, arowA, z1a, m0, seqCnt, seqBc, s, smu, vis);
                    s = s * beta; smu = smu * beta;
                } else {
                    sp_alpha_seq<SP_MODE_ONE>(S, p.r1, p.c1, 0u, 0.f, arowA, z1a, -1.f * sp_dot(arowA, z2A, K), seqCnt, seqBc, s, smu, vis);
                    s = s * beta; smu = smu * beta;
                }
                if (t == 0) nzShared = vis;
            } else {
            float x[4] = {0.f, 0.f, 0.f, 0.f};
            if (diff) {
                if (!WIDE && S.Wn <= BS) sp_partial_pair(S, p.r1, p.c1, arowA, preA, p.r2, p.c2, arowB, preB, bal, x, nz);
                else if (WIDE) sp_partial_merged_pair(S, p.r1, p.c1, arowA, preA, p.r2, p.c2, arowB, preB, bal, x, nz);
                else { sp_partial_balanced<SP_MODE_ONE, WIDE>(S, p.r1, p.c1, 0u, 0.f, arowA, bal, preA, x[0], x[1], nz); sp_partial_balanced<SP_MODE_ONE, WIDE>(S, p.r2, p.c2, 0u, 0.f, arowB, bal, preB, x[2], x[3], nz); }
            }
            else if (p.type == 'D') sp_partial_balanced<SP_MODE_CH, WIDE>(S, p.r1, p.c1, 0u, -1.f * m1, arowA, bal, preA, x[0], x[1], nz);
            else if (two) sp_partial_balanced<SP_MODE_SAME, WIDE>(S, p.r1, p.c1, p.c2, 0.f, arowA, bal, preA, x[0], x[1], nz);
            else sp_partial_balanced<SP_MODE_ONE, WIDE>(S, p.r1, p.c1, 0u, 0.f, arowA, bal, preA, x[0], x[1], nz);
            EVAL_TS(3);
            { const uint32_t waveNz = cg_wave_sum_u32(nz); if ((t & 63u) == 0u && waveNz) cg_atomic_add_u32(&nzShared, waveNz); }
#pragma unroll
            for (int c = 0; c < 4; ++c) x[c] = cg_wave_allsum_f32(x[c]);
            float tot[4] = {x[0], x[1], x[2], x[3]};
            if (multiWave) {
                if ((t & 63u) == 0) { for (int c = 0; c < 4; ++c) lds[(t >> 6) * 4 + c] = x[c]; }
                cg_sync();
                eval_vfinish<4, 1>(lds, tot, BS >> 6, t);
            }
            EVAL_TS(4);
            if (scalarLane) {
                if (diff) {
                    const float sa = (z1a + tot[0]) * beta, ma = (-1.f * sp_dot(arowA, z2A, K) + tot[1]) * beta;
                    const float sb = (z1b + tot[2]) * beta, mb = (-1.f * sp_dot(arowB, z2B, K) + tot[3]) * beta;
                    s = sa + sb; smu = ma - mb;
                } else if (two) {
                    float s0 = z1a - 2.f * z2B[p.c1] + z1b;
                    float d0 = 0.f;
                    for (uint32_t k = 0; k < K; ++k) d0 += arowA[k] * (z2A[k] - z2B[k]);
                    float m0 = -1.f * d0;
                    s = (s0 + tot[0]) * beta; smu = (m0 + tot[1]) * beta;
                } else {
                    float m0 = -1.f * sp_dot(arowA, z2A, K);
                    if (p.type == 'D') m0 -= (-1.f * m1) * z2A[p.c1];
                    s = (z1a + tot[0]) * beta; smu = (m0 + tot[1]) * beta;
                }
            }
            }
        }
        EVAL_PIN(s); EVAL_TS(5);
        s = s * T; smu = smu * T;
        const bool writer = !CHAIN && t == 0u;
        uint32_t bytes = 0;
        if (t == 0u && need) bytes = (diff ? 2u : 1u) * (16u * S.Wn + 8u * K) + ((two && !diff) ? 8u * S.Wn : 0u) + nzShared * (8u + 4u * K);
#define SP_PUBLISH(CODE, VAL) do { if (CHAIN && t == 0u) { unsigned long long *gr_ = hot.grans + (size_t)q * CHAIN_GRAN_STRIDE; \
        cg_store_agent_u64(&gr_[0], ((unsigned long long)first.tag << 32) | (unsigned long long)((CODE) | (((bytes + 16u) >> 5) << 8))); \
        cg_store_agent_u64(&gr_[1], ((unsigned long long)first.tag << 32) | (unsigned long long)gm_f2u(VAL)); } } while (0)
#define SP_BCAST(F0, I0) do { if (multiWave && !CHAIN) { if (t == 0) { decf = (F0); deci = (I0); } cg_sync(); (F0) = decf; (I0) = deci; } } while (0)
        if (p.type == 'B') {
            float bv = 0.f; uint32_t bhas = 0;
            if (scalarLane) {
                if (gibbs1) { OptF g = gm_gibbs_mass(s, smu, 0.f, S.maxGibbsMass, rng, S.luts, true, lambda); bv = g.v; bhas = g.has ? 1u : 0u; }
                else { bv = pcg_exponential(rng, lambda, mm); bhas = 1u; }
                if (bhas != 0u && bv >= GAPS_EPSILON) SP_PUBLISH(CHAIN_APPLY, bv); else SP_PUBLISH(CHAIN_ERASE, 0.f);
            }
            SP_BCAST(bv, bhas);
            if (bhas != 0u && bv >= GAPS_EPSILON) {
                if (writer) { atom_set_mass(S, p.h1, ea.a1.left, bv); sp_change_matrix(S, p.r1, p.c1, old1, bv, cell1); }
            } else if (writer) eval_cache_erase(S, p.h1, p.r1, p.c1);
        } else if (p.type == 'D') {
            float rebirth = m1; uint32_t acc = 0;
            if (scalarLane) {
                if (gibbs1) { OptF g = gm_gibbs_mass(s, smu, 0.f, S.maxGibbsMass, rng, S.luts, true, lambda); if (g.has) rebirth = g.v; }
                const float deltaLL = rebirth * (smu - s * rebirth / 2.f);
                acc = (gm_logf_m(pcg_uniform(rng), mm) < deltaLL) ? 1u : 0u;
                if (acc != 0u) { if (rebirth != m1) SP_PUBLISH(CHAIN_APPLY, rebirth); else SP_PUBLISH(CHAIN_NONE, 0.f); } else SP_PUBLISH(CHAIN_ERASE, 0.f);
            }
            SP_BCAST(rebirth, acc);
            if (writer) {
                if (acc != 0u) { if (rebirth != m1) { sp_safely_change_matrix(S, p.r1, p.c1, old1, rebirth - m1, cell1); atom_set_mass(S, p.h1, ea.a1.left, rebirth); } }
                else { sp_safely_change_matrix(S, p.r1, p.c1, old1, -1.f * m1, cell1); eval_cache_erase(S, p.h1, p.r1, p.c1); }
            }
        } else if (p.type == 'M') {
            uint32_t acc = 0; float unused = 0.f;
            if (scalarLane) { const float deltaLL = -1.f * m1 * (smu + s * m1 / 2.f); acc = (gm_logf_m(pcg_uniform(rng), mm) < deltaLL) ? 1u : 0u;
                              if (acc) SP_PUBLISH(CHAIN_APPLY, 0.f); else SP_PUBLISH(CHAIN_NONE, 0.f); }
            SP_BCAST(unused, acc);
            if (acc && writer) {
                eval_domain_move(S, p, ea.a1);
                sp_safely_change_matrix(S, p.r1, p.c1, old1, -m1, cell1);
                sp_change_matrix(S, p.r2, p.c2, old2, m1, cell2);
            }
        } else if (need) {
            float gv = 0.f; uint32_t gh = 0;
            if (scalarLane) { OptF g0 = gm_gibbs_mass(s, smu, -m1, m2, rng, S.luts, false, 0.f); gv = g0.v; gh = g0.has ? 1u : 0u;
                              if (gh != 0u && m1 + gv > GAPS_EPSILON && m2 - gv > GAPS_EPSILON) SP_PUBLISH(CHAIN_APPLY, gv); else SP_PUBLISH(CHAIN_NONE, 0.f); }
            SP_BCAST(gv, gh);
            const float n1 = m1 + gv, n2 = m2 - gv;
            if (gh != 0u && n1 > GAPS_EPSILON && n2 > GAPS_EPSILON && writer) {
                sp_safely_change_matrix(S, p.r1, p.c1, old1, n1 - m1, cell1);
                sp_safely_change_matrix(S, p.r2, p.c2, old2, n2 - m2, cell2);
                atom_set_mass(S, p.h1, ea.a1.left, n1); atom_set_mass(S, p.h2, ea.left2, n2);
            }
        }
        else SP_PUBLISH(CHAIN_NONE, 0.f);
        EVAL_TS(6);
#if defined(GEN_TIMELINE)
        if (cg_bid() < 16u && (t & 63u) == 0u && ((t >> 6) == 0u || (t >> 6) == ((BS - 1u) >> 6)) && qlen >= 20u) {
            unsigned long long *o_ = &g_eval_timeline[((S.N > 4096u ? 16u : 0u) * 2u + cg_bid() * 2u + ((t >> 6) ? 1u : 0u)) * 12u];
            o_[0] = (unsigned long long)(p.type | ((need ? 1u : 0u) << 8) | ((p.r1 == p.r2 ? 1u : 0u) << 16));
            for (uint32_t i_ = 0; i_ < 11u; ++i_) o_[1 + i_] = i_ < ets_n ? ets[i_] : 0ull;
        }
#endif
        if (writer) S.queueUnits[q] = bytes;
        if (q + vgdim >= qlen) break;
        { const uint32_t qn_ = q + vgdim; pNext = hot.queue[qn_ < hot.queueCap ? qn_ : 0u]; }
        cg_sync();
    }
}
template <bool SEQ, bool WIDE>
CG_DEVICE void eval_sparse_body(const SamplerDev &S, const uint32_t vbid, const uint32_t vgdim, const EvalHot hot, const EvalFirst &first)
{
    CG_SHARED SpShared<SEQ, WIDE> sm;
    eval_sparse_body_sh<SEQ, WIDE, false>(S, vbid, vgdim, hot, first, sm);
}
CG_KERNEL void CG_LAUNCH_BOUNDS(256) eval_sparse_kernel(const PropRec *hotQueue, const GenScalars *hotGs, uint32_t hotCap, const SamplerDev CG_CONSTANT *sp)
{
    EvalHot hot; hot.queue = hotQueue; hot.gs = hotGs; hot.queueCap = hotCap; hot.slot = nullptr; hot.grans = nullptr;
    const EvalFirst first = eval_first<EVAL_FUSED>(hot, 1u, cg_bid());
    const SamplerDev &S = eval_record<EVAL_FUSED>(sp);
    eval_sparse_body<false, false>(S, cg_bid(), cg_gdim(), hot, first);
}
// ... 218 lines not shown
```

Measured before the change: 8.186 million.

## Read old cell values and gibbs flags at eval time instead of at proposal generation

```diff
diff --git a/cogaps_amd/csrc/eval_kernel.h b/cogaps_amd/csrc/eval_kernel.h
--- a/cogaps_amd/csrc/eval_kernel.h
+++ b/cogaps_amd/csrc/eval_kernel.h
@@ -67,13 +67,28 @@
     else tot[0] = x;
 }
 
-struct EvalSpec { uint64_t rng; uint32_t n, mm; float l1, l2; };
+struct EvalSpec { uint64_t rng; uint32_t n, mm; float l1, l2;
+                  uint32_t want; const float *cellA, *cellB; const uint32_t *cntA, *cntB; float old1, old2; uint32_t gib1, gib2; };
 CG_DEVICE void eval_spec_run(EvalSpec &sp)
 {
     uint64_t r = sp.rng;
     sp.l1 = gm_logf_m(pcg_uniform(r), sp.mm);
     if (sp.n > 1u) sp.l2 = gm_logf_m(pcg_uniform(r), sp.mm);
     sp.n = 0u;
+}
+CG_DEVICE void eval_cells_want(const SamplerDev &S, const PropRec &p, const bool want, const bool sparse, EvalSpec &sp)
+{
+    const bool two = p.type == 'M' || p.type == 'E';
+    const uint32_t r2 = two ? p.r2 : p.r1, c2 = two ? p.c2 : p.c1;
+    sp.cellA = sparse ? &S.rows[(size_t)p.r1 * S.Kpad + p.c1] : &S.mat[(size_t)p.c1 * S.Mpad + p.r1];
+    sp.cellB = sparse ? &S.rows[(size_t)r2 * S.Kpad + c2] : &S.mat[(size_t)c2 * S.Mpad + r2];
+    sp.cntA = &S.otherColPos[p.c1]; sp.cntB = &S.otherColPos[c2];
+    sp.old1 = 0.f; sp.old2 = 0.f; sp.gib1 = 0u; sp.gib2 = 0u; sp.want = want ? 1u : 0u;
+}
+CG_DEVICE void eval_cells_issue(EvalSpec &sp)
+{
+    sp.old1 = *sp.cellA; sp.old2 = *sp.cellB; sp.gib1 = *sp.cntA; sp.gib2 = *sp.cntB;
+    sp.want = 0u;
 }
 template <int NR, int MODE>
 CG_DEVICE void eval_alpha(const SamplerDev &S, const uint32_t (&row)[NR], const uint32_t (&col)[NR], uint32_t col2, float ch, uint32_t chunk0, uint32_t stride, float *lds, float (&tot)[2 * NR], EvalSpec &spec EVAL_TS_PARAMS)
@@ -93,6 +108,7 @@
             const float *Vr = S.other + (size_t)col[r] * S.Npad, *V2 = S.other + (size_t)col2 * S.Npad;
             v[r] = ld4(Vr, j); d[r] = ld4_stream(Dr, j); if (!S.defaultS) s[r] = ld4_stream(Sr, j); p[r] = ld4(Ar, j); if (MODE == EVAL_MODE_SAME) w2 = ld4(V2, j);
         }
+        if (spec.want) eval_cells_issue(spec);
         if (spec.n) { cg_sched_fence(); eval_spec_run(spec); cg_sched_fence(); }
         if (S.defaultS) {
 #pragma unroll
@@ -346,6 +362,7 @@
         }
         w2[sl] = (MODE == EVAL_MODE_SAME) ? ld4(S.other + (size_t)col2 * S.Npad, jj) : f4_zero();
     }
+    if (spec.want) eval_cells_issue(spec);
     if (spec.n) { cg_sched_fence(); eval_spec_run(spec); cg_sched_fence(); }
 #pragma unroll
     for (int sl = 0; sl < 2; ++sl) {
@@ -422,15 +439,13 @@
     const bool scalarLane = u < 64u;
     uint64_t rng = p.rng;
     const bool two = (p.type == 'M' || p.type == 'E');
-    const float m1 = p.m1, m2 = p.m2, old1 = p.old1, old2 = p.old2;
-    const bool gibbs1 = (p.gibbs & 1u) != 0u, gibbs2 = (p.gibbs & 2u) != 0u;
-    const bool need = (p.type == 'B') ? gibbs1 : ((p.type == 'D' || p.type == 'M') ? true : (gibbs1 || gibbs2));
+    const float m1 = p.m1, m2 = p.m2;
     const bool diff = two && p.r1 != p.r2;
-    const uint32_t alphaUnits = need ? (!two ? 4u : (diff ? 8u : 5u)) : 0u;
     EvalSpec spec; spec.rng = rng; spec.mm = mm; spec.l1 = 0.f; spec.l2 = 0.f;
-    spec.n = (scalarLane && need && (p.type == 'D' || p.type == 'M')) ? ((p.type == 'D' && gibbs1) ? 2u : 1u) : 0u;
+    spec.n = (scalarLane && (p.type == 'D' || p.type == 'M')) ? (p.type == 'D' ? 2u : 1u) : 0u;
+    eval_cells_want(S, p, scalarLane, false, spec);
     float *lds = &ldsP[h][0];
-    if (need) {
+    {
         const uint32_t rowA[1] = {p.r1}, colA[1] = {p.c1};
         if (diff) { const uint32_t rowAB[2] = {p.r1, p.r2}, colAB[2] = {p.c1, p.c2}; eval_pair_alpha<2, EVAL_MODE_ONE>(S, rowAB, colAB, 0u, 0.f, u, H, lds, spec); }
         else if (p.type == 'D') eval_pair_alpha<1, EVAL_MODE_CH>(S, rowA, colA, 0u, -1.f * m1, u, H, lds, spec);
@@ -439,11 +454,16 @@
     }
     cg_sync();
     float s = 0.f, smu = 0.f;
-    if (need) {
+    {
         if (diff) { float tot[4] = {0.f, 0.f, 0.f, 0.f}; eval_pair_fold<4>(lds, u, nwH, tot); s = tot[0] + tot[2]; smu = tot[1] - tot[3]; }
         else { float t2[2] = {0.f, 0.f}; eval_pair_fold<2>(lds, u, nwH, t2); s = t2[0]; smu = t2[1]; }
         if (spec.n) eval_spec_run(spec);
     }
+    const float old1 = spec.old1, old2 = spec.old2;
+    const bool gibbs1 = spec.gib1 > 0u, gibbs2 = two && spec.gib2 > 0u;
+    const bool need = (p.type == 'B') ? gibbs1 : ((p.type == 'D' || p.type == 'M') ? true : (gibbs1 || gibbs2));
+    const uint32_t alphaUnits = need ? (!two ? 4u : (diff ? 8u : 5u)) : 0u;
+    if (!need) { s = 0.f; smu = 0.f; }
     s = s * T; smu = smu * T;
     DecRec owe; owe.n = 0; owe.r1 = 0; owe.c1 = 0; owe.d1 = 0.f; owe.r2 = 0; owe.c2 = 0; owe.d2 = 0.f; owe.pad = 0;
     if (scalarLane) {
@@ -520,6 +540,7 @@
     sp = cg_const_warm_end(sp, lines);
     return *(const SamplerDev *)sp;
 }
+#define CHAIN_DELTA_GRAN(q) ((size_t)(q) * 64u + 60u)
 CG_DEVICE void eval_chain_updates(const SamplerDev &S, const EvalHot hot, const uint32_t tag, const uint32_t qlen, const uint32_t wg, const uint32_t nwg)
 {
     const uint32_t TPB = cg_bdim(), nq = S.Npad >> 2;
@@ -539,17 +560,25 @@
         }
         if (!have) return;
         const uint32_t code = (uint32_t)g0 & 0xFFu; const float val = gm_u2f((uint32_t)g1);
-        const float m1 = p.m1, m2 = p.m2, old1 = p.old1, old2 = p.old2;
+        const bool owes = (code == CHAIN_APPLY && p.type != 'B') || (code == CHAIN_ERASE && p.type == 'D');
+        float d1 = val, d2 = 0.f;
+        if (owes) {
+            const unsigned long long *gd = S.grans + CHAIN_DELTA_GRAN(q);
+            unsigned long long h0 = 0ull, h1 = 0ull;
+            for (spins = 0;;) {
+                h0 = cg_load_l2_u64(&gd[0]); h1 = cg_load_l2_u64(&gd[1]);
+                const bool ok = (uint32_t)(h0 >> 32) == tag && (uint32_t)(h1 >> 32) == tag;
+                if (cg_ballot(!ok) == 0ull) break;
+                if (cg_poll_expired(++spins)) { if (cg_tid() == 0u) S.gs->error = GAPS_ERR_SPIN; have = false; break; }
+                cg_poll_pause();
+            }
+            if (!have) return;
+            d1 = gm_u2f((uint32_t)h0); d2 = gm_u2f((uint32_t)h1);
+        }
         if (code == CHAIN_APPLY) {
-            if (p.type == 'B') eval_update_ap(S, p.r1, p.c1, val, part * TPB, TPB * parts);
-            else if (p.type == 'D') { const float nv = gm_max(old1 + (val - m1), 0.f); eval_update_ap(S, p.r1, p.c1, nv - old1, part * TPB, TPB * parts); }
-            else if (p.type == 'M') { const float nv1 = gm_max(old1 + (-m1), 0.f); eval_update_ap2(S, p.r1, p.c1, nv1 - old1, p.r2, p.c2, m1, part * TPB, TPB * parts); }
-            else if (p.type == 'E') {
-                const float n1 = m1 + val, n2 = m2 - val;
-                const float nv1 = gm_max(old1 + (n1 - m1), 0.f), nv2 = gm_max(old2 + (n2 - m2), 0.f);
-                eval_update_ap2(S, p.r1, p.c1, nv1 - old1, p.r2, p.c2, nv2 - old2, part * TPB, TPB * parts);
-            }
-        } else if (code == CHAIN_ERASE && p.type == 'D') { const float nv = gm_max(old1 + (-1.f * m1), 0.f); eval_update_ap(S, p.r1, p.c1, nv - old1, part * TPB, TPB * parts); }
+            if (p.type == 'B' || p.type == 'D') eval_update_ap(S, p.r1, p.c1, d1, part * TPB, TPB * parts);
+            else if (p.type == 'M' || p.type == 'E') eval_update_ap2(S, p.r1, p.c1, d1, p.r2, p.c2, d2, part * TPB, TPB * parts);
+        } else if (code == CHAIN_ERASE && p.type == 'D') eval_update_ap(S, p.r1, p.c1, d1, part * TPB, TPB * parts);
     }
 }
 
@@ -622,19 +651,17 @@
 #endif
         bool eaLoaded = false;
         const bool two = (p.type == 'M' || p.type == 'E');
-        const float m1 = p.m1, m2 = p.m2, old1 = p.old1, old2 = p.old2;
-        const bool gibbs1 = (p.gibbs & 1u) != 0u, gibbs2 = (p.gibbs & 2u) != 0u;
+        const float m1 = p.m1, m2 = p.m2;
         EVAL_PROF(0);
         EVAL_TS(2);
 #if defined(GEN_PROFILE)
-        if (S.dbg & 1u) { if (p.type == 0xFFu || m1 == -1.f) S.queueUnits[q] = (uint32_t)old1; break; }
-#endif
-        bool need = (p.type == 'B') ? gibbs1 : ((p.type == 'D' || p.type == 'M') ? true : (gibbs1 || gibbs2));
+        if (S.dbg & 1u) { if (p.type == 0xFFu || m1 == -1.f) S.queueUnits[q] = (uint32_t)S.mat[(size_t)p.c1 * S.Mpad + p.r1]; break; }
+#endif
+        bool reduce = true;
 #if defined(GEN_PROFILE)
-        if (S.dbg & 16u) need = false;
+        if (S.dbg & 16u) reduce = false;
 #endif
         const bool diff = two && p.r1 != p.r2;
-        const uint32_t alphaUnits = need ? (!two ? 4u : (diff ? 8u : 5u)) : 0u;
         float s = 0.f, smu = 0.f;
         uint32_t typeX = p.type;
         constexpr bool PRE = FUSEDF && SINGLE;
@@ -650,8 +677,10 @@
             else if (PRE) eval_update_pre2(S, (R1), (C1), (D1), (R2), (C2), (D2), chunk0, stride, pre); else eval_update_ap2(S, (R1), (C1), (D1), (R2), (C2), (D2), chunk0, stride); } while (0)
         constexpr bool AHEAD = (FUSEDF && SINGLE) || DECIDE;
         EvalSpec spec; spec.rng = rng; spec.mm = mm; spec.l1 = 0.f; spec.l2 = 0.f;
-        spec.n = (AHEAD && scalarLane && need && (p.type == 'D' || p.type == 'M')) ? ((p.type == 'D' && gibbs1) ? 2u : 1u) : 0u;
-        if (need) {
+        spec.n = (AHEAD && scalarLane && reduce && (p.type == 'D' || p.type == 'M')) ? (p.type == 'D' ? 2u : 1u) : 0u;
+        eval_cells_want(S, p, PHASE == EVAL_ALPHA ? slice == 0u : (PHASE != EVAL_APPLY && (!DECIDE || decider)), false, spec);
+        if (PHASE == EVAL_SEQ && spec.want) eval_cells_issue(spec);
+        if (reduce) {
             float tot[4] = {0.f, 0.f, 0.f, 0.f};
             if (PHASE == EVAL_SEQ) {
                 const uint32_t rowA[1] = {p.r1}, colA[1] = {p.c1};
@@ -712,6 +741,17 @@
             s = diff ? tot[0] + tot[2] : tot[0]; smu = diff ? tot[1] - tot[3] : tot[1];
             if (AHEAD && spec.n) eval_spec_run(spec);
         }
+        if (spec.want) eval_cells_issue(spec);
+        if (PHASE == EVAL_ALPHA && slice == 0u && t == 0u) {
+            PropRec *rec = &S.queue[q];
+            rec->old1 = spec.old1; rec->old2 = spec.old2; rec->gibbs = (spec.gib1 > 0u ? 1u : 0u) | ((two && spec.gib2 > 0u) ? 2u : 0u);
+        }
+        if (PHASE == EVAL_APPLY) { spec.old1 = p.old1; spec.old2 = p.old2; spec.gib1 = p.gibbs & 1u; spec.gib2 = (p.gibbs >> 1) & 1u; }
+        const float old1 = spec.old1, old2 = spec.old2;
+        const bool gibbs1 = spec.gib1 > 0u, gibbs2 = two && spec.gib2 > 0u;
+        const bool need = reduce && ((p.type == 'B') ? gibbs1 : ((p.type == 'D' || p.type == 'M') ? true : (gibbs1 || gibbs2)));
+        const uint32_t alphaUnits = need ? (!two ? 4u : (diff ? 8u : 5u)) : 0u;
+        if (!need) { s = 0.f; smu = 0.f; }
         EVAL_PIN(s); EVAL_TS(3);
         if (FUSEDF) EVAL_PREFETCH();
 #if defined(EVAL_ATOMS_LATE)
@@ -812,6 +852,11 @@
         EVAL_TS(6);
         EVAL_TS_DUMP(p.type | (nUpd << 8) | ((p.r1 == p.r2 ? 1u : 0u) << 16));
         if (DECIDE && writer) S.dec[q] = owe;
+        if (CHAINP && decider && t == 0u) {
+            unsigned long long *gd = S.grans + CHAIN_DELTA_GRAN(q);
+            cg_store_agent_u64(&gd[0], ((unsigned long long)first.tag << 32) | (unsigned long long)gm_f2u(owe.d1));
+            cg_store_agent_u64(&gd[1], ((unsigned long long)first.tag << 32) | (unsigned long long)gm_f2u(owe.d2));
+        }
         if (writer) {
             uint32_t units = nUpd * 3u;
             if (need) units += !two ? 4u : (diff ? 8u : 5u);
diff --git a/cogaps_amd/csrc/gen_chain_apply.h b/cogaps_amd/csrc/gen_chain_apply.h
--- a/cogaps_amd/csrc/gen_chain_apply.h
+++ b/cogaps_amd/csrc/gen_chain_apply.h
@@ -7,7 +7,7 @@
     uint32_t mb1, mb2;
     uint32_t *head1, *head2; uint32_t head1Val, h1;
     unsigned long long *b0clr, *b0set, *b1set, *b2set; uint32_t bit1, bit2, bit1w, bit2w;
-    uint32_t hL, hR, h2, l2, cell1, cell2, idx;
+    uint32_t hL, hR, h2, l2, cell1, idx;
     uint32_t sparse; float *rows1, *rows2; unsigned long long *fl1, *fl2; unsigned long long fbit1, fbit2; float colv1, colv2; uint32_t flg1, flg2;
 };
 CG_DEVICE void chain_item_clear(ChainItem &it)
@@ -17,10 +17,10 @@
     it.mb1 = 0; it.mb2 = 0;
     it.pos1 = nullptr; it.rposL = nullptr; it.lposR = nullptr; it.head1 = nullptr; it.head2 = nullptr; it.head1Val = CG_NONE; it.h1 = 0;
     it.b0clr = nullptr; it.b0set = nullptr; it.b1set = nullptr; it.b2set = nullptr; it.bit1 = 0; it.bit2 = 0; it.bit1w = 0; it.bit2w = 0;
-    it.hL = CG_NONE; it.hR = CG_NONE; it.h2 = CG_NONE; it.l2 = CG_NONE; it.cell1 = 0; it.cell2 = 0; it.idx = 0;
+    it.hL = CG_NONE; it.hR = CG_NONE; it.h2 = CG_NONE; it.l2 = CG_NONE; it.cell1 = 0; it.idx = 0;
     it.sparse = 0; it.rows1 = nullptr; it.rows2 = nullptr; it.fl1 = nullptr; it.fl2 = nullptr; it.fbit1 = 0ull; it.fbit2 = 0ull; it.colv1 = 0.f; it.colv2 = 0.f; it.flg1 = 0; it.flg2 = 0;
 }
-struct ChainMid { AtomRec a; uint32_t l2, head1, b1, b2; unsigned long long x1, x2;
+struct ChainMid { AtomRec a; uint32_t l2, head1, b1, b2; unsigned long long x1, x2; float old1, old2;
                   float colv1, colv2; unsigned long long fw1, fw2; };
 CG_DEVICE ChainMid chain_fetch_mid(const SamplerDev &S, const PropRec &p, const bool sparse)
 {
@@ -32,6 +32,8 @@
     m.l2 = S.atoms[hE].left;
     m.head1 = S.binHead[m.b1];
     m.x1 = S.bits1[w1]; m.x2 = S.bits2[w2];
+    m.old1 = sparse ? S.rows[(size_t)p.r1 * S.Kpad + p.c1] : S.mat[(size_t)p.c1 * S.Mpad + p.r1];
+    m.old2 = sparse ? S.rows[(size_t)p.r2 * S.Kpad + p.c2] : S.mat[(size_t)p.c2 * S.Mpad + p.r2];
     m.colv1 = 0.f; m.colv2 = 0.f; m.fw1 = 0ull; m.fw2 = 0ull;
     if (sparse) {
         m.colv1 = S.mat[(size_t)p.c1 * S.Mpad + p.r1]; m.fw1 = S.mflags[(size_t)p.c1 * S.Mw + (p.r1 >> 6)];
@@ -49,10 +51,10 @@
 CG_DEVICE void chain_fetch_build(const SamplerDev &S, const PropRec &p, const ChainMid &m, ChainItem &it, const bool sparse)
 {
     chain_item_clear(it);
-    it.type = p.type; it.m1 = p.m1; it.m2 = p.m2; it.old1 = p.old1; it.old2 = p.old2; it.pos = p.pos; it.h1 = p.h1;
+    it.type = p.type; it.m1 = p.m1; it.m2 = p.m2; it.old1 = m.old1; it.old2 = m.old2; it.pos = p.pos; it.h1 = p.h1;
     it.eraseEntry = ((unsigned long long)(p.r1 * S.K + p.c1) << 32) | (unsigned long long)p.h1;
     const AtomRec a = m.a;
-    it.hL = a.left; it.hR = a.right; it.idx = a.idx; it.cell1 = p.r1 * S.K + p.c1; it.cell2 = p.r2 * S.K + p.c2; it.h2 = p.h2; it.l2 = m.l2;
+    it.hL = a.left; it.hR = a.right; it.idx = a.idx; it.cell1 = p.r1 * S.K + p.c1; it.h2 = p.h2; it.l2 = m.l2;
     it.mass1 = &S.atoms[p.h1].mass; it.rm1 = a.left != CG_NONE ? &S.atoms[a.left].rmass : nullptr;
     it.mat1 = &S.mat[(size_t)p.c1 * S.Mpad + p.r1]; it.col1 = &S.colPos[p.c1];
     const bool two = p.type == 'M' || p.type == 'E';
diff --git a/cogaps_amd/csrc/gen_draw.h b/cogaps_amd/csrc/gen_draw.h
--- a/cogaps_amd/csrc/gen_draw.h
+++ b/cogaps_amd/csrc/gen_draw.h
@@ -70,8 +70,8 @@
 template <int WORDS>
 CG_DEVICE GenNotePos gen_note_pos(uint32_t key)
 {
-    constexpr uint32_t LOG2 = WORDS == 4096 ? 17u : (WORDS == 2048 ? 16u : 13u);
-    static_assert(WORDS == 4096 || WORDS == 2048 || WORDS == 256, "bit numbers are 17 / 16 / 13 bits of the hash");
+    constexpr uint32_t LOG2 = WORDS == 4096 ? 17u : 13u;
+    static_assert(WORDS == 4096 || WORDS == 256, "bit numbers are 17 / 13 bits of the hash");
     const uint32_t h = key * 2654435761u;
     GenNotePos p; p.a = h >> (32u - LOG2); p.b = (h ^ (h >> 11)) & ((1u << LOG2) - 1u);
     return p;
@@ -90,7 +90,7 @@
     uint32_t go, flags; bool isB, pick;
     uint64_t rng, rngPick, pos, cpos;
     uint32_t h1, h2, i1, hl, hr, r1, c1, r2, c2, bin;
-    float nm1, nm2, amass, m2x, old1, old2; uint32_t gib1, gib2;
+    float nm1, nm2, amass, m2x;
     uint64_t lposB, rposB; float rmassB;
     uint32_t headBin, v2, v3, xPick; bool redo;
 };
@@ -98,7 +98,7 @@
 {
     d.go = 0; d.flags = 0; d.isB = false; d.pick = false; d.rng = 0; d.rngPick = 0; d.pos = 0; d.cpos = 0;
     d.h1 = CG_NONE; d.h2 = CG_NONE; d.i1 = CG_NONE; d.hl = CG_NONE; d.hr = CG_NONE; d.r1 = 0; d.c1 = 0; d.r2 = 0; d.c2 = 0; d.bin = 0;
-    d.nm1 = 0.f; d.nm2 = 0.f; d.amass = 0.f; d.m2x = 0.f; d.old1 = 0.f; d.old2 = 0.f; d.gib1 = 0; d.gib2 = 0; d.lposB = 0; d.rposB = 0; d.rmassB = 0.f;
+    d.nm1 = 0.f; d.nm2 = 0.f; d.amass = 0.f; d.m2x = 0.f; d.lposB = 0; d.rposB = 0; d.rmassB = 0.f;
     d.headBin = 0; d.v2 = CG_NONE; d.v3 = CG_NONE; d.xPick = 0; d.redo = false;
 }
 template <int WIN, bool SPEC, bool AHEAD = false>
@@ -177,12 +177,10 @@
         }
     }
     if ((AHEAD || soft) && frontE) { d.redo = true; frontE = false; h2 = h1; }
-    float old1 = 0.f, old2 = 0.f; uint32_t gib1 = 0, gib2 = 0;
     uint64_t lposB = 0, rposB = 0; float rmassB = 0.f;
     if (AHEAD && isB && !slowB && v2 == CG_NONE) { d.redo = true; slowB = true; }
     if (isB && !slowB) b3 = S.atoms[v2];
     if (frontE) b3 = S.atoms[h2];
-    if (isB || pick) { old1 = c.sparse ? S.rows[(size_t)r1 * S.Kpad + c1] : S.mat[(size_t)c1 * S.Mpad + r1]; gib1 = S.otherColPos[c1]; }
     if (pick && type == 'M') {
         if (hl != CG_NONE) { flags |= GEN_F_HASLEFT; lbpos = lp; } else lbpos = 0;
         if (hr != CG_NONE) { flags |= GEN_F_HASRIGHT; rbpos = rp; } else rbpos = S.rboundNone;
@@ -196,7 +194,6 @@
         const uint32_t bin2 = gen_bin_of(S, rbpos);
         r2 = gen_div_k(S, bin2); c2 = bin2 - r2 * K;
     }
-    if (pick && (type == 'M' || (type == 'E' && !frontE))) { old2 = c.sparse ? S.rows[(size_t)r2 * S.Kpad + c2] : S.mat[(size_t)c2 * S.Mpad + r2]; gib2 = S.otherColPos[c2]; }
     if (isB) {
         if (!slowB) {
             if ((flags & GEN_F_BINEMPTY) || b3.pos > pos) { hr = v2; hl = b3.left; lposB = b3.lpos; rposB = b3.pos; rmassB = b3.mass; flags |= GEN_F_NEWHEAD; }
@@ -229,7 +226,6 @@
             flags &= ~(GEN_F_BINEMPTY | GEN_F_WORDZERO | GEN_F_NEWHEAD);
             if (nh) flags |= GEN_F_NEWHEAD;
             if (S.binHead[bin] == CG_NONE) { flags |= GEN_F_BINEMPTY; if (S.bits0[bin >> 6] == 0ull) flags |= GEN_F_WORDZERO; }
-            old1 = c.sparse ? S.rows[(size_t)r1 * S.Kpad + c1] : S.mat[(size_t)c1 * S.Mpad + r1]; gib1 = S.otherColPos[c1];
             lposB = (hl != CG_NONE) ? S.atoms[hl].pos : 0ull;
             if (hr != CG_NONE) { rposB = S.atoms[hr].pos; rmassB = S.atoms[hr].mass; } else { rposB = 0ull; rmassB = 0.f; }
         }
@@ -238,7 +234,6 @@
             rbpos = b3.pos; m2x = b3.mass;
             const uint32_t bin2 = gen_bin_of(S, rbpos);
             r2 = gen_div_k(S, bin2); c2 = bin2 - r2 * K;
-            old2 = c.sparse ? S.rows[(size_t)r2 * S.Kpad + c2] : S.mat[(size_t)c2 * S.Mpad + r2]; gib2 = S.otherColPos[c2];
         }
         if (r1 == r2 && c1 == c2 && !((AHEAD || soft) && d.redo)) {
             flags |= GEN_F_INLINE;
@@ -253,16 +248,15 @@
         }
     }
     d.flags = flags; d.rng = rng; d.pos = pos; d.cpos = cpos; d.h1 = h1; d.h2 = h2; d.hl = hl; d.hr = hr; d.r1 = r1; d.c1 = c1; d.r2 = r2; d.c2 = c2; d.bin = bin;
-    d.nm1 = nm1; d.nm2 = nm2; d.amass = a.mass; d.m2x = m2x; d.old1 = old1; d.old2 = old2; d.gib1 = gib1; d.gib2 = gib2; d.lposB = lposB; d.rposB = rposB; d.rmassB = rmassB;
+    d.nm1 = nm1; d.nm2 = nm2; d.amass = a.mass; d.m2x = m2x; d.lposB = lposB; d.rposB = rposB; d.rmassB = rmassB;
     d.headBin = headBin; d.v2 = v2;
 }
 
-struct GenCheck { GenNotePos atomA, atomB, slot, cellA, cellB, eraseA; uint32_t iPartS; };
-CG_DEVICE GenCheck gen_draw_check(const GenSpec &sp, const GenDraw &d, const uint32_t nRs, const uint32_t K)
+struct GenCheck { GenNotePos atomA, atomB, slot, eraseA; uint32_t iPartS; };
+CG_DEVICE GenCheck gen_draw_check(const GenSpec &sp, const GenDraw &d, const uint32_t nRs)
 {
     const bool isB = (sp.info & 0xFFu) == 'B';
     GenCheck c;
-    c.cellA = gen_note_pos<GEN_DIRTY_CELLS>(isB ? d.bin : d.r1 * K + d.c1); c.cellB = gen_note_pos<GEN_DIRTY_CELLS>(d.r2 * K + d.c2);
     c.atomA = gen_note_pos<GEN_DIRTY_ATOMS>(isB ? d.v2 : d.h1); c.atomB = gen_note_pos<GEN_DIRTY_ATOMS>(d.v3); c.slot = gen_note_pos<GEN_DIRTY_ATOMS>(~d.i1);
     c.eraseA = gen_note_pos<GEN_DIRTY_ERASE>(d.h1);
     c.iPartS = 0xFFFFFFFFu / (nRs + (sp.info >> 8));
@@ -283,11 +277,10 @@
     const bool isB = type == 'B';
     const bool reads = isB || d.pick;
     const uint32_t nA = gen_note_get(sh.dAtom, ck.atomA), nB = gen_note_get(sh.dAtom, ck.atomB), nS = gen_note_get(sh.dAtom, ck.slot);
-    const uint32_t cA = gen_note_get(sh.dCell, ck.cellA), cB = gen_note_get(sh.dCell, ck.cellB);
-    if (isB) { if (reads) bad |= nA | cA; if (d.v3 != CG_NONE) bad |= nB; }
+    if (isB) { if (reads) bad |= nA; if (d.v3 != CG_NONE) bad |= nB; }
     else if (d.pick) {
         const uint32_t nE = gen_note_get(sh.dErase, ck.eraseA);
-        light |= nA | cA | ((type == 'M' || type == 'E') ? cB : 0u);
+        light |= nA;
         bad |= nA & nE;
     }
 #if defined(GEN_TIMELINE)
@@ -326,14 +319,13 @@
     const uint32_t level = d.go == 0u ? 0u : (bad ? 2u : (light && (d.pick || moved) ? 1u : (light ? 2u : 0u)));
 #if defined(GEN_TIMELINE)
     if (d.go) {
-        const uint32_t movedL = (!isB && m != 0u && type != 0u) ? (uint32_t)(((bad & 1u) != 0u) && !(d.redo) && !((reads ? (nA | cA) : 0u) & 1u)) : 0u;
+        const uint32_t movedL = (!isB && m != 0u && type != 0u) ? (uint32_t)(((bad & 1u) != 0u) && !(d.redo) && !((reads ? nA : 0u) & 1u)) : 0u;
         cg_atomic_add_u64(&g_ahead_why[0], 1ull);
         if (!ok) cg_atomic_add_u64(&g_ahead_why[1], 1ull);
         if (movedL | moved) cg_atomic_add_u64(&g_ahead_why[2], 1ull);
         if (d.pick && m != 0u && nS) cg_atomic_add_u64(&g_ahead_why[3], 1ull);
         if (reads && (nA | ((isB && d.v3 != CG_NONE) ? nB : 0u))) cg_atomic_add_u64(&g_ahead_why[4], 1ull);
-        if (reads && (cA | ((d.pick && (type == 'M' || type == 'E')) ? cB : 0u))) cg_atomic_add_u64(&g_ahead_why[5], 1ull);
-        if (isB && !ok && !d.redo && !(nA | cA)) cg_atomic_add_u64(&g_ahead_why[6], 1ull);
+        if (isB && !ok && !d.redo && !nA) cg_atomic_add_u64(&g_ahead_why[6], 1ull);
         if (d.redo) cg_atomic_add_u64(&g_ahead_why[7], 1ull);
     }
     if (level == 2u) {
@@ -342,7 +334,7 @@
             const uint32_t hasB = (uint32_t)(d.v3 != CG_NONE);
             const uint32_t ers = (nA & gen_note_get(sh.dErase, gen_note_pos<GEN_DIRTY_ERASE>(d.v2))) | (hasB & nB & gen_note_get(sh.dErase, gen_note_pos<GEN_DIRTY_ERASE>(d.v3)));
             if (tlDirty) cause |= 4u;
-            if (ers) cause |= 2u; else if (nA | cA | (hasB & nB)) cause |= 1u;
+            if (ers) cause |= 2u; else if (nA | (hasB & nB)) cause |= 1u;
         } else {
             if (d.pick && (nA & gen_note_get(sh.dErase, ck.eraseA))) cause |= 32u;
             if (tlSame == 0u) {
diff --git a/cogaps_amd/csrc/gen_handover_pass.h b/cogaps_amd/csrc/gen_handover_pass.h
--- a/cogaps_amd/csrc/gen_handover_pass.h
+++ b/cogaps_amd/csrc/gen_handover_pass.h
@@ -4,8 +4,7 @@
                 bool have = (HP_MINE) && q < e_prevQ;
                 if (HP_FETCH(base)) { chain_item_clear(it); if (have) chain_fetch(S, hot.queueRd, q, it, isSparse); }
                 const GenNotePos nH1 = gen_note_pos<GEN_DIRTY_ATOMS>(it.h1), nHL = gen_note_pos<GEN_DIRTY_ATOMS>(it.hL), nHR = gen_note_pos<GEN_DIRTY_ATOMS>(it.hR),
-                                 nH2 = gen_note_pos<GEN_DIRTY_ATOMS>(it.h2), nL2 = gen_note_pos<GEN_DIRTY_ATOMS>(it.l2), nIdx = gen_note_pos<GEN_DIRTY_ATOMS>(~it.idx),
-                                 nC1 = gen_note_pos<GEN_DIRTY_CELLS>(it.cell1), nC2 = gen_note_pos<GEN_DIRTY_CELLS>(it.cell2);
+                                 nH2 = gen_note_pos<GEN_DIRTY_ATOMS>(it.h2), nL2 = gen_note_pos<GEN_DIRTY_ATOMS>(it.l2), nIdx = gen_note_pos<GEN_DIRTY_ATOMS>(~it.idx);
                 const unsigned long long *gr = hot.grans + (size_t)q * CHAIN_GRAN_STRIDE;
                 unsigned long long g0 = 0ull, g1 = 0ull; uint32_t spins = 0;
                 for (;;) {
@@ -39,8 +38,6 @@
                         if (it.hL != CG_NONE) gen_note_set(sh.dErase, gen_note_pos<GEN_DIRTY_ERASE>(it.hL));
                         if (it.hR != CG_NONE) gen_note_set(sh.dErase, gen_note_pos<GEN_DIRTY_ERASE>(it.hR));
                     }
-                    if (ap || it.type == 'D') gen_note_set(sh.dCell, nC1);
-                    if (ap && (it.type == 'M' || it.type == 'E')) gen_note_set(sh.dCell, nC2);
                 }
                 const unsigned long long em = cg_ballot(er);
                 if (em) {
diff --git a/cogaps_amd/csrc/gen_kernel.h b/cogaps_amd/csrc/gen_kernel.h
--- a/cogaps_amd/csrc/gen_kernel.h
+++ b/cogaps_amd/csrc/gen_kernel.h
@@ -67,7 +67,6 @@
 #define GEN_CHAIN_THREADS 512
 
 #define GEN_DIRTY_ATOMS 4096
-#define GEN_DIRTY_CELLS 2048
 #define GEN_DIRTY_ERASE 256
 struct GenTabVal { uint32_t used, gap, inl, pad; };
 struct GenTabKeys { uint32_t k[4]; };
@@ -101,7 +100,7 @@
     unsigned long long eraseTmp[FLUSH_MAX]; uint32_t eraseN, specBad, spinFail;
     float dpWin[4 * WIN];
     uint32_t dirty[512];
-    alignas(16) uint32_t dAtom[GEN_DIRTY_ATOMS]; uint32_t dCell[GEN_DIRTY_CELLS]; uint32_t dErase[GEN_DIRTY_ERASE]; uint32_t anyRedo;
+    alignas(16) uint32_t dAtom[GEN_DIRTY_ATOMS]; uint32_t dErase[GEN_DIRTY_ERASE]; uint32_t anyRedo;
 };
 
 CG_DEVICE uint32_t gen_bin_of(const SamplerDev &S, uint64_t pos)
diff --git a/cogaps_amd/csrc/gen_populate.h b/cogaps_amd/csrc/gen_populate.h
--- a/cogaps_amd/csrc/gen_populate.h
+++ b/cogaps_amd/csrc/gen_populate.h
@@ -25,7 +25,7 @@
     const uint64_t jm0 = hot.lcgMul[2u * ta], ji0 = hot.lcgInc[2u * ta];
     const uint64_t jm1 = hot.lcgMul[ta ? 2u * (ta - 1u) : 0u], ji1 = hot.lcgInc[ta ? 2u * (ta - 1u) : 0u];
     unsigned long long specE = (!CHAIN && helper && ht < (unsigned)FLUSH_MAX && ht < hot.eraseCap) ? hot.eraseList[ht] : 0ull;
-    PropRec p0; p0.type = 0; p0.h1 = 0; p0.h2 = 0; p0.pos = 0; p0.curPos = 0; p0.r1 = 0; p0.c1 = 0; p0.r2 = 0; p0.c2 = 0; p0.m1 = 0.f; p0.m2 = 0.f; p0.old1 = 0.f; p0.old2 = 0.f;
+    PropRec p0; p0.type = 0; p0.h1 = 0; p0.h2 = 0; p0.pos = 0; p0.curPos = 0; p0.r1 = 0; p0.c1 = 0; p0.r2 = 0; p0.c2 = 0; p0.m1 = 0.f; p0.m2 = 0.f;
     if (applier && ht < hot.queueCap) p0 = hot.queueRd[ht];
 
     uint32_t units = (!CHAIN && attempt && t < hot.queueCap) ? hot.queueUnits[t] : 0u;
@@ -46,11 +46,10 @@
 #pragma unroll
         for (uint32_t k = 0; k < ROUNDS; ++k) { if (!CHAIN && !spare && ((k + 1u) * TPB <= UNITS || t + k * TPB < UNITS)) tab[k * TPB] = none; }
         if (CHAIN) {
-            static_assert(offsetof(GenShared<WIN>, dCell) == offsetof(GenShared<WIN>, dAtom) + 4u * (size_t)GEN_DIRTY_ATOMS
-                          && offsetof(GenShared<WIN>, dErase) == offsetof(GenShared<WIN>, dCell) + 4u * (size_t)GEN_DIRTY_CELLS, "the note tables are contiguous");
+            static_assert(offsetof(GenShared<WIN>, dErase) == offsetof(GenShared<WIN>, dAtom) + 4u * (size_t)GEN_DIRTY_ATOMS, "the note tables are contiguous");
             GenTabKeys *dt = reinterpret_cast<GenTabKeys *>(&sh.dAtom[0]);
             GenTabKeys zero; zero.k[0] = zero.k[1] = zero.k[2] = zero.k[3] = 0u;
-            for (uint32_t i = t; i < (uint32_t)(GEN_DIRTY_ATOMS + GEN_DIRTY_CELLS + GEN_DIRTY_ERASE) / 4u; i += cg_bdim()) dt[i] = zero;
+            for (uint32_t i = t; i < (uint32_t)(GEN_DIRTY_ATOMS + GEN_DIRTY_ERASE) / 4u; i += cg_bdim()) dt[i] = zero;
         }
     }
     GEN_TS(27);
@@ -75,7 +74,7 @@
     uint64_t epoch0 = 0;
     GenDraw drawKeep; gen_draw_clear(drawKeep);
     GenCheck checkKeep; checkKeep.atomA.a = checkKeep.atomA.b = checkKeep.atomB.a = checkKeep.atomB.b = checkKeep.slot.a = checkKeep.slot.b = 0u;
-    checkKeep.cellA.a = checkKeep.cellA.b = checkKeep.cellB.a = checkKeep.cellB.b = checkKeep.eraseA.a = checkKeep.eraseA.b = 0u; checkKeep.iPartS = 1u;
+    checkKeep.eraseA.a = checkKeep.eraseA.b = 0u; checkKeep.iPartS = 1u;
     if (!CHAIN) {
         GEN_TS_ZERO(7u, 13u);
 #if defined(GEN_TIMELINE)
@@ -108,7 +107,7 @@
         constexpr bool ATTEMPTS_APPLY = SP == 1 && 2 * WIN >= GEN_CHAIN_THREADS;
 #endif
         const uint32_t passLanes = ATTEMPTS_APPLY ? NA + (uint32_t)WIN : NA;
-        ChainMid mid0; mid0.l2 = CG_NONE; mid0.head1 = CG_NONE; mid0.b1 = 0; mid0.b2 = 0; mid0.x1 = 0ull; mid0.x2 = 0ull;
+        ChainMid mid0; mid0.l2 = CG_NONE; mid0.head1 = CG_NONE; mid0.b1 = 0; mid0.b2 = 0; mid0.x1 = 0ull; mid0.x2 = 0ull; mid0.old1 = 0.f; mid0.old2 = 0.f;
         mid0.a.pos = 0; mid0.a.lpos = 0; mid0.a.rpos = 0; mid0.a.left = CG_NONE; mid0.a.right = CG_NONE; mid0.a.mass = 0.f; mid0.a.rmass = 0.f; mid0.a.idx = 0; mid0.a.pad0 = 0;
         const uint32_t freeTopAhead = (helper && ht < 16u && ht < e_fc) ? S.freeHandles[e_fc - 1u - ht] : CG_NONE;
         if (applier) mid0 = chain_fetch_mid(S, p0, isSparse);
@@ -163,8 +162,8 @@
                 gen_draw_b<WIN, true>(S, sh, rcS, typeS, drawKeep, [&]() {});
             }
 #endif
-            if (drawAhead) checkKeep = gen_draw_check(spS, drawKeep, e_n, rcS.K);
-            GEN_PIN(drawKeep.flags); GEN_PIN(drawKeep.old1); GEN_PIN(drawKeep.old2);
+            if (drawAhead) checkKeep = gen_draw_check(spS, drawKeep, e_n);
+            GEN_PIN(drawKeep.flags);
             GEN_TS(36);
             GEN_RT(2);
             if constexpr (ATTEMPTS_APPLY) {
diff --git a/cogaps_amd/csrc/gen_round.h b/cogaps_amd/csrc/gen_round.h
--- a/cogaps_amd/csrc/gen_round.h
+++ b/cogaps_amd/csrc/gen_round.h
@@ -109,7 +109,7 @@
     const uint64_t rng = d.rng, pos = d.pos, cpos = d.cpos;
     uint32_t h1 = d.h1, h2 = d.h2, i1 = d.i1, i2 = CG_NONE; const uint32_t hl = d.hl, hr = d.hr;
     const uint32_t r1 = d.r1, c1 = d.c1, r2 = d.r2, c2 = d.c2, bin = d.bin; const float nm1 = d.nm1, nm2 = d.nm2;
-    const float old1 = d.old1, old2 = d.old2, m2x = d.m2x; const uint32_t gib1 = d.gib1, gib2 = d.gib2;
+    const float m2x = d.m2x;
     const uint64_t lposB = d.lposB, rposB = d.rposB; const float rmassB = d.rmassB;
     struct { float mass; } a; a.mass = d.amass;
     (void)isB; (void)pick;
@@ -371,11 +371,19 @@
                 PropRec p; p.pos = (type == 'M') ? pos : 0ull; p.rng = rng; p.h1 = h1; p.h2 = h2; p.i1 = i1; p.i2 = i2;
                 p.r1 = r1; p.c1 = c1; p.r2 = r2; p.c2 = c2; p.type = type; p.batch = 0; p.pad[0] = p.pad[1] = p.pad[2] = 0;
                 const bool two = type == 'M' || type == 'E';
-                p.gibbs = (gib1 > 0u ? 1u : 0u) | ((two && gib2 > 0u) ? 2u : 0u);
+                p.gibbs = 0u; p.old1 = 0.f; p.old2 = 0.f;
                 p.m1 = (type == 'B') ? 0.f : a.mass; p.m2 = (type == 'E') ? m2x : 0.f;
-                p.old1 = old1; p.old2 = two ? old2 : 0.f; p.curPos = (type == 'M') ? cpos : 0ull;
+                p.curPos = (type == 'M') ? cpos : 0ull;
                 c.queueOut[slot] = p;
-                if (c_traceOn) { const uint32_t ti = c_traceCount + slot; if (ti < c_traceCap) { p.batch = c_nBatches; S.trace[ti] = p; } }
+                if (c_traceOn) {
+                    const uint32_t ti = c_traceCount + slot;
+                    if (ti < c_traceCap) {
+                        p.old1 = c.sparse ? S.rows[(size_t)r1 * S.Kpad + c1] : S.mat[(size_t)c1 * S.Mpad + r1];
+                        if (two) p.old2 = c.sparse ? S.rows[(size_t)r2 * S.Kpad + c2] : S.mat[(size_t)c2 * S.Mpad + r2];
+                        p.gibbs = (S.otherColPos[c1] > 0u ? 1u : 0u) | ((two && S.otherColPos[c2] > 0u) ? 2u : 0u);
+                        p.batch = c_nBatches; S.trace[ti] = p;
+                    }
+                }
             }
         }
     }
diff --git a/cogaps_amd/csrc/sparse_kernels.h b/cogaps_amd/csrc/sparse_kernels.h
--- a/cogaps_amd/csrc/sparse_kernels.h
+++ b/cogaps_amd/csrc/sparse_kernels.h
@@ -563,19 +563,20 @@
         uint64_t rng = p.rng;
         const EvalAtoms ea = eval_atoms_load(S, p, !CHAIN && t == 0u);
         const bool two = (p.type == 'M' || p.type == 'E');
-        const float m1 = p.m1, m2 = p.m2, old1 = p.old1, old2 = p.old2;
-        const bool gibbs1 = (p.gibbs & 1u) != 0u, gibbs2 = (p.gibbs & 2u) != 0u;
-        const bool need = (p.type == 'B') ? gibbs1 : ((p.type == 'D' || p.type == 'M') ? true : (gibbs1 || gibbs2));
+        const float m1 = p.m1, m2 = p.m2;
+        const bool reduce = true;
         const bool diff = two && p.r1 != p.r2;
         float s = 0.f, smu = 0.f;
         uint32_t nz = 0;
         if (t == 0) nzShared = 0u;
         SpCell cell1, cell2; cell1.colv = 0.f; cell1.flagged = false; cell2 = cell1;
         if (!CHAIN && t == 0u) { cell1 = sp_cell_load(S, p.r1, p.c1); if (two) cell2 = sp_cell_load(S, p.r2, p.c2); }
-        const float z1a = need ? S.Z1[p.c1] : 0.f, z1b = (need && two) ? S.Z1[p.c2] : 0.f;
+        EvalSpec cl; cl.rng = 0ull; cl.n = 0u; cl.mm = 0u; cl.l1 = 0.f; cl.l2 = 0.f;
+        eval_cells_want(S, p, true, true, cl); eval_cells_issue(cl);
+        const float z1a = reduce ? S.Z1[p.c1] : 0.f, z1b = (reduce && two) ? S.Z1[p.c2] : 0.f;
         SpPre preA, preB; preA.dfl = preA.fv = 0ull; preA.dbase = 0u; preB = preA;
-        if (!SEQ && need) { preA = sp_preload(S, p.r1, p.c1, p.c2, two && !diff); if (diff) preB = sp_preload(S, p.r2, p.c2, 0u, false); }
-        if (need) {
+        if (!SEQ && reduce) { preA = sp_preload(S, p.r1, p.c1, p.c2, two && !diff); if (diff) preB = sp_preload(S, p.r2, p.c2, 0u, false); }
+        if (reduce) {
             for (uint32_t k = t; k < S.Kpad; k += BS) {
                 arowA[k] = S.rows[(size_t)p.r1 * S.Kpad + k];
                 if (diff) arowB[k] = S.rows[(size_t)p.r2 * S.Kpad + k];
@@ -648,6 +649,10 @@
             }
             }
         }
+        const float old1 = cl.old1, old2 = cl.old2;
+        const bool gibbs1 = cl.gib1 > 0u, gibbs2 = two && cl.gib2 > 0u;
+        const bool need = (p.type == 'B') ? gibbs1 : ((p.type == 'D' || p.type == 'M') ? true : (gibbs1 || gibbs2));
+        if (!need) { s = 0.f; smu = 0.f; }
         EVAL_PIN(s); EVAL_TS(5);
         s = s * T; smu = smu * T;
         const bool writer = !CHAIN && t == 0u;
```

After: 8.054 million. 0.984x the previous value.
